# shiinamiyuki/akari_render

Hardware: AMD Instinct MI355X
Metric: Msamples/s (whole node), 1080p path tracer, C2 (higher is better)
Workload: dtype f32

## Files before the change

akari_render_amd/abi.py:

```python
from __future__ import annotations

import ctypes as C
from dataclasses import dataclass, field
from typing import List, Optional

import numpy as np

c_f32p = C.POINTER(C.c_float)
c_u32p = C.POINTER(C.c_uint32)


class _Struct(C.Structure):

    def __setattr__(self, name, value):
        if not any(f[0] == name for f in self._fields_):
            raise AttributeError("%s has no field %r" % (type(self).__name__, name))
        super().__setattr__(name, value)


class MeshDesc(C.Structure):
    _fields_ = [
        ("n_vertices", C.c_uint32),
        ("n_triangles", C.c_uint32),
        ("vertices", c_f32p),
# ... 239 lines not shown
        ("adaptive", C.c_uint32), ("wis", C.c_uint32),
        ("seed", C.c_uint64),
        ("filter_type", C.c_uint32), ("filter_radius", C.c_float), ("sampler_type", C.c_uint32), ("color", C.c_uint32),
        ("sampler_seed", C.c_uint64),
    ]

    @staticmethod
    def default() -> "McmcConfig":
        c = McmcConfig()
        c.spp, c.max_depth, c.rr_depth, c.spp_per_pass, c.use_nee = 256, 7, 5, 64, 1
        c.mcmc_depth, c.n_chains, c.n_bootstrap, c.direct_spp = 0xFFFFFFFF, 512, 100000, 64
        c.exponential_mutation, c.small_sigma, c.large_step_prob, c.image_mutation_prob, c.image_mutation_size = 1, 0.01, 0.1, 0.0, 0.0
        c.filter_type, c.filter_radius = FILTER_GAUSSIAN, 1.5
        c.sampler_type, c.sampler_seed = SAMPLER_INDEPENDENT, 0
        return c


class McmcResult(C.Structure):
    _fields_ = [("normalization", C.c_double), ("acceptance_rate", C.c_double), ("splat_scale", C.c_float), ("contribution", C.c_float),
                ("n_mutations", C.c_uint64), ("sample_dimension", C.c_uint32), ("_pad", C.c_uint32)]


class McmcPartial(C.Structure):

    _fields_ = [("bootstrap_sum", C.c_double), ("b_sum", C.c_double), ("n_bootstrap", C.c_uint64), ("b_cnt", C.c_uint64), ("n_accepted", C.c_uint64),
                ("n_mutations", C.c_uint64), ("n_executed", C.c_uint64), ("spp", C.c_uint32), ("contribution", C.c_float)]


MARKOV_STATE_DTYPE = [("cur_pixel", "<u4", (2,)), ("chain_id", "<u4"), ("cur_f", "<f4"), ("b", "<f4"), ("b_cnt", "<u4"), ("n_accepted", "<u4"),
                      ("n_mutations", "<u4"), ("cur_iter", "<u4"), ("last_large_iter", "<u4")]


class AdaptiveConfig(_Struct):

    _fields_ = [("threshold", C.c_float), ("min_spp", C.c_uint32), ("round_passes", C.c_uint32), ("_pad", C.c_uint32)]

    @staticmethod
    def default() -> "AdaptiveConfig":
        c = AdaptiveConfig()
        c.threshold, c.min_spp, c.round_passes = 0.0625, 16, 1
        return c


DISPLAY_LINEAR, DISPLAY_REINHARD, DISPLAY_ACES, DISPLAY_HABLE = 1, 2, 3, 4
DISPLAY_CURVE_NAMES = {DISPLAY_LINEAR: "linear", DISPLAY_REINHARD: "reinhard", DISPLAY_ACES: "aces", DISPLAY_HABLE: "hable"}


class DisplayConfig(_Struct):

    _fields_ = [
        ("curve", C.c_uint32),
        ("auto_exposure", C.c_uint32),
        ("exposure_ev", C.c_float),
        ("key", C.c_float),
        ("low_permille", C.c_uint32),
        ("high_permille", C.c_uint32),
        ("white", C.c_float),
        ("bloom_strength", C.c_float),
        ("bloom_threshold", C.c_float),
        ("bloom_levels", C.c_uint32),
        ("_pad", C.c_uint32 * 2),
    ]

    @staticmethod
    def default() -> "DisplayConfig":
        c = DisplayConfig()
        c.curve, c.auto_exposure, c.exposure_ev, c.key = DISPLAY_ACES, 0, 0.0, 0.18
        c.low_permille, c.high_permille, c.white = 50, 20, 0.0
        c.bloom_strength, c.bloom_threshold, c.bloom_levels = 0.0, 1.0, 5
        return c


class PtStats(C.Structure):
    _fields_ = [
        ("n_samples", C.c_uint64),
        ("n_closest", C.c_uint64),
        ("n_shadow", C.c_uint64),
        ("n_shaded", C.c_uint64),
        ("n_node_visits", C.c_uint64),
        ("n_tri_tests", C.c_uint64),
        ("kernel_ms", C.c_double),
        ("n_launches", C.c_uint32),
        ("_pad", C.c_uint32),
    ]

    def as_dict(self):
        return {k: getattr(self, k) for k, _ in self._fields_ if not k.startswith("_")}


class AdaptiveStats(C.Structure):

    _fields_ = [("rounds", C.c_uint32), ("tiles_retired", C.c_uint32), ("samples_drawn", C.c_uint64), ("samples_uniform", C.c_uint64), ("pt", PtStats)]

    def as_dict(self):
        return {"rounds": self.rounds, "tiles_retired": self.tiles_retired, "samples_drawn": self.samples_drawn, "samples_uniform": self.samples_uniform,
                "pt": self.pt.as_dict()}


class KernelInfo(C.Structure):

    _fields_ = [
        ("struct_size", C.c_uint32),
        ("specialised", C.c_uint32),
        ("cache_hit", C.c_uint32),
        ("n_shader_kinds", C.c_uint32),
        ("absent_mask", C.c_uint32),
        ("min_waves", C.c_uint32),
        ("vgprs", C.c_uint32),
        ("scratch_bytes", C.c_uint32),
        ("kernel_flags", C.c_uint32),
        ("_pad", C.c_uint32),
        ("compile_ms", C.c_double),
        ("load_ms", C.c_double),
        ("status", C.c_char * 256),
    ]

    def as_dict(self):
        d = {k: getattr(self, k) for k, _ in self._fields_ if k not in ("struct_size", "status", "_pad")}
        d["status"] = self.status.decode(errors="replace")
        return d


class PtLaunchPlan(C.Structure):

    VARIANT = ("bvh", "fd", "tex", "pmj", "stage", "defer", "simple", "inst", "env", "lens")
    _fields_ = [
        ("variant", C.c_uint32 * 10),
        ("simple_scene", C.c_uint32), ("defer_metal", C.c_uint32), ("defer_flags", C.c_uint32),
        ("stage_bytes", C.c_uint32 * 13), ("stage_total", C.c_uint32),
        ("tile_offset", C.c_uint32), ("bvh_tile_nodes", C.c_uint32), ("park_offset", C.c_uint32), ("carry_offset", C.c_uint32),
        ("bn_offset", C.c_uint32), ("val_offset_words", C.c_uint32),
        ("lds_bytes", C.c_uint32), ("blocks", C.c_uint32),
        ("specialised", C.c_uint32),
        ("wrapper", C.c_char * 600),
    ]

    def as_dict(self):
        d = {k: getattr(self, k) for k, _ in self._fields_ if k not in ("variant", "stage_bytes", "wrapper")}
        d["variant"] = {n: int(self.variant[i]) for i, n in enumerate(self.VARIANT)}
        d["stage_bytes"] = [int(b) for b in self.stage_bytes]
        d["wrapper"] = self.wrapper.decode()
        return d


class PtFeaturesPlan(C.Structure):

    _fields_ = [
        ("plan", PtLaunchPlan),
        ("feat", C.c_uint32), ("kernel_compiled", C.c_uint32), ("park_slots", C.c_uint32), ("park_slots_feat", C.c_uint32),
        ("required_bytes", C.c_uint32), ("lds_budget", C.c_uint32),
    ]

    def as_dict(self):
        d = self.plan.as_dict()
        d["variant"]["feat"] = int(self.feat)
        for k in ("kernel_compiled", "park_slots", "park_slots_feat", "required_bytes", "lds_budget"):
            d[k] = int(getattr(self, k))
        return d


class SceneInfo(C.Structure):
    _fields_ = [
        ("width", C.c_uint32),
        ("height", C.c_uint32),
        ("n_instances", C.c_uint32),
        ("n_triangles", C.c_uint32),
        ("n_materials", C.c_uint32),
        ("n_lights", C.c_uint32),
        ("n_bvh_nodes", C.c_uint32),
        ("uses_bvh", C.c_uint32),
# ... 243 lines not shown
```

akari_render_amd/capi.py:

```python
from __future__ import annotations

import ctypes as C
import os
from typing import Optional

import numpy as np

from . import abi
from .build import LIB, build

AKR_OK = 0
FILM_PLANE_RGB, FILM_PLANE_SPLAT, FILM_PLANE_WEIGHT, FILM_PLANES_PT, FILM_PLANES_ALL = 1, 2, 4, 5, 7
ERR_INVALID_ARGUMENT, ERR_HIP, ERR_NO_DEVICE, ERR_IO, ERR_PARSE, ERR_UNSUPPORTED, ERR_OOM, ERR_RENDER = -1, -2, -3, -4, -5, -6, -7, -8

(ARRAY_WOOP, ARRAY_TRI_GID, ARRAY_SHADE, ARRAY_INSTANCES, ARRAY_MATERIALS, ARRAY_BVH_NODES, ARRAY_LIGHT_ENTRIES,
 ARRAY_LIGHT_PDF, ARRAY_AREA_ENTRIES, ARRAY_AREA_PDF, ARRAY_INST_TRI_OFFSET, ARRAY_R2C, ARRAY_C2W,
 ARRAY_TEX_NODES, ARRAY_TEX_IMAGES, ARRAY_TEX_TEXELS, ARRAY_MAT_INPUTS,
 ARRAY_INST_LEAVES, ARRAY_MESH_TRIS, ARRAY_MESH_POS, ARRAY_MESH_META, ARRAY_MESH_NORMALS,
 ARRAY_ENV_MARGINAL_ENTRIES, ARRAY_ENV_MARGINAL_PDF, ARRAY_ENV_CONDITIONAL_ENTRIES, ARRAY_ENV_CONDITIONAL_PDF, ARRAY_ENV_TEXELS) = range(27)
ENV_LIGHT_INSTANCE = 0xFFFFFFFF

EXPORTS = [
    "akr_last_error", "akr_version", "akr_struct_size", "akr_option_set", "akr_option_get", "akr_context_create",
    "akr_context_destroy", "akr_context_synchronize", "akr_context_device_info", "akr_scene_create", "akr_scene_load",
    "akr_scene_destroy", "akr_scene_set_resolution", "akr_scene_get_info", "akr_scene_get_light", "akr_scene_get_ggx_table",
    "akr_scene_get_desc_counts", "akr_scene_get_mesh", "akr_scene_get_instance", "akr_scene_get_material", "akr_scene_get_camera",
    "akr_scene_get_array", "akr_scene_get_image_count", "akr_scene_get_image", "akr_scene_get_material_graph", "akr_film_create",
    "akr_film_wrap", "akr_film_destroy", "akr_film_clear", "akr_film_read", "akr_film_write", "akr_film_resolve",
    "akr_film_device_ptr", "akr_pt_config_default", "akr_pt_config_from_json", "akr_pt_render", "akr_pt_begin", "akr_pt_passes",
    "akr_pt_begin_features", "akr_pt_render_features",
    "akr_pt_end", "akr_pt_get_stats", "akr_render_task", "akr_image_write", "akr_aov_config_default", "akr_aov_render",
    "akr_gpt_config_default", "akr_gpt_render", "akr_gpt_begin", "akr_gpt_sample", "akr_gpt_sums", "akr_gpt_sums_read",
    "akr_gpt_sums_write", "akr_gpt_finish", "akr_gpt_abort", "akr_gpt_reduce", "akr_mcmc_config_default", "akr_mcmc_render",
    "akr_film_set_splat_scale", "akr_film_get_splat_scale", "akr_pt_read_sampler_states", "akr_context_device_ordinal",
    "akr_device_count", "akr_comm_unique_id", "akr_comm_create", "akr_comm_wrap", "akr_comm_destroy", "akr_film_reduce",
    "akr_pt_kernel_info", "akr_scene_spec_source", "akr_host_spec_compile", "akr_host_spec_compile_text",
    "akr_film_reduce_planes", "akr_mcmc_render_shard", "akr_mcmc_combine_host", "akr_mcmc_combine",
    "akr_scene_set_environment", "akr_scene_get_environment", "akr_scene_set_lens", "akr_scene_get_lens",
    "akr_denoise_config_default", "akr_denoise", "akr_denoise_variance",
    "akr_pt_set_active_tiles", "akr_film_tile_error", "akr_adaptive_config_default", "akr_pt_adaptive_render",
    "akr_display_config_default", "akr_film_luminance_histogram", "akr_display_exposure", "akr_display_transform",
]
TEST_EXPORTS = [
    "akr_probe_material_inputs_host", "akr_host_stdrng_u64", "akr_host_chacha_block", "akr_host_pcg32_states",
    "akr_host_pcg_start", "akr_host_alias_table", "akr_probe_math", "akr_probe_bsdf", "akr_probe_intersect",
    "akr_probe_surface_interaction", "akr_probe_material_inputs", "akr_host_decode_png", "akr_host_decode_jpeg",
    "akr_host_decode_exr", "akr_host_decode_tiff", "akr_host_decode_dds", "akr_host_pmj02bn_tables",
    "akr_probe_material_folded_host", "akr_host_sobol_dim1", "akr_host_fastmod", "akr_host_tri_pretest",
    "akr_probe_env_sample", "akr_probe_env_pdf", "akr_host_lens_ray", "akr_probe_camera_rays",
    "akr_probe_div", "akr_probe_intersect_pair", "akr_probe_math2", "akr_host_denoise", "akr_probe_denoise_times",
    "akr_host_pt_launch_plan", "akr_host_denoise_variance", "akr_probe_denoise_variance_times",
    "akr_host_tile_error", "akr_host_half_bracket", "akr_probe_adapt_times",
    "akr_host_display_transform", "akr_host_luminance_histogram", "akr_probe_display_times",
    "akr_host_pt_features_plan", "akr_host_pcg_end_pass", "akr_probe_pcg_end_pass",
]


class RenderSession(C.Structure):

    _fields_ = [("save_intermediate", C.c_int32), ("save_stats", C.c_int32), ("name", C.c_char_p),
                ("override_sampler_independent", C.c_int32), ("verbose", C.c_int32)]


class AkariError(RuntimeError):
    def __init__(self, code: int, msg: str):
        super().__init__(f"akari_hip error {code}: {msg}")
        self.code = code


_lib: Optional[C.CDLL] = None


def lib() -> C.CDLL:
    global _lib
    if _lib is not None:
        return _lib
    if not os.path.exists(LIB):
        build()
    L = C.CDLL(os.environ.get("AKR_HIP_LIB") or LIB)
    vp, u32, u64, i32, f32 = C.c_void_p, C.c_uint32, C.c_uint64, C.c_int32, C.c_float
    fp, up, u64p, vpp = C.POINTER(C.c_float), C.POINTER(C.c_uint32), C.POINTER(C.c_uint64), C.POINTER(C.c_void_p)
    L.akr_last_error.restype = C.c_char_p
    L.akr_version.restype = C.c_char_p
    L.akr_struct_size.restype = C.c_uint32
    L.akr_struct_size.argtypes = [C.c_int32]
    for sid, cls in enumerate((abi.MeshDesc, abi.InstanceDesc, abi.MaterialDesc, abi.CameraDesc, abi.SceneDesc, abi.PtConfig, abi.PtStats, abi.SceneInfo,
                               abi.KernelInfo, abi.AovConfig, abi.GptConfig, abi.McmcConfig, abi.McmcResult, abi.McmcPartial,
                               abi.EnvironmentDesc, abi.LensDesc, abi.DenoiseConfig), start=1):
        if L.akr_struct_size(sid) != C.sizeof(cls):
            raise ImportError("libakari_hip.so and akari_render_amd/abi.py disagree on sizeof(%s): %d vs %d" % (cls.__name__, L.akr_struct_size(sid), C.sizeof(cls)))
    for sid, cls in ((19, abi.AdaptiveConfig), (20, abi.AdaptiveStats), (22, abi.DisplayConfig)):
        if L.akr_struct_size(sid) != C.sizeof(cls):
            raise ImportError("libakari_hip.so and akari_render_amd/abi.py disagree on sizeof(%s): %d vs %d" % (cls.__name__, L.akr_struct_size(sid), C.sizeof(cls)))

    def proto(name, *args):
        if name in TEST_EXPORTS and not hasattr(L, name):
            return
        fn = getattr(L, name)
        fn.restype = i32
        fn.argtypes = list(args)

    proto("akr_context_create", i32, vpp)
    proto("akr_context_destroy", vp)
    proto("akr_context_synchronize", vp)
    proto("akr_context_device_info", vp, C.c_char_p, u32, up, u64p)
    proto("akr_scene_create", vp, C.POINTER(abi.SceneDesc), vpp)
    proto("akr_scene_load", vp, C.c_char_p, u32, u32, vpp)
    proto("akr_scene_destroy", vp)
    proto("akr_scene_set_resolution", vp, u32, u32)
    proto("akr_scene_get_info", vp, C.POINTER(abi.SceneInfo))
    proto("akr_scene_get_light", vp, u32, up, fp, fp)
    proto("akr_scene_set_environment", vp, C.POINTER(abi.EnvironmentDesc))
    proto("akr_scene_get_environment", vp, C.POINTER(abi.EnvironmentDesc))
    proto("akr_scene_set_lens", vp, C.POINTER(abi.LensDesc))
    proto("akr_scene_get_lens", vp, C.POINTER(abi.LensDesc))
    proto("akr_host_lens_ray", vp, u32, f32, u32, up, fp, fp)
    proto("akr_probe_camera_rays", vp, vp, u32, f32, u32, up, fp, fp)
    proto("akr_host_pt_launch_plan", vp, C.POINTER(abi.PtConfig), i32, i32, i32, i32, C.POINTER(abi.PtLaunchPlan))
    proto("akr_host_pt_features_plan", vp, C.POINTER(abi.PtConfig), i32, i32, i32, i32, i32, i32, i32, C.POINTER(abi.PtFeaturesPlan))
    proto("akr_probe_env_sample", vp, vp, u32, fp, fp)
    proto("akr_probe_env_pdf", vp, vp, u32, fp, fp)
    proto("akr_scene_get_ggx_table", vp, fp)
    proto("akr_scene_get_desc_counts", vp, up, up, up)
    proto("akr_scene_get_mesh", vp, u32, C.POINTER(abi.MeshDesc))
    proto("akr_scene_get_instance", vp, u32, C.POINTER(abi.InstanceDesc))
    proto("akr_scene_get_material", vp, u32, C.POINTER(abi.MaterialDesc))
    proto("akr_scene_get_camera", vp, C.POINTER(abi.CameraDesc))
    proto("akr_scene_get_array", vp, i32, vpp, u64p)
    proto("akr_scene_get_image_count", vp, up)
    proto("akr_scene_get_image", vp, u32, C.POINTER(abi.ImageDesc))
    proto("akr_scene_get_material_graph", vp, u32, C.POINTER(abi.MaterialGraph))
    proto("akr_film_create", vp, u32, u32, vpp)
    proto("akr_film_wrap", vp, u32, u32, vp, vpp)
    proto("akr_film_destroy", vp)
    proto("akr_film_clear", vp)
    proto("akr_film_read", vp, fp)
    proto("akr_film_write", vp, fp)
    proto("akr_film_resolve", vp, fp)
    proto("akr_film_device_ptr", vp, vpp, u64p)
    proto("akr_pt_kernel_info", vp, C.POINTER(abi.KernelInfo))
    proto("akr_scene_spec_source", vp, C.c_char_p, u64, u64p)
    proto("akr_host_spec_compile", vp, u32, u32, C.c_char_p, u64p, C.c_char_p, u32)
    proto("akr_probe_material_folded_host", vp, u32, u32, fp, up, fp, fp)
    proto("akr_host_sobol_dim1", u32, up, up, up)
    proto("akr_host_fastmod", u32, up, up, up)
    proto("akr_host_tri_pretest", u32, fp, fp, f32, up, up, fp)
    proto("akr_host_spec_compile_text", C.c_char_p, u32, u32, C.c_char_p, C.c_char_p)
    proto("akr_context_device_ordinal", vp, C.POINTER(C.c_int32))
    proto("akr_device_count", C.POINTER(C.c_int32))
    proto("akr_option_set", C.c_char_p, i32)
    proto("akr_option_get", C.c_char_p, C.POINTER(C.c_int32))
    proto("akr_comm_unique_id", C.POINTER(C.c_uint8))
    proto("akr_comm_create", vp, C.POINTER(C.c_uint8), i32, i32, vpp)
    proto("akr_comm_wrap", vp, vp, i32, i32, vpp)
    proto("akr_comm_destroy", vp)
    proto("akr_film_reduce", vp, vp, i32, i32)
    proto("akr_film_reduce_planes", vp, vp, i32, i32, u32)
    proto("akr_mcmc_render_shard", vp, vp, C.POINTER(abi.McmcConfig), u32, u32, vp, C.POINTER(abi.McmcPartial), up, C.POINTER(abi.PtStats))
    proto("akr_mcmc_combine_host", vp, C.POINTER(abi.McmcPartial), u32, C.POINTER(abi.McmcResult))
    proto("akr_mcmc_combine", vp, vp, i32, C.POINTER(abi.McmcPartial), C.POINTER(abi.McmcResult))
    proto("akr_pt_config_default", C.POINTER(abi.PtConfig))
    proto("akr_aov_config_default", C.POINTER(abi.AovConfig))
    proto("akr_aov_render", vp, vp, C.POINTER(abi.AovConfig), vp, C.POINTER(abi.PtStats))
    proto("akr_gpt_config_default", C.POINTER(abi.GptConfig))
    proto("akr_gpt_render", vp, vp, C.POINTER(abi.GptConfig), vp, fp, C.POINTER(abi.PtStats))
    proto("akr_gpt_begin", vp, vp, C.POINTER(abi.GptConfig), vp, vp, vpp)
    proto("akr_gpt_sample", vp, u32, i32)
    proto("akr_gpt_sums", vp, C.POINTER(fp), u64p)
    proto("akr_gpt_sums_read", vp, fp)
    proto("akr_gpt_sums_write", vp, fp)
    proto("akr_gpt_finish", vp, fp, C.POINTER(abi.PtStats))
    proto("akr_gpt_abort", vp, C.POINTER(abi.PtStats))
    proto("akr_gpt_reduce", vp, vp, i32, i32)
    proto("akr_mcmc_config_default", C.POINTER(abi.McmcConfig))
    proto("akr_mcmc_render", vp, vp, C.POINTER(abi.McmcConfig), vp, C.POINTER(abi.McmcResult), up, C.POINTER(abi.PtStats))
    proto("akr_film_set_splat_scale", vp, C.c_float)
    proto("akr_film_get_splat_scale", vp, fp)
    proto("akr_pt_config_from_json", C.c_char_p, C.POINTER(abi.PtConfig), C.c_char_p, u32)
    proto("akr_pt_render", vp, vp, C.POINTER(abi.PtConfig), vp, C.POINTER(abi.PtStats))
    proto("akr_pt_begin", vp, vp, C.POINTER(abi.PtConfig), vp, vpp)
    proto("akr_pt_passes", vp, u32, i32, up)
    proto("akr_pt_begin_features", vp, vp, C.POINTER(abi.PtConfig), vp, vp, vp, vpp)
    proto("akr_pt_render_features", vp, vp, C.POINTER(abi.PtConfig), vp, vp, vp, C.POINTER(abi.PtStats))
    proto("akr_pt_end", vp, C.POINTER(abi.PtStats))
    proto("akr_pt_get_stats", vp, C.POINTER(abi.PtStats))
    proto("akr_render_task", vp, vp, C.c_char_p, C.POINTER(RenderSession), C.POINTER(abi.PtStats))
    proto("akr_image_write", C.c_char_p, fp, u32, u32)
    proto("akr_pt_read_sampler_states", vp, u64p)
    proto("akr_host_stdrng_u64", u64, u32, u64p)
    proto("akr_host_chacha_block", up, u64, u64, i32, up)
    proto("akr_host_pcg32_states", u64, u64, u64p)
    proto("akr_host_pcg_start", u64p, u64)
    proto("akr_host_pcg_end_pass", u64p, u64, u32)
    proto("akr_probe_pcg_end_pass", vp, u32, u64p, u64p, up, u64p, u64p)
    proto("akr_host_alias_table", fp, u32, up, fp, fp)
    proto("akr_probe_math", vp, u32, fp, fp, fp, fp)
    proto("akr_probe_math2", vp, u32, fp, fp)
    proto("akr_probe_bsdf", vp, C.POINTER(abi.MaterialDesc), fp, i32, fp, u32, fp, fp)
    proto("akr_probe_intersect", vp, vp, u32, fp, up, fp)
    proto("akr_probe_div", vp, u32, fp, fp, fp, fp)
    proto("akr_probe_intersect_pair", vp, vp, u32, fp, up, up, fp)
    proto("akr_probe_surface_interaction", vp, vp, u32, up, fp, fp)
# ... 238 lines not shown
        for i in range(nm.value):
            m = abi.MeshDesc()
            check(lib().akr_scene_get_mesh(self.h, i, C.byref(m)))
            nt = m.n_triangles
            uv = arr(m.uvs, 6 * nt, np.float32)
            nr = arr(m.normals, 9 * nt, np.float32)
            tg = arr(m.tangents, 9 * nt, np.float32)
            meshes.append(abi.MeshData(
                vertices=arr(m.vertices, 3 * m.n_vertices, np.float32).reshape(-1, 3),
                indices=arr(m.indices, 3 * nt, np.uint32).reshape(-1, 3),
                uvs=None if uv is None else uv.reshape(-1, 3, 2),
                normals=None if nr is None else nr.reshape(-1, 3, 3),
                tangents=None if tg is None else tg.reshape(-1, 3, 3),
                material_slots=arr(m.material_slots, nt, np.uint32)))
        for i in range(ni.value):
            d = abi.InstanceDesc()
            check(lib().akr_scene_get_instance(self.h, i, C.byref(d)))
            instances.append(abi.InstanceData(d.mesh, [int(d.materials[k]) for k in range(d.n_materials)],
                                              np.array(list(d.transform), dtype=np.float32)))
        for i in range(nmat.value):
            d = abi.MaterialDesc()
            check(lib().akr_scene_get_material(self.h, i, C.byref(d)))
            md = abi.MaterialData()
            md.kind = d.kind & abi.MAT_KIND_MASK
            md.colorspaces = d.kind & 0xF00
            for name in ("base_color", "specular_tint", "coat_tint", "emission_color", "normal"):
                setattr(md, name, tuple(float(x) for x in getattr(d, name)))
            for name in ("base_alpha", "metallic", "roughness", "ior", "specular_ior_level", "transmission_weight",
                         "coat_weight", "coat_roughness", "coat_ior", "emission_strength"):
                setattr(md, name, float(getattr(d, name)))
            g = abi.MaterialGraph()
            check(lib().akr_scene_get_material_graph(self.h, i, C.byref(g)))
            if g.n_nodes:
                nodes = [abi.NodeData(int(g.nodes[j].op), tuple(int(a) for a in g.nodes[j].arg), tuple(float(x) for x in g.nodes[j].k))
                         for j in range(g.n_nodes)]
                inputs = {abi.INPUT_NAMES[k]: int(g.input[k]) for k in range(abi.IN_COUNT) if g.input[k] != abi.NODE_NONE}
                md.graph = abi.GraphData(nodes, inputs)
            materials.append(md)
        images = []
        nimg = C.c_uint32()
        check(lib().akr_scene_get_image_count(self.h, C.byref(nimg)))
        for i in range(nimg.value):
            d = abi.ImageDesc()
            check(lib().akr_scene_get_image(self.h, i, C.byref(d)))
            n = d.width * d.height * 4
            if d.format == abi.IMAGE_RGBA8:
                t = np.frombuffer((C.c_uint8 * n).from_address(d.texels), dtype=np.uint8).copy()
            else:
                t = np.frombuffer((C.c_float * n).from_address(d.texels), dtype=np.float32).copy()
            images.append(abi.ImageData(t.reshape(d.height, d.width, 4), d.filter, d.address))
        c = abi.CameraDesc()
        check(lib().akr_scene_get_camera(self.h, C.byref(c)))
        cam = abi.CameraData(np.array(list(c.c2w), dtype=np.float32), float(c.fov), c.width, c.height)
        return abi.SceneData(meshes, instances, materials, cam, images=images, environment=self.environment(), lens=self.lens())


def set_option(name: str, value: int) -> None:
    check(lib().akr_option_set(name.encode(), int(value)))


def get_option(name: str) -> int:
    v = C.c_int32()
    check(lib().akr_option_get(name.encode(), C.byref(v)))
    return v.value


class options:

    def __init__(self, **kw):
        self.kw, self.old = kw, {}

    def __enter__(self):
        for k, v in self.kw.items():
            self.old[k] = get_option(k)
            set_option(k, v)
        return self

    def __exit__(self, *exc):
        for k, v in self.old.items():
            set_option(k, v)
        return False


def last_error() -> str:
    return lib().akr_last_error().decode("utf-8", "replace")


def device_count() -> int:
    n = C.c_int32()
    check(lib().akr_device_count(C.byref(n)))
    return n.value


def comm_unique_id() -> bytes:
    buf = (C.c_uint8 * 128)()
    check(lib().akr_comm_unique_id(buf))
    return bytes(buf)


class Comm:

    def __init__(self, ctx: "Context", unique_id: bytes, rank: int, world: int):
        assert len(unique_id) == 128
        self.h = C.c_void_p()
        buf = (C.c_uint8 * 128).from_buffer_copy(unique_id)
        check(lib().akr_comm_create(ctx.h, buf, rank, world, C.byref(self.h)))
        self.rank, self.world = rank, world

    def close(self):
        if getattr(self, "h", None):
            lib().akr_comm_destroy(self.h)
            self.h = None

    def __del__(self):
        try:
            self.close()
        except Exception:
            pass

    def mcmc_combine(self, film: "Film", partial, root: int = 0) -> dict:
        res = abi.McmcResult()
        check(lib().akr_mcmc_combine(film.h, self.h, root, C.byref(partial), C.byref(res)))
        return {k: getattr(res, k) for k, _ in abi.McmcResult._fields_ if k != "_pad"}

    def reduce_film(self, film: "Film", root: int = 0, blocking: bool = True, planes: int = 7):
        check(lib().akr_film_reduce_planes(film.h, self.h, root, 1 if blocking else 0, planes))


class Film:

    def __init__(self, ctx: Context, width: int, height: int, device_ptr: Optional[int] = None):
        self.ctx, self.width, self.height = ctx, width, height
        self.h = C.c_void_p()
        if device_ptr is None:
            check(lib().akr_film_create(ctx.h, width, height, C.byref(self.h)))
        else:
            check(lib().akr_film_wrap(ctx.h, width, height, C.c_void_p(device_ptr), C.byref(self.h)))

    def close(self):
        if self.h:
            lib().akr_film_destroy(self.h)
            self.h = C.c_void_p()

    def __del__(self):
        try:
            self.close()
        except Exception:
            pass

    def clear(self):
        check(lib().akr_film_clear(self.h))

    def read(self) -> np.ndarray:
        out = np.zeros(7 * self.width * self.height, dtype=np.float32)
        check(lib().akr_film_read(self.h, _fp(out)))
        return out

    def write(self, data: np.ndarray):
        data = np.ascontiguousarray(data, dtype=np.float32)
        assert data.size == 7 * self.width * self.height
        check(lib().akr_film_write(self.h, _fp(data)))

    def resolve(self) -> np.ndarray:
        out = np.zeros(3 * self.width * self.height, dtype=np.float32)
        check(lib().akr_film_resolve(self.h, _fp(out)))
        return out.reshape(self.height, self.width, 3)
# ... 522 lines not shown
```

akari_render_amd/csrc/device/pt_pass.h:

```cpp
#pragma once
#include "dpath.h"

namespace akr {

#ifndef AKR_PT_MIN_WAVES
#define AKR_PT_MIN_WAVES 4
#endif
#ifndef AKR_PT_MIN_WAVES_BVH
#define AKR_PT_MIN_WAVES_BVH 4
#endif
#ifndef AKR_PT_MIN_WAVES_FD
#define AKR_PT_MIN_WAVES_FD 4
#endif
#ifndef AKR_PT_MIN_WAVES_TEX
#define AKR_PT_MIN_WAVES_TEX 3
#endif
#ifndef AKR_PT_MIN_WAVES_BVH_TEX
#define AKR_PT_MIN_WAVES_BVH_TEX 3
#endif
template <bool TEX>
using PairWalkOpt = WalkOpt<!TEX>;
template <bool BVH, bool FD, bool TEX, bool PMJ, bool STAGE, bool DEFER, uint32_t ABSENT = 0, bool INST = false, bool ENV = false, bool LENS = false, bool FEAT = false>
AKR_D void pt_pass_body(const PtParams& p) {
    extern __shared__ __attribute__((aligned(16))) uint32_t lds_stack[];
    TraceCtx tc;
    tc.stack = lds_stack + threadIdx.x;
    tc.cnt = TraceCounters{0, 0, 0};
    PtParams staged = p;
    if (STAGE) stage_scene_tables<BVH, TEX, !BVH && !FD && TEX>(p, lds_stack, staged);
    const PtParams& q = STAGE ? staged : p;
    const DScene& sc = q.sc;
    constexpr bool TILE = BVH && !TEX && !INST;
    constexpr uint32_t STRAG = BVH ? (INST ? AKR_PT_STRAGGLERS_INST : (TEX ? AKR_PT_STRAGGLERS_TEX : AKR_PT_STRAGGLERS)) : 0;
    const uint4* tile = (const uint4*)(lds_stack + p.tile_offset);
    if (TILE) {
        uint32_t* l = lds_stack + p.tile_offset;
        const uint32_t* g = (const uint32_t*)p.sc.bvh_nodes;
        for (uint32_t i = threadIdx.x; i < p.sc.bvh_tile_nodes * kBvhNodeWords; i += 256u) l[i] = g[i];
        __syncthreads();
    }
    const float4* lds_recs = nullptr;
    if (!BVH) {
        uint32_t* l = lds_stack + (p.stage_total >> 2);
        const uint32_t* g = (const uint32_t*)p.sc.woop;
        for (uint32_t i = threadIdx.x; i < (p.sc.n_tris + 2u) * 12u; i += 256u) l[i] = g[i];
        __syncthreads();
        lds_recs = (const float4*)l;
    }
    const uint32_t item = blockIdx.x * 256u + threadIdx.x;
    uint32_t px = 0, py = 0;
    const bool in_frame = item < p.n_items && item_to_pixel(p, item, px, py);
    const uint32_t pix = px + py * p.width;
    uint32_t sx, sy;
    shifted_pixel(p, px, py, sx, sy);
    if (PMJ && p.bn_offset != 0) pmj_bluenoise_stage(p, px, py);
    PathRegs r;
    path_regs_init<PMJ, LENS, FEAT>(r, q, in_frame, pix, sx, sy);
    constexpr bool PARK = !FD && TEX;
    uint32_t* park = lds_stack + p.park_offset + threadIdx.x;
    if (PARK) {
        park_put(park, PK_PIX, pix);
        park_put(park, PK_SX, sx);
        park_put(park, PK_SY, sy);
        if (FEAT) {
            park_put(park, PK_FEAT_A + 0, f2u(r.feat_a.x)); park_put(park, PK_FEAT_A + 1, f2u(r.feat_a.y)); park_put(park, PK_FEAT_A + 2, f2u(r.feat_a.z));
            park_put(park, PK_FEAT_N + 0, f2u(r.feat_n.x)); park_put(park, PK_FEAT_N + 1, f2u(r.feat_n.y)); park_put(park, PK_FEAT_N + 2, f2u(r.feat_n.z));
        }
    }

    uint32_t iteration = 0;
    while (__builtin_amdgcn_ballot_w64(r.active) != 0) {
        iteration++;
        if (r.active) {
            Hit hit;
            bool found = false, occluded = false;
            if (!(STRAG > 0 && r.carry)) {
                r.c_closest += r.has_ray ? 1u : 0u;
                r.c_shadow += r.has_shadow ? 1u : 0u;
            }
            if (BVH && INST) {
                trace_pair_inst<TEX, STRAG>(sc, r.has_ray, r.ro, r.rd, r.ray_ex0, r.has_shadow, r.s_o, r.s_d, r.s_tmax, r.s_ex0, r.s_ex1, r.carry, hit, found, occluded, tc.stack,
                                            lds_stack + p.carry_offset + threadIdx.x, tc.cnt);
            } else if (BVH && STRAG > 0) {
                uint32_t* cy = lds_stack + p.carry_offset + threadIdx.x;
                Trav s;
                uint32_t phase;
                hit.t = 1e20f; hit.u = 0.0f; hit.v = 0.0f; hit.gid = kInvalid;
                if (!r.carry) {
                    phase = r.has_ray ? 0u : (r.has_shadow ? 1u : 2u);
                    if (phase == 0) trav_begin(s, r.ro, r.rd, 0.0f, 1e20f, r.ray_ex0, kInvalid);
                    else trav_begin(s, r.s_o, r.s_d, 0.0f, phase == 1 ? r.s_tmax : -1.0f, r.s_ex0, r.s_ex1);
                } else {
                    phase = cy[CY_PHASE * 256];
                    if (phase == 0) trav_begin(s, r.ro, r.rd, 0.0f, 1e20f, r.ray_ex0, kInvalid);
                    else {
                        trav_begin(s, r.s_o, r.s_d, 0.0f, r.s_tmax, r.s_ex0, r.s_ex1);
                        hit.t = u2f(cy[CY_HIT_T * 256]); hit.u = u2f(cy[CY_HIT_U * 256]); hit.v = u2f(cy[CY_HIT_V * 256]); hit.gid = cy[CY_HIT_GID * 256];
                        found = hit.gid != kInvalid;
                    }
                    s.best_t = u2f(cy[CY_BEST_T * 256]); s.best_u = u2f(cy[CY_BEST_U * 256]); s.best_v = u2f(cy[CY_BEST_V * 256]); s.best = cy[CY_BEST * 256];
                    s.G = cy[CY_G * 256]; s.T = cy[CY_T * 256]; s.tbase = cy[CY_TBASE * 256]; s.sp = cy[CY_SP * 256];
                    s.active = true;
                }
                const uint32_t n_in = (uint32_t)__builtin_popcountll(__builtin_amdgcn_ballot_w64(phase != 2u));
                const uint32_t n_leave = n_in / (STRAG > 0 ? STRAG : 1u);
                while (true) {
                    const uint32_t n_now = (uint32_t)__builtin_popcountll(__builtin_amdgcn_ballot_w64(phase != 2u));
                    if (n_now <= n_leave) break;
                    if (phase != 2u) {
                        if (s.active) trav_step<2, TEX, TILE>(sc, s, tc.stack, tc.cnt, phase == 1u, tile);
                        if (!s.active) {
                            if (phase == 0u) {
                                found = s.best != kInvalid;
                                hit.t = s.best_t; hit.u = s.best_u; hit.v = s.best_v; hit.gid = s.best;
                                phase = r.has_shadow ? 1u : 2u;
                                if (r.has_shadow) trav_begin(s, r.s_o, r.s_d, 0.0f, r.s_tmax, r.s_ex0, r.s_ex1);
                            } else {
                                occluded = s.best != kInvalid;
                                phase = 2u;
                            }
                        }
                    }
                }
                r.carry = phase != 2u;
                if (r.carry) {
                    cy[CY_BEST_T * 256] = f2u(s.best_t); cy[CY_BEST_U * 256] = f2u(s.best_u); cy[CY_BEST_V * 256] = f2u(s.best_v); cy[CY_BEST * 256] = s.best;
                    cy[CY_G * 256] = s.G; cy[CY_T * 256] = s.T; cy[CY_TBASE * 256] = s.tbase; cy[CY_SP * 256] = s.sp;
                    cy[CY_PHASE * 256] = phase;
                    if (phase == 1u) { cy[CY_HIT_T * 256] = f2u(hit.t); cy[CY_HIT_U * 256] = f2u(hit.u); cy[CY_HIT_V * 256] = f2u(hit.v); cy[CY_HIT_GID * 256] = hit.gid; }
                }
            } else if (BVH) {
                Trav s;
                uint32_t phase = r.has_ray ? 0u : (r.has_shadow ? 1u : 2u);
                if (phase == 0) trav_begin(s, r.ro, r.rd, 0.0f, 1e20f, r.ray_ex0, kInvalid);
                else trav_begin(s, r.s_o, r.s_d, 0.0f, phase == 1 ? r.s_tmax : -1.0f, r.s_ex0, r.s_ex1);
                hit.t = 1e20f; hit.u = 0.0f; hit.v = 0.0f; hit.gid = kInvalid;
                while (phase != 2u) {
                    if (s.active) trav_step<2, TEX, TILE>(sc, s, tc.stack, tc.cnt, phase == 1u, tile);
                    if (!s.active) {
                        if (phase == 0u) {
                            found = s.best != kInvalid;
                            hit.t = s.best_t; hit.u = s.best_u; hit.v = s.best_v; hit.gid = s.best;
                            phase = r.has_shadow ? 1u : 2u;
                            if (r.has_shadow) trav_begin(s, r.s_o, r.s_d, 0.0f, r.s_tmax, r.s_ex0, r.s_ex1);
                        } else {
                            occluded = s.best != kInvalid;
                            phase = 2u;
                        }
                    }
                }
            } else {
                trace_pair_exhaustive<TEX, PairWalkOpt<TEX>>(sc, r.ro, r.rd, r.has_ray ? 1e20f : -1.0f, r.ray_ex0, r.s_o, r.s_d, r.has_shadow ? r.s_tmax : -1.0f, r.s_ex0, r.s_ex1, hit, found,
                                           occluded, lds_recs);
            }
            if (DEFER) {
                if (r.deferred) {
                    hit.gid = r.d_gid; hit.u = r.d_u; hit.v = r.d_v; hit.t = 0.0f;
                    found = true;
                    r.has_ray = true;
                    r.deferred = false;
                } else if (r.has_ray && found && (iteration & q.defer_metal)) {
                    const uint32_t mat = f2u(sc.shade[(size_t)hit.gid * SHADE_ROWS + 6].y);
                    if (sc.materials[mat].flags & q.defer_flags) {
                        r.d_gid = hit.gid; r.d_u = hit.u; r.d_v = hit.v;
                        r.deferred = true;
                        r.has_ray = false;
                    }
                }
            }
            if (STRAG > 0 && r.carry) {
            } else if (PARK) path_step<FD ? 1 : 0, TEX, PMJ, DEFER ? 1 : 2, ABSENT, INST, ENV, LENS, FEAT>(q, r, hit, found, occluded, 0, 0, 0, park);
            else path_step<FD ? 1 : 0, TEX, PMJ, 0, ABSENT, INST, ENV, LENS, FEAT>(q, r, hit, found, occluded, pix, sx, sy);
        }
    }
    flush_counters(p, r, tc.cnt, BVH);
}

constexpr int pt_pass_min_waves(bool bvh, bool fd, bool tex) {
    return bvh ? (tex ? AKR_PT_MIN_WAVES_BVH_TEX : AKR_PT_MIN_WAVES_BVH) : (fd ? AKR_PT_MIN_WAVES_FD : (tex ? AKR_PT_MIN_WAVES_TEX : AKR_PT_MIN_WAVES));
}

}
```

akari_render_amd/csrc/host/api_internal.h:

```cpp
#pragma once
#include <atomic>
#include <mutex>
#include <hip/hip_runtime.h>

#include <algorithm>
#include <array>
#include <cstdlib>
#include <cstdio>
#include <chrono>
#include <cstring>
#include <functional>
#include <map>
#include <memory>
#include <new>
#include <stdexcept>
#include <string>
#include <vector>

#include "scene_build.h"
#include "specialise.h"
#include "stdrng.h"


namespace akr_api {
// ... 88 lines not shown
    TileGrid g;
    auto or_default = [](uint32_t t) { return t ? t : 32u; };
    g.tile_w = or_default(tile_w);
    g.tile_h = or_default(tile_h);
    g.tiles_x = (width + g.tile_w - 1) / g.tile_w;
    g.tiles_y = (height + g.tile_h - 1) / g.tile_h;
    uint32_t n = g.tiles_x * g.tiles_y;
    if (count > 1) {
        n = 0;
        for (uint32_t ty = 0; ty < g.tiles_y; ty++)
            for (uint32_t tx = 0; tx < g.tiles_x; tx++) n += tile_owner(tx, ty, count) == rank ? 1u : 0u;
    }
    g.n_items = n * g.tile_w * g.tile_h;
    return g;
}

}
using namespace akr_api;


struct akr_context {
    int device = 0;
    hipStream_t stream = nullptr;
    hipDeviceProp_t props;
    void bind() const { HIP_CHECK(hipSetDevice(device)); }
    SpecCache spec_cache;
    std::mutex ggx_mutex;
    std::vector<float> ggx_cache;
    DevBuf pmj_sets, bluenoise;
    void ensure_pmj_tables() {
        if (pmj_sets.p && bluenoise.p) return;
        std::vector<uint32_t> sets;
        std::vector<uint16_t> bn;
        make_pmj02_sets(sets);
        load_bluenoise(bn);
        pmj_sets.upload(sets);
        bluenoise.upload(bn);
    }
};

struct akr_scene {
    akr_context* ctx = nullptr;
    FlatScene flat;
    CompiledScene cs;
    DevBuf light_alias, area_alias, lights;
    DevBuf woop, tri_gid, shade, normals, inst, materials, ggx_table, light_entries, light_pdf, light_inst, light_tri_offset,
        light_n_tris, area_entries, area_pdf, inst_tri_offset, bvh_nodes, tex_nodes, tex_images, tex_texels, tex_mat_inputs;
    DevBuf in2_tlas_leaves, in2_mesh_tris, in2_mesh_pos, in2_mesh_meta, in2_mesh_normals, in2_inst_mats, in2_share_bits;
    DevBuf env_texels, env_marginal, env_conditional, env_rec;
    std::atomic<int> sessions{0};
    std::vector<float> ggx_host;
    struct ColorSet {
        DevBuf materials, tex_nodes, mat_inputs;
    };
    std::map<uint32_t, std::unique_ptr<ColorSet>> color_sets;
    std::mutex color_sets_mutex;
    std::string spec_header;
    bool spec_header_made = false;
    std::mutex spec_mutex;
    DScene dscene;
    float r2c[16], c2w[16];
    uint32_t c2w_identity = 0;
    uint64_t device_bytes = 0;
};

struct akr_film {
    akr_context* ctx = nullptr;
    uint32_t width = 0, height = 0;
    DevBuf own;
    float* data = nullptr;
    float splat_scale = 1.0f;
    size_t n_floats() const { return 7ull * width * height; }
};

struct RenderBase {
    akr_context* ctx = nullptr;
    akr_scene* scene = nullptr;
    akr_film* film = nullptr;
    akr_pt_config cfg;
    DevBuf states, counters;
    TileGrid grid;
    DevBuf owned_tiles;
    uint32_t spp_done = 0, n_launches = 0;
    uint32_t pmj_spp = 1;
    const akr_scene::ColorSet* color_set = nullptr;
    int defer_metal_option = -1;
    int simple_kernels_option = 1;
    int defer_on_option = 0;
    std::vector<std::pair<hipEvent_t, hipEvent_t>> pending;
    double kernel_ms = 0.0;
    PtVariant variant{};
    PtParams params;
    bool holds_scene = false;
    akr_film *feat_albedo = nullptr, *feat_normal = nullptr;
    void fold_events(bool all) {
        size_t keep = 0;
        for (size_t i = 0; i < pending.size(); i++) {
            auto& ev = pending[i];
            if (all || hipEventQuery(ev.second) == hipSuccess) {
                float t = 0.0f;
                if (hipEventElapsedTime(&t, ev.first, ev.second) == hipSuccess) kernel_ms += t;
                (void)hipEventDestroy(ev.first);
                (void)hipEventDestroy(ev.second);
            } else {
                pending[keep++] = ev;
            }
        }
        pending.resize(keep);
    }
    virtual ~RenderBase() {
        if (holds_scene) scene->sessions--;
        for (auto& ev : pending) {
            (void)hipEventDestroy(ev.first);
            (void)hipEventDestroy(ev.second);
        }
    }
};

struct WavefrontState {
    DevBuf state, queues, ctrl, pend, carry;
    bool sort = false;
    DevBuf keys, sorted, sort_tmp;
    uint32_t *sorted_closest = nullptr, *sorted_shadow = nullptr, *sorted_keys = nullptr;
    WfBuffers buf;
    uint32_t slots = 0, trace_blocks = 0;
    std::vector<WfBuffers> group;
    std::vector<hipStream_t> streams;
    std::vector<hipEvent_t> join;
    hipEvent_t fork = nullptr;
    ~WavefrontState() {
        for (hipStream_t st : streams) (void)hipStreamDestroy(st);
        for (hipEvent_t ev : join) (void)hipEventDestroy(ev);
        if (fork) (void)hipEventDestroy(fork);
    }
};

struct akr_pt_session : RenderBase {
    std::unique_ptr<WavefrontState> wf;
    int sched_trial = 0;
    uint64_t passes_launched = 0;
    int max_fused_option = 0;
    bool spec_active = false;
    bool arith_relaxed = false;
    int spec_waves = 3;
    std::shared_ptr<SpecKernel> spec;
    std::string spec_status = "not requested";
    DevBuf active_tiles;
    bool active_set = false;
};

namespace akr_api {
struct LaunchTimer {
    RenderBase* se;
    hipEvent_t e0 = nullptr, e1 = nullptr;
    explicit LaunchTimer(RenderBase* s) : se(s) {
        HIP_CHECK(hipEventCreate(&e0));
        HIP_CHECK(hipEventCreate(&e1));
        HIP_CHECK(hipEventRecord(e0, se->ctx->stream));
    }
    LaunchTimer(const LaunchTimer&) = delete;
    LaunchTimer& operator=(const LaunchTimer&) = delete;
    void stop() {
        HIP_CHECK(hipEventRecord(e1, se->ctx->stream));
        se->pending.emplace_back(e0, e1);
        e0 = e1 = nullptr;
        if (se->pending.size() > 16) se->fold_events(false);
    }
    ~LaunchTimer() {
        if (e0) (void)hipEventDestroy(e0);
        if (e1) (void)hipEventDestroy(e1);
    }
};

void base_begin(RenderBase* se, akr_context* ctx, akr_scene* scene, const akr_pt_config* cfg, akr_film* film);
int32_t render_begin(akr_context* ctx, akr_scene* scene, const akr_pt_config* cfg, akr_film* film, RenderBase** out);
int32_t base_end(RenderBase* se, akr_pt_stats* stats);
void session_params(RenderBase* se, bool spec_active = false, int spec_waves = 3, bool wf_sort = false);
inline void set_launch_passes(RenderBase* se, uint32_t n_passes, uint32_t last_pass_spp) {
    se->params.n_passes = n_passes;
    se->params.last_pass_spp = last_pass_spp;
}
struct PtPlan {
    PtVariant v;
    uint32_t simple_scene, defer_metal, defer_flags;
    uint32_t stage_bytes[13], stage_total, tex_slots;
};
PtPlan pt_plan(const akr_scene* s, const akr_pt_config& c, int defer_metal_option, int simple_kernels_option, int defer_on_option, bool spec_active, int spec_waves, bool feat = false);
std::string pt_features_refusal(const akr_scene* s, const TuningOptions& t);
PtVariant pt_scene_facts(const akr_scene* s, const akr_pt_config& c);
inline uint32_t scene_stack_depth(const CompiledScene& cs) {
    return cs.instanced.on ? cs.bvh_depth : std::max(1u, std::min(cs.bvh_depth, kBvhStackDepth));
}
inline uint32_t scene_n_nodes(const CompiledScene& cs) { return (uint32_t)((cs.instanced.on ? cs.instanced.nodes.size() : cs.bvh_nodes.size()) / kBvhNodeWords); }
void camera_params(PtParams& p, const akr_scene* s, uint32_t filter_type, float filter_radius);
template <typename End>
int32_t end_keeping_first_error(int32_t rc, End&& end) {
    const std::string err = g_last_error;
    const int32_t rc2 = end();
    if (rc == AKR_OK) return rc2;
    g_last_error = err;
    return rc;
}
uint32_t session_samples(const akr_pt_config& c);
std::vector<uint32_t> owned_tiles(uint32_t tiles_x, uint32_t tiles_y, uint32_t rank, uint32_t count);
void scene_finish(akr_scene* s);
void scene_spec_header(akr_scene* scene, std::string& out);
int32_t mcmc_render_impl(akr_context* ctx, akr_scene* scene, const akr_mcmc_config* cfg, akr_film* film, akr_mcmc_result* result, uint32_t* chain_states,
                         akr_pt_stats* stats, const std::function<void(uint32_t, double)>& on_pass, uint32_t shard_rank = 0, uint32_t shard_count = 1,
                         akr_mcmc_partial* partial = nullptr);
}
```

akari_render_amd/csrc/host/api_probe.cpp:

```cpp
#if defined(AKR_TEST_HOOKS) && AKR_TEST_HOOKS
#include "api_internal.h"
#include "../../../include/akari_hip_test.h"
#include "../device/dinst.h"
#include "../device/disect.h"
#include "../device/dpath.h"

extern "C" {

AKR_TEST_API int32_t akr_host_stdrng_u64(uint64_t seed, uint32_t n, uint64_t* out) {
    if (!out) return fail(AKR_ERR_INVALID_ARGUMENT, "out is NULL");
    StdRng rng(seed);
    for (uint32_t i = 0; i < n; i++) out[i] = rng.next_u64();
    return AKR_OK;
}
AKR_TEST_API int32_t akr_host_chacha_block(const uint32_t* key8, uint64_t counter, uint64_t stream, int32_t rounds, uint32_t* out16) {
    if (!key8 || !out16) return fail(AKR_ERR_INVALID_ARGUMENT, "NULL argument");
    StdRng::chacha_block(key8, counter, stream, rounds, out16);
    return AKR_OK;
}
AKR_TEST_API int32_t akr_host_pcg32_states(uint64_t seed, uint64_t n, uint64_t* out2n) {
    if (!out2n) return fail(AKR_ERR_INVALID_ARGUMENT, "out is NULL");
    StdRng rng(seed);
    for (uint64_t i = 0; i < n; i++) {
        Pcg32 p = pcg_new_seq_offset(i, rng.next_u64());
// ... 191 lines not shown
        DevBuf din, dout;
        din.upload(std::vector<float>(in, in + n_in));
        dout.alloc(n_out * 4);
        if (n) HIP_CHECK(launch_probe_env(probe_params(scene), mode, n, din.as<float>(), dout.as<float>(), ctx->stream));
        HIP_CHECK(hipStreamSynchronize(ctx->stream));
        if (n) HIP_CHECK(hipMemcpy(out, dout.p, n_out * 4, hipMemcpyDeviceToHost));
    });
}
AKR_TEST_API int32_t akr_probe_env_sample(akr_context* ctx, akr_scene* scene, uint32_t n, const float* u2, float* out5) {
    return probe_env(ctx, scene, 0, n, u2, out5, "akr_probe_env_sample");
}
AKR_TEST_API int32_t akr_probe_env_pdf(akr_context* ctx, akr_scene* scene, uint32_t n, const float* dirs3, float* out4) {
    return probe_env(ctx, scene, 1, n, dirs3, out4, "akr_probe_env_pdf");
}
static PtParams probe_camera_params(const akr_scene* s, uint32_t filter_type, float filter_radius) {
    PtParams p;
    std::memset(&p, 0, sizeof p);
    camera_params(p, s, filter_type, filter_radius);
    return p;
}
AKR_TEST_API int32_t akr_host_lens_ray(const akr_scene* scene, uint32_t filter_type, float filter_radius, uint32_t n, const uint32_t* pixels2, const float* u4, float* out6) {
    if (!scene || !pixels2 || !u4 || !out6) return fail(AKR_ERR_INVALID_ARGUMENT, "akr_host_lens_ray: NULL argument");
    if (filter_type > AKR_FILTER_GAUSSIAN) return fail(AKR_ERR_INVALID_ARGUMENT, "akr_host_lens_ray: unknown filter_type");
    const PtParams p = probe_camera_params(scene, filter_type, filter_radius);
    for (uint32_t i = 0; i < n; i++) {
        const float* u = u4 + 4ull * i;
        vec3 o, d;
        if (p.lens_radius > 0.0f) generate_ray_lens_from(p, pixels2[2ull * i], pixels2[2ull * i + 1], mk2(u[0], u[1]), mk2(u[2], u[3]), o, d);
        else generate_ray_from(p, pixels2[2ull * i], pixels2[2ull * i + 1], mk2(u[0], u[1]), o, d);
        float* r = out6 + 6ull * i;
        r[0] = o.x; r[1] = o.y; r[2] = o.z; r[3] = d.x; r[4] = d.y; r[5] = d.z;
    }
    return AKR_OK;
}
static std::pair<PtVariant, PtLdsLayout> fill_launch_plan(akr_scene* scene, const akr_pt_config* cfg, int32_t defer_metal, int32_t simple_kernels, int32_t defer_on, int32_t spec_waves, bool feat,
                                                          akr_pt_launch_plan* out) {
        const CompiledScene& cs = scene->cs;
        const bool spec = !feat && spec_waves != 0 && cs.has_textures && !cfg->force_diffuse;
        const PtPlan pl = pt_plan(scene, *cfg, defer_metal, simple_kernels, defer_on, spec, spec ? spec_waves : 3, feat);
        const PtVariant& v = pl.v;
        const PtLdsSizes sizes{scene_stack_depth(cs), cs.n_tris, scene_n_nodes(cs), pl.tex_slots, pl.stage_total, cfg->sampler_type == AKR_SAMPLER_PMJ02BN};
        const PtLdsLayout L = pt_lds_layout(v, sizes);
        const TileGrid grid = tile_grid(cfg->tile_w, cfg->tile_h, scene->flat.camera.width, scene->flat.camera.height, cfg->shard_rank, cfg->shard_count);
        std::memset(out, 0, sizeof *out);
        const bool flags[10] = {v.bvh, v.fd, v.tex, v.pmj, v.stage, v.defer, v.simple, v.inst, v.env, v.lens};
        for (int i = 0; i < 10; i++) out->variant[i] = flags[i] ? 1u : 0u;
        out->simple_scene = pl.simple_scene; out->defer_metal = pl.defer_metal; out->defer_flags = pl.defer_flags;
        std::memcpy(out->stage_bytes, pl.stage_bytes, sizeof out->stage_bytes);
        out->stage_total = pl.stage_total;
        out->tile_offset = L.tile_offset; out->bvh_tile_nodes = L.tile_nodes; out->park_offset = L.park_offset; out->carry_offset = L.carry_offset;
        out->bn_offset = L.bn_offset; out->val_offset_words = L.val_offset_words;
        out->lds_bytes = (uint32_t)L.total_bytes;
        out->blocks = (grid.n_items + 255u) / 256u;
        out->specialised = spec ? 1u : 0u;
        if (spec) std::snprintf(out->wrapper, sizeof out->wrapper, "%s", spec_wrapper_source(v, spec_waves).c_str());
        return {v, L};
}
AKR_TEST_API int32_t akr_host_pt_launch_plan(akr_scene* scene, const akr_pt_config* cfg, int32_t defer_metal, int32_t simple_kernels, int32_t defer_on, int32_t spec_waves,
                                             akr_pt_launch_plan* out) {
    if (!scene || !cfg || !out) return fail(AKR_ERR_INVALID_ARGUMENT, "akr_host_pt_launch_plan: NULL argument");
    return guarded([&] { fill_launch_plan(scene, cfg, defer_metal, simple_kernels, defer_on, spec_waves, false, out); });
}
AKR_TEST_API int32_t akr_host_pt_features_plan(akr_scene* scene, const akr_pt_config* cfg, int32_t defer_metal, int32_t simple_kernels, int32_t defer_on, int32_t spec_waves, int32_t feat,
                                               int32_t wavefront, int32_t arith, akr_pt_features_plan* out) {
    if (!scene || !cfg || !out) return fail(AKR_ERR_INVALID_ARGUMENT, "akr_host_pt_features_plan: NULL argument");
    return guarded([&] {
        if (feat) {
            TuningOptions t;
            t.wavefront = wavefront;
            t.arith = arith;
            const std::string why = pt_features_refusal(scene, t);
            if (!why.empty()) throw Unsupported(why);
        }
        std::memset(out, 0, sizeof *out);
        const auto vl = fill_launch_plan(scene, cfg, defer_metal, simple_kernels, defer_on, spec_waves, feat != 0, &out->plan);
        out->feat = vl.first.feat ? 1u : 0u;
        out->kernel_compiled = pt_variant_compiled(vl.first) ? 1u : 0u;
        out->park_slots = (vl.second.carry_offset - vl.second.park_offset) / 256u;
        out->required_bytes = (uint32_t)vl.second.required_bytes;
        out->lds_budget = (uint32_t)pt_lds_budget(vl.first.tex);
        out->park_slots_feat = kParkSlotsFeat;
    });
}
AKR_TEST_API int32_t akr_probe_camera_rays(akr_context* ctx, akr_scene* scene, uint32_t filter_type, float filter_radius, uint32_t n, const uint32_t* pixels2,
                                      const float* u4, float* out6) {
    if (!ctx || !scene || !pixels2 || !u4 || !out6) return fail(AKR_ERR_INVALID_ARGUMENT, "akr_probe_camera_rays: NULL argument");
    if (filter_type > AKR_FILTER_GAUSSIAN) return fail(AKR_ERR_INVALID_ARGUMENT, "akr_probe_camera_rays: unknown filter_type");
    return guarded([&] {
        ctx->bind();
        DevBuf dpx, du, dout;
        dpx.upload(std::vector<uint32_t>(pixels2, pixels2 + 2ull * n));
        du.upload(std::vector<float>(u4, u4 + 4ull * n));
        dout.alloc(6ull * n * 4);
        if (n) HIP_CHECK(launch_probe_camera_rays(probe_camera_params(scene, filter_type, filter_radius), n, dpx.as<uint32_t>(), du.as<float>(), dout.as<float>(), ctx->stream));
        HIP_CHECK(hipStreamSynchronize(ctx->stream));
        if (n) HIP_CHECK(hipMemcpy(out6, dout.p, 6ull * n * 4, hipMemcpyDeviceToHost));
    });
}
AKR_TEST_API int32_t akr_probe_surface_interaction(akr_context* ctx, akr_scene* scene, uint32_t n, const uint32_t* inst_prim, const float* bary,
                                              float* out) {
    if (!ctx || !scene || !inst_prim || !bary || !out) return fail(AKR_ERR_INVALID_ARGUMENT, "akr_probe_surface_interaction: NULL argument");
    return guarded([&] {
        ctx->bind();
        for (uint32_t i = 0; i < n; i++) {
            uint32_t inst = inst_prim[2 * i], prim = inst_prim[2 * i + 1];
            if (inst >= scene->flat.instances.size() || prim >= scene->flat.meshes[scene->flat.instances[inst].mesh].n_triangles())
                throw std::invalid_argument("akr_probe_surface_interaction: (inst, prim) out of range");
        }
        DevBuf dip, db, dout;
        std::vector<uint32_t> ipv(inst_prim, inst_prim + 2ull * n);
        std::vector<float> bv(bary, bary + 2ull * n);
        dip.upload(ipv);
        db.upload(bv);
        dout.alloc(19ull * n * 4);
        if (n) HIP_CHECK(launch_probe_si(probe_params(scene), n, dip.as<uint32_t>(), db.as<float>(), dout.as<float>(), ctx->stream));
        HIP_CHECK(hipStreamSynchronize(ctx->stream));
        if (n) HIP_CHECK(hipMemcpy(out, dout.p, 19ull * n * 4, hipMemcpyDeviceToHost));
    });
}

AKR_TEST_API int32_t akr_host_pmj02bn_tables(uint32_t* sets, uint16_t* bluenoise) {
    return guarded([&] {
        if (sets) {
            std::vector<uint32_t> v;
            make_pmj02_sets(v);
            std::memcpy(sets, v.data(), v.size() * 4);
        }
        if (bluenoise) {
            std::vector<uint16_t> v;
            load_bluenoise(v);
            std::memcpy(bluenoise, v.data(), v.size() * 2);
        }
    });
}
AKR_TEST_API int32_t akr_host_decode_png(const uint8_t* data, uint64_t len, uint32_t* width, uint32_t* height, uint8_t* rgba, uint64_t capacity) {
    if (!data || !width || !height) return fail(AKR_ERR_INVALID_ARGUMENT, "akr_host_decode_png: NULL argument");
    return guarded([&] {
        std::vector<uint8_t> px;
        decode_png(data, (size_t)len, *width, *height, px);
        if (rgba) {
            if (capacity < px.size()) throw std::invalid_argument("akr_host_decode_png: output buffer too small");
            std::memcpy(rgba, px.data(), px.size());
        }
    });
}
AKR_TEST_API int32_t akr_host_decode_jpeg(const uint8_t* data, uint64_t len, uint32_t* width, uint32_t* height, uint8_t* rgba, uint64_t capacity) {
    if (!data || !width || !height) return fail(AKR_ERR_INVALID_ARGUMENT, "akr_host_decode_jpeg: NULL argument");
    return guarded([&] {
        std::vector<uint8_t> px;
        decode_jpeg(data, (size_t)len, *width, *height, px);
        if (rgba) {
            if (capacity < px.size()) throw std::invalid_argument("akr_host_decode_jpeg: output buffer too small");
            std::memcpy(rgba, px.data(), px.size());
        }
    });
}
AKR_TEST_API int32_t akr_host_decode_tiff(const uint8_t* data, uint64_t len, uint32_t* width, uint32_t* height, uint8_t* rgba, uint64_t capacity) {
    if (!data || !width || !height) return fail(AKR_ERR_INVALID_ARGUMENT, "akr_host_decode_tiff: NULL argument");
    return guarded([&] {
        std::vector<uint8_t> px;
        decode_tiff(data, (size_t)len, *width, *height, px);
        if (rgba) {
            if (capacity < px.size()) throw std::invalid_argument("akr_host_decode_tiff: output buffer too small");
            std::memcpy(rgba, px.data(), px.size());
        }
    });
// ... 101 lines not shown
```

akari_render_amd/csrc/host/api_pt.cpp:

```cpp
#include "api_internal.h"

void akr_api::camera_params(PtParams& p, const akr_scene* s, uint32_t filter_type, float filter_radius) {
    std::memcpy(p.r2c, s->r2c, 64);
    std::memcpy(p.c2w, s->c2w, 64);
    p.c2w_identity = s->c2w_identity;
    p.width = s->flat.camera.width;
    p.height = s->flat.camera.height;
    p.filter_type = filter_type;
    p.filter_radius = filter_radius;
    p.lens_radius = s->flat.lens.radius;
    p.lens_focal = s->flat.lens.focal_distance;
}
PtVariant akr_api::pt_scene_facts(const akr_scene* s, const akr_pt_config& c) {
    const CompiledScene& cs = s->cs;
    return PtVariant{cs.has_tree(), c.force_diffuse != 0, cs.has_textures, c.sampler_type != AKR_SAMPLER_INDEPENDENT, false, false, false,
                     cs.instanced.on, cs.env.on, s->flat.lens.radius > 0.0f};
}
std::string akr_api::pt_features_refusal(const akr_scene* s, const TuningOptions& t) {
    if (s->cs.instanced.on)
        return "unsupported: akr_pt_begin_features: the scene is kept as meshes + instances (option instancing); its kernels collect no guides -- render them with akr_aov_render";
    if (t.wavefront == 1) return "unsupported: akr_pt_begin_features: the wavefront schedule is forced (option wavefront = 1); only the megakernel collects guides";
    if (t.arith == 1) return "unsupported: akr_pt_begin_features: the relaxed arithmetic tier (option arith = 1) has no kernels that collect guides";
    return "";
}
// ... 374 lines not shown
    });
}

}
void akr_api::base_begin(RenderBase* se, akr_context* ctx, akr_scene* scene, const akr_pt_config* cfg, akr_film* film) {
    if (!ctx || !scene || !cfg || !film) throw std::invalid_argument("akr_pt_begin: NULL argument");
    if (scene->ctx != ctx) throw std::invalid_argument("akr_pt_begin: the scene was not created on this context (host-only scenes cannot render)");
    se->grid = tile_grid(cfg->tile_w, cfg->tile_h, scene->flat.camera.width, scene->flat.camera.height, cfg->shard_rank, cfg->shard_count);
    validate_config(*cfg, se->grid);
    if (film->width != scene->flat.camera.width || film->height != scene->flat.camera.height)
        throw std::invalid_argument("film resolution does not match the scene camera (pt.rs:1072-1073)");
    ctx->bind();
    se->ctx = ctx;
    se->scene = scene;
    se->film = film;
    se->cfg = *cfg;
    std::unique_lock<std::mutex> color_lock(scene->color_sets_mutex);
    if (cfg->color != 0 && !scene->color_sets.count(cfg->color)) {
        CompiledScene tmp;
        tmp.images = scene->cs.images;
        std::vector<akr_material_desc> descs;
        compile_materials(scene->flat, cfg->color, tmp, descs);
        auto set = std::make_unique<akr_scene::ColorSet>();
        set->materials.upload(tmp.materials);
        if (tmp.has_textures) {
            set->tex_nodes.upload(tmp.tex_nodes);
            set->mat_inputs.upload(tmp.mat_inputs);
        }
        scene->color_sets[cfg->color] = std::move(set);
    }
    if (cfg->color != 0) se->color_set = scene->color_sets.at(cfg->color).get();
    color_lock.unlock();
    const uint64_t n = (uint64_t)film->width * film->height;
    if (cfg->sampler_type == AKR_SAMPLER_PMJ02BN || cfg->sampler_type == AKR_SAMPLER_SOBOL) {
        if (cfg->sampler_type == AKR_SAMPLER_PMJ02BN) ctx->ensure_pmj_tables();
        se->pmj_spp = cfg->spp ? cfg->spp : 1;
        std::vector<Pcg32> init(n);
        const uint64_t first = cfg->sample_begin ? (uint64_t)(cfg->sample_begin - 1u) : 0xffffffffull;
        for (uint64_t i = 0; i < n; i++) init[i] = Pcg32{first, (i % film->width) | ((i / film->width) << 32)};
        se->states.upload(init);
    } else {
        std::vector<uint64_t> seeds(n);
        StdRng rng(cfg->sampler_seed);
        for (auto& v : seeds) v = rng.next_u64();
        DevBuf dseeds;
        dseeds.upload(seeds);
        se->states.alloc(n * sizeof(Pcg32));
        HIP_CHECK(launch_init_pcg32(dseeds.as<uint64_t>(), se->states.p, n, ctx->stream));
        HIP_CHECK(hipStreamSynchronize(ctx->stream));
    }
    se->counters.alloc(8 * kStatStripes * sizeof(uint64_t));
    HIP_CHECK(hipMemsetAsync(se->counters.p, 0, se->counters.bytes, ctx->stream));
    if (cfg->shard_count > 1) se->owned_tiles.upload(owned_tiles(se->grid.tiles_x, se->grid.tiles_y, cfg->shard_rank, cfg->shard_count));
    const TuningOptions t = tuning();
    se->defer_metal_option = t.defer_metal;
    se->simple_kernels_option = t.simple_kernels;
    se->defer_on_option = t.defer_on;
    scene->sessions++;
    se->holds_scene = true;
}
int32_t akr_api::render_begin(akr_context* ctx, akr_scene* scene, const akr_pt_config* cfg, akr_film* film, RenderBase** out) {
    *out = nullptr;
    return guarded([&] {
        auto se = std::make_unique<RenderBase>();
        base_begin(se.get(), ctx, scene, cfg, film);
        session_params(se.get());
        HIP_CHECK(hipStreamSynchronize(ctx->stream));
        *out = se.release();
    });
}
static int32_t pt_begin(akr_context* ctx, akr_scene* scene, const akr_pt_config* cfg, akr_film* film, akr_film* albedo, akr_film* normal, akr_pt_session** out) {
    *out = nullptr;
    return guarded([&] {
        auto se = std::make_unique<akr_pt_session>();
        base_begin(se.get(), ctx, scene, cfg, film);
        se->feat_albedo = albedo;
        se->feat_normal = normal;
        const bool features = albedo != nullptr;
        const bool wavefront = !features && choose_wavefront(se.get());
        const bool wf_sort = wavefront && tuning().wf_sort != 0;
        {
            const TuningOptions t = tuning();
            se->max_fused_option = t.max_fused_passes;
            const uint64_t samples = (uint64_t)film->width * film->height * (uint64_t)session_samples(*cfg);
            const bool may_compile = t.specialise == 1 || samples >= kSpecAutoSamples;
            const PtVariant facts = pt_scene_facts(scene, *cfg);
            se->arith_relaxed = t.arith == 1 && !facts.inst && !wavefront && !features;
            if (se->arith_relaxed && facts.env)
                throw Unsupported("unsupported: the relaxed arithmetic tier (option arith = 1) does not render scenes with an environment light");
            if (se->arith_relaxed && facts.lens)
                throw Unsupported("unsupported: the relaxed arithmetic tier (option arith = 1) does not render through a lens (akr_scene_set_lens)");
            if (se->arith_relaxed) se->spec_status = "relaxed arithmetic tier: precompiled kernels";
            else if (wavefront) se->spec_status = "wavefront schedule";
            else if (features) se->spec_status = scene->cs.has_textures && t.specialise == 1 ? "guides are collected by the interpreter kernels: no per-scene kernel (option specialise ignored)"
                                                                                            : "guides are collected by the precompiled kernels";
            else if (!scene->cs.has_textures) se->spec_status = "the scene has no texture-fed material";
            else if (t.specialise == 0) se->spec_status = "option specialise = 0";
            else if (cfg->force_diffuse) se->spec_status = "force_diffuse kernels evaluate no surface graphs";
            else {
                {
                    std::lock_guard<std::mutex> lock(scene->spec_mutex);
                    if (!scene->spec_header_made) {
                        scene->spec_header = generate_scene_spec(scene->cs);
                        scene->spec_header_made = true;
                    }
                }
                se->spec_waves = t.specialise_waves ? t.specialise_waves : 3;
                se->spec_active = true;
            }
            session_params(se.get(), se->spec_active, se->spec_waves, wf_sort);
            if (se->spec_active) {
                se->spec = ctx->spec_cache.get(scene->spec_header, se->variant, se->spec_waves, ctx->props.gcnArchName, may_compile);
                se->spec_status = se->spec->status;
                if (!se->spec->fn) {
                    se->spec_active = false;
                    session_params(se.get(), false, se->spec_waves, wf_sort);
                }
            }
        }
        if (wavefront) se->wf = wf_allocate(se.get(), wf_sort);
        se->sched_trial = schedule_trial_eligible(se.get()) ? 1 : 0;
        HIP_CHECK(hipStreamSynchronize(ctx->stream));
        *out = se.release();
    });
}
extern "C" {
AKR_API int32_t akr_pt_begin(akr_context* ctx, akr_scene* scene, const akr_pt_config* cfg, akr_film* film, akr_pt_session** out) {
    if (!out) return fail(AKR_ERR_INVALID_ARGUMENT, "akr_pt_begin: NULL argument");
    return pt_begin(ctx, scene, cfg, film, nullptr, nullptr, out);
}
AKR_API int32_t akr_pt_begin_features(akr_context* ctx, akr_scene* scene, const akr_pt_config* cfg, akr_film* film, akr_film* albedo, akr_film* normal, akr_pt_session** out) {
    if (!out) return fail(AKR_ERR_INVALID_ARGUMENT, "akr_pt_begin_features: NULL argument");
    *out = nullptr;
    if (!ctx || (scene && !scene->ctx))
        return fail(AKR_ERR_UNSUPPORTED, "unsupported: akr_pt_begin_features: guides are collected by GPU kernels; a host-only scene (no device context) cannot render them");
    if (!scene || !cfg || !film) return fail(AKR_ERR_INVALID_ARGUMENT, "akr_pt_begin_features: NULL argument");
    if (!albedo || !normal) return fail(AKR_ERR_INVALID_ARGUMENT, "akr_pt_begin_features: both guide films are required (albedo and normal)");
    if (albedo == normal || albedo == film || normal == film) return fail(AKR_ERR_INVALID_ARGUMENT, "akr_pt_begin_features: film, albedo and normal must be three different films");
    for (const akr_film* g : {albedo, normal}) {
        if (g->ctx != ctx) return fail(AKR_ERR_INVALID_ARGUMENT, "akr_pt_begin_features: a guide film belongs to another context");
        if (g->width != scene->flat.camera.width || g->height != scene->flat.camera.height)
            return fail(AKR_ERR_INVALID_ARGUMENT, "akr_pt_begin_features: a guide film's resolution does not match the scene camera");
    }
    const std::string why = pt_features_refusal(scene, tuning());
    if (!why.empty()) return fail(AKR_ERR_UNSUPPORTED, why);
    return pt_begin(ctx, scene, cfg, film, albedo, normal, out);
}
AKR_API int32_t akr_pt_passes(akr_pt_session* se, uint32_t n_passes, int32_t blocking, uint32_t* spp_done) {
    if (!se) return fail(AKR_ERR_INVALID_ARGUMENT, "session is NULL");
    return guarded([&] {
        se->ctx->bind();
        uint32_t kMaxFusedPasses = 16;
        se->fold_events(false);
        if (se->max_fused_option > 0) {
            kMaxFusedPasses = (uint32_t)se->max_fused_option;
        } else if (blocking && se->pending.empty() && se->passes_launched > 0 && se->kernel_ms > 0.0) {
            const double per_pass_ms = se->kernel_ms / (double)se->passes_launched;
            const double fit = 3000.0 / per_pass_ms;
            kMaxFusedPasses = fit >= 64.0 ? 64u : (fit <= 16.0 ? 16u : (uint32_t)fit);
        }
        uint32_t left = n_passes;
        const uint32_t total = session_samples(se->cfg);
        auto launch = [&](uint32_t max_fused) {
            uint32_t fused = 0, last = 0, done = se->spp_done;
            while (fused < max_fused && fused < left && done < total) {
                last = std::min(total - done, se->cfg.spp_per_pass);
                done += last;
                fused++;
            }
            set_launch_passes(se, fused, last);
            LaunchTimer timer(se);
            if (se->active_set && se->params.n_items == 0) {}
            else if (se->wf) wf_run(se);
            else HIP_CHECK(launch_pt_pass(se->params, se->variant, se->ctx->stream, se->spec_active ? se->spec->fn : nullptr, se->arith_relaxed));
            timer.stop();
            se->spp_done = done;
            se->n_launches++;
            se->passes_launched += fused;
            left -= fused;
        };
        if (se->sched_trial == 1 && blocking && left >= 4 && total - se->spp_done >= 4 * se->cfg.spp_per_pass) {
            se->sched_trial = 2;
            auto timed = [&](double& ms_per_sample, double& shaded_per_closest) {
                HIP_CHECK(hipStreamSynchronize(se->ctx->stream));
                akr_pt_stats a, b;
                read_stats(se, &a);
                launch(2);
                read_stats(se, &b);
                ms_per_sample = (b.kernel_ms - a.kernel_ms) / (double)std::max<uint64_t>(1, b.n_samples - a.n_samples);
                shaded_per_closest = (double)(b.n_shaded - a.n_shaded) / (double)std::max<uint64_t>(1, b.n_closest - a.n_closest);
            };
            double mk = 0.0, wf = 0.0, ratio = 0.0, unused = 0.0;
            timed(mk, ratio);
            char msg[200];
            if (ratio >= 0.97 && tuning().sched_trial != 1) {
                std::snprintf(msg, sizeof msg, "megakernel (no trial of the other schedule: %.3f shaded vertices per closest-hit ray, a closed scene)", ratio);
            } else {
                se->wf = wf_allocate(se, false);
                timed(wf, unused);
                const bool keep = wf < 0.95 * mk;
                std::snprintf(msg, sizeof msg, keep ? "wavefront schedule (timed trial, 2 passes each: %.3g ns per sample against the megakernel's %.3g)"
                                                    : "megakernel (timed trial, 2 passes each: %.3g ns per sample against the other schedule's %.3g)",
                              (keep ? wf : mk) * 1e6, (keep ? mk : wf) * 1e6);
                if (!keep) se->wf.reset();
            }
            se->spec_status = msg;
        }
        while (left > 0 && se->spp_done < total) launch(kMaxFusedPasses);
        if (blocking) HIP_CHECK(hipStreamSynchronize(se->ctx->stream));
        if (spp_done) *spp_done = se->spp_done;
    });
}
AKR_API int32_t akr_pt_set_active_tiles(akr_pt_session* se, const uint32_t* tiles, uint32_t n) {
    if (!se) return fail(AKR_ERR_INVALID_ARGUMENT, "akr_pt_set_active_tiles: session is NULL");
    return guarded([&] {
        se->ctx->bind();
        PtParams& p = se->params;
        const akr_pt_config& c = se->cfg;
        const uint32_t n_tiles = se->grid.tiles_x * se->grid.tiles_y, tile_px = se->grid.tile_w * se->grid.tile_h;
        const uint32_t count = c.shard_count > 1 ? c.shard_count : 1, rank = c.shard_count > 1 ? c.shard_rank : 0;
        if (tiles) {
            std::vector<uint8_t> seen(n_tiles, 0);
            for (uint32_t j = 0; j < n; j++) {
                const uint32_t t = tiles[j];
                if (t >= n_tiles) throw std::invalid_argument("akr_pt_set_active_tiles: tile " + std::to_string(t) + " is out of range (the grid has " + std::to_string(n_tiles) + " tiles)");
                if (tile_owner(t % se->grid.tiles_x, t / se->grid.tiles_x, count) != rank)
                    throw std::invalid_argument("akr_pt_set_active_tiles: tile " + std::to_string(t) + " is not owned by this session (shard " + std::to_string(rank) + " of " + std::to_string(count) + ")");
                if (seen[t]) throw std::invalid_argument("akr_pt_set_active_tiles: duplicate tile " + std::to_string(t));
                seen[t] = 1;
            }
        }
        HIP_CHECK(hipStreamSynchronize(se->ctx->stream));
        se->sched_trial = se->sched_trial == 1 ? 0 : se->sched_trial;
        if (!tiles) {
            se->active_set = false;
            p.shard_count = count;
            p.owned_tiles = se->owned_tiles.as<uint32_t>();
            p.n_items = se->grid.n_items;
        } else {
            if (!se->active_tiles.p) se->active_tiles.alloc((size_t)std::max(1u, n_tiles) * sizeof(uint32_t));
            if (n) HIP_CHECK(hipMemcpy(se->active_tiles.p, tiles, (size_t)n * sizeof(uint32_t), hipMemcpyHostToDevice));
            se->active_set = true;
            p.shard_count = std::max(2u, count);
            p.owned_tiles = se->active_tiles.as<uint32_t>();
            p.n_items = n * tile_px;
        }
        if (se->wf) wf_set_range(*se->wf, p.n_items);
    });
}
AKR_API int32_t akr_pt_read_sampler_states(akr_pt_session* se, uint64_t* dst) {
    if (!se || !dst) return fail(AKR_ERR_INVALID_ARGUMENT, "akr_pt_read_sampler_states: NULL argument");
    return guarded([&] {
        se->ctx->bind();
        HIP_CHECK(hipStreamSynchronize(se->ctx->stream));
        HIP_CHECK(hipMemcpy(dst, se->states.p, se->states.bytes, hipMemcpyDeviceToHost));
    });
}
static std::array<uint64_t, 8> read_counters(RenderBase* se) {
    se->ctx->bind();
    HIP_CHECK(hipStreamSynchronize(se->ctx->stream));
    std::vector<uint64_t> stripes(8 * kStatStripes);
    HIP_CHECK(hipMemcpy(stripes.data(), se->counters.p, stripes.size() * sizeof(uint64_t), hipMemcpyDeviceToHost));
    std::array<uint64_t, 8> c{};
    for (uint32_t k = 0; k < kStatStripes; k++)
        for (int i = 0; i < 8; i++) c[i] += stripes[8 * k + i];
    return c;
}
static void read_stats(RenderBase* se, akr_pt_stats* stats) {
    const std::array<uint64_t, 8> c = read_counters(se);
    se->fold_events(true);
    const double ms = se->kernel_ms;
    if (stats) {
        stats->n_samples = c[0];
        stats->n_closest = c[1];
        stats->n_shadow = c[2];
        stats->n_shaded = c[3];
        stats->n_node_visits = c[4];
        stats->n_tri_tests = c[5];
        stats->kernel_ms = ms;
        stats->n_launches = se->n_launches;
        stats->_pad = (uint32_t)c[6];
    }
    if (c[6] != 0) throw RenderError("BVH traversal stack overflow: the render is incomplete");
}
AKR_API int32_t akr_pt_get_stats(akr_pt_session* se, akr_pt_stats* stats) {
    if (!se || !stats) return fail(AKR_ERR_INVALID_ARGUMENT, "akr_pt_get_stats: NULL argument");
    return guarded([&] { read_stats(se, stats); });
}
AKR_API int32_t akr_pt_kernel_info(akr_pt_session* se, akr_kernel_info* info) {
    if (!se || !info) return fail(AKR_ERR_INVALID_ARGUMENT, "akr_pt_kernel_info: NULL argument");
    if (info->struct_size < sizeof(akr_kernel_info)) return fail(AKR_ERR_INVALID_ARGUMENT, "akr_pt_kernel_info: struct_size is smaller than this library's akr_kernel_info (set it to sizeof)");
    return guarded([&] {
        const uint32_t size = info->struct_size;
        std::memset(info, 0, sizeof *info);
        info->struct_size = size;
        info->specialised = se->spec_active ? 1u : 0u;
        info->n_shader_kinds = (uint32_t)se->scene->cs.shader_kinds.size();
        const PtVariant& v = se->variant;
        info->kernel_flags = (v.bvh && !v.inst ? 1u : 0u) | (v.pmj ? 2u : 0u) | (v.stage ? 4u : 0u) | (v.defer ? 8u : 0u) | (se->arith_relaxed ? 16u : 0u) | (v.lens ? 32u : 0u) | (v.feat ? 64u : 0u);
        info->absent_mask = se->scene->cs.absent;
        if (se->spec) {
            info->cache_hit = se->spec->cache_hit ? 1u : 0u;
            info->min_waves = (uint32_t)se->spec_waves;
            info->vgprs = (uint32_t)se->spec->vgprs;
            info->scratch_bytes = (uint32_t)se->spec->scratch_bytes;
            info->compile_ms = se->spec->compile_ms;
            info->load_ms = se->spec->load_ms;
        }
        std::snprintf(info->status, sizeof info->status, "%s", se->spec_status.c_str());
        if (se->wf && se->wf->buf.carry != nullptr && se->counters.p) {
            const uint64_t carried = read_counters(se)[7];
            std::snprintf(info->status, sizeof info->status, "%s; %llu rays carried into a later trace launch", se->spec_status.c_str(), (unsigned long long)carried);
        }
    });
}
AKR_API int32_t akr_pt_end(akr_pt_session* se, akr_pt_stats* stats) { return base_end(se, stats); }
AKR_API int32_t akr_pt_render(akr_context* ctx, akr_scene* scene, const akr_pt_config* cfg, akr_film* film, akr_pt_stats* stats) {
    akr_pt_session* se = nullptr;
    int32_t rc = akr_pt_begin(ctx, scene, cfg, film, &se);
    if (rc != AKR_OK) return rc;
    uint32_t n_passes = (session_samples(*cfg) + cfg->spp_per_pass - 1) / cfg->spp_per_pass;
    rc = akr_pt_passes(se, n_passes, 1, nullptr);
    return end_keeping_first_error(rc, [&] { return akr_pt_end(se, stats); });
}
AKR_API int32_t akr_pt_render_features(akr_context* ctx, akr_scene* scene, const akr_pt_config* cfg, akr_film* film, akr_film* albedo, akr_film* normal, akr_pt_stats* stats) {
    akr_pt_session* se = nullptr;
    int32_t rc = akr_pt_begin_features(ctx, scene, cfg, film, albedo, normal, &se);
    if (rc != AKR_OK) return rc;
    uint32_t n_passes = (session_samples(*cfg) + cfg->spp_per_pass - 1) / cfg->spp_per_pass;
    rc = akr_pt_passes(se, n_passes, 1, nullptr);
    return end_keeping_first_error(rc, [&] { return akr_pt_end(se, stats); });
}

}
int32_t akr_api::base_end(RenderBase* se, akr_pt_stats* stats) {
    if (!se) return AKR_OK;
    int32_t rc = guarded([&] { read_stats(se, stats); });
    (void)hipSetDevice(se->ctx->device);
    delete se;
    return rc;
}
```

akari_render_amd/csrc/host/scene_build.cpp:

```cpp
#include "scene_build.h"
#include "../device/dinst.h"
#include "host_parallel.h"

#include <chrono>
#include <cstdio>
#include <mutex>
#include <cmath>
#include <cstdlib>
#include <cstring>
#include <deque>
#include <stdexcept>

#include "../device/dgeom.h"

namespace akr {

FlatScene FlatScene::from_desc(const akr_scene_desc& d) {
    FlatScene s;
    if ((d.n_meshes && !d.meshes) || (d.n_instances && !d.instances) || (d.n_materials && !d.materials))
        throw std::invalid_argument("akr_scene_desc: null array with non-zero count");
    s.meshes.resize(d.n_meshes);
    for (uint32_t i = 0; i < d.n_meshes; i++) {
        const akr_mesh_desc& m = d.meshes[i];
        if (!m.vertices || !m.indices || m.n_triangles == 0) throw std::invalid_argument("akr_mesh_desc: empty mesh");
// ... 678 lines not shown
                    for (int a = 0; a < 3; a++) {
                        const float extra = pad_scale * tri_cond_extra(k[a], mag, pad / pad_scale);
                        if (extra > 0.0f) {
                            bb[a] -= extra;
                            bb[3 + a] += extra;
                        }
                    }
                }
            });
        }
        std::vector<float>().swap(tri_cond);
        std::vector<uint32_t> order;
        const bool force_balanced = tune.bvh_balanced != 0;
        build_bvh8(bounds, n_tris, pad, kBvhNodeWords, force_balanced, order, out.bvh_nodes, out.bvh_depth);
        if (out.bvh_depth > kBvhStackDepth) build_bvh8(bounds, n_tris, pad, kBvhNodeWords, true, order, out.bvh_nodes, out.bvh_depth);
        if (out.bvh_depth > kBvhStackDepth)
            throw std::runtime_error("unsupported: BVH depth " + std::to_string(out.bvh_depth) + " exceeds the traversal stack (" +
                                     std::to_string(kBvhStackDepth) + " levels)");
        phase.lap("BVH build");
        std::vector<float> rec((size_t)kBvhTriWords * n_tris, 0.0f);
        {
            const unsigned nc = n_tris > (1u << 17) ? host_threads() * 4 : 1;
            parallel_chunks(nc, host_threads(), [&](unsigned c) {
                const uint32_t lo = (uint32_t)((uint64_t)n_tris * c / nc), hi = (uint32_t)((uint64_t)n_tris * (c + 1) / nc);
                for (uint32_t k = lo; k < hi; k++) {
                    std::memcpy(&rec[(size_t)kBvhTriWords * k], &out.woop[12ull * order[k]], 48);
                    rec[(size_t)kBvhTriWords * k + 12] = u2f(order[k]);
                }
            });
        }
        out.woop.swap(rec);
        out.tri_gid = order;
        phase.lap("records in traversal order");
    }
    out.woop.resize(out.woop.size() + 32, 0.0f);
}

namespace {
std::mutex g_tuning_mutex;
bool g_tuning_init = false;
TuningOptions g_tuning;
void tuning_init_locked() {
    if (g_tuning_init) return;
    g_tuning_init = true;
    auto flag = [](const char* name) { const char* e = std::getenv(name); return e && e[0] == '1' ? 1 : 0; };
    g_tuning.force_bvh = flag("AKR_FORCE_BVH");
    g_tuning.bvh_balanced = flag("AKR_BVH_BALANCED");
    if (const char* e = std::getenv("AKR_PT_DEFER_METAL")) g_tuning.defer_metal = std::atoi(e);
    if (const char* e = std::getenv("AKR_PT_MODE")) g_tuning.wavefront = std::string(e) == "wavefront" ? 1 : (std::string(e) == "auto" ? -1 : 0);
    if (const char* e = std::getenv("AKR_PT_SIMPLE")) g_tuning.simple_kernels = std::atoi(e) != 0 ? 1 : 0;
    if (const char* e = std::getenv("AKR_SPECIALISE")) g_tuning.specialise = std::atoi(e);
    if (const char* e = std::getenv("AKR_SPECIALISE_WAVES")) g_tuning.specialise_waves = std::atoi(e);
    if (const char* e = std::getenv("AKR_WF_SORT")) g_tuning.wf_sort = std::atoi(e) != 0 ? 1 : 0;
    if (const char* e = std::getenv("AKR_LENS")) g_tuning.lens = std::atoi(e) != 0 ? 1 : 0;
    if (const char* e = std::getenv("AKR_INSTANCING")) g_tuning.instancing = std::atoi(e);
    if (const char* e = std::getenv("AKR_WF_GROUPS")) g_tuning.wf_groups = std::max(0, std::min(32, std::atoi(e)));
    if (const char* e = std::getenv("AKR_WF_CARRY")) g_tuning.wf_carry = std::max(0, std::min(1 << 30, std::atoi(e)));
    if (const char* e = std::getenv("AKR_SCHED_TRIAL")) g_tuning.sched_trial = std::max(-1, std::min(1, std::atoi(e)));
    if (const char* e = std::getenv("AKR_REBRAID")) g_tuning.rebraid = std::max(1, std::min(64, std::atoi(e)));
    if (const char* e = std::getenv("AKR_ARITH")) g_tuning.arith = std::atoi(e) != 0 ? 1 : 0;
    if (const char* e = std::getenv("AKR_DENOISE")) g_tuning.denoise = std::max(0, std::min(65536, std::atoi(e)));
    if (const char* e = std::getenv("AKR_DENOISE_VARIANCE")) g_tuning.denoise_variance = std::atoi(e) != 0 ? 1 : 0;
    if (const char* e = std::getenv("AKR_DENOISE_FEATURES")) g_tuning.denoise_features = std::atoi(e) != 0 ? 1 : 0;
    if (const char* e = std::getenv("AKR_DENOISE_KERNEL")) g_tuning.denoise_kernel = std::max(-1, std::min(1, std::atoi(e)));
    if (const char* e = std::getenv("AKR_ADAPTIVE")) g_tuning.adaptive = std::max(0, std::min(1 << 20, std::atoi(e)));
    if (const char* e = std::getenv("AKR_DISPLAY")) g_tuning.display = std::max(0, std::min(4, std::atoi(e)));
    if (const char* e = std::getenv("AKR_DISPLAY_AUTO_EXPOSURE")) g_tuning.display_auto_exposure = std::atoi(e) != 0 ? 1 : 0;
    if (const char* e = std::getenv("AKR_DISPLAY_EXPOSURE")) g_tuning.display_exposure = std::max(-65536, std::min(65536, std::atoi(e)));
    if (const char* e = std::getenv("AKR_DISPLAY_BLOOM")) g_tuning.display_bloom = std::max(0, std::min(65536, std::atoi(e)));
    if (const char* e = std::getenv("AKR_DISPLAY_KERNEL")) g_tuning.display_kernel = std::max(-1, std::min(1, std::atoi(e)));
    if (const char* e = std::getenv("AKR_ADAPTIVE_MIN_SPP")) g_tuning.adaptive_min_spp = std::max(0, std::min(65536, std::atoi(e)));
}
int* tuning_field(const char* name) {
    const std::string n = name ? name : "";
    if (n == "force_bvh") return &g_tuning.force_bvh;
    if (n == "bvh_balanced") return &g_tuning.bvh_balanced;
    if (n == "defer_metal") return &g_tuning.defer_metal;
    if (n == "wavefront") return &g_tuning.wavefront;
    if (n == "simple_kernels") return &g_tuning.simple_kernels;
    if (n == "defer_on") return &g_tuning.defer_on;
    if (n == "specialise") return &g_tuning.specialise;
    if (n == "specialise_waves") return &g_tuning.specialise_waves;
    if (n == "max_fused_passes") return &g_tuning.max_fused_passes;
    if (n == "wf_sort") return &g_tuning.wf_sort;
    if (n == "lens") return &g_tuning.lens;
    if (n == "instancing") return &g_tuning.instancing;
    if (n == "arith") return &g_tuning.arith;
    if (n == "rebraid") return &g_tuning.rebraid;
    if (n == "wf_groups") return &g_tuning.wf_groups;
    if (n == "wf_carry") return &g_tuning.wf_carry;
    if (n == "sched_trial") return &g_tuning.sched_trial;
    if (n == "pad_percent") return &g_tuning.pad_percent;
    if (n == "denoise") return &g_tuning.denoise;
    if (n == "denoise_variance") return &g_tuning.denoise_variance;
    if (n == "denoise_features") return &g_tuning.denoise_features;
    if (n == "denoise_kernel") return &g_tuning.denoise_kernel;
    if (n == "adaptive") return &g_tuning.adaptive;
    if (n == "adaptive_min_spp") return &g_tuning.adaptive_min_spp;
    if (n == "display") return &g_tuning.display;
    if (n == "display_auto_exposure") return &g_tuning.display_auto_exposure;
    if (n == "display_exposure") return &g_tuning.display_exposure;
    if (n == "display_bloom") return &g_tuning.display_bloom;
    if (n == "display_kernel") return &g_tuning.display_kernel;
    return nullptr;
}
}
TuningOptions tuning() {
    std::lock_guard<std::mutex> lock(g_tuning_mutex);
    tuning_init_locked();
    return g_tuning;
}
bool tuning_set(const char* name, int value) {
    std::lock_guard<std::mutex> lock(g_tuning_mutex);
    tuning_init_locked();
    int* f = tuning_field(name);
    if (!f) return false;
    if (f == &g_tuning.defer_on && (value < 0 || value > 3)) return false;
    if (f == &g_tuning.specialise && (value < -1 || value > 1)) return false;
    if (f == &g_tuning.specialise_waves && value != 0 && (value < 2 || value > 4)) return false;
    if (f == &g_tuning.max_fused_passes && (value < 0 || value > 64)) return false;
    if (f == &g_tuning.wf_sort && (value < 0 || value > 1)) return false;
    if (f == &g_tuning.lens && (value < 0 || value > 1)) return false;
    if (f == &g_tuning.instancing && (value < -1 || value > 1)) return false;
    if (f == &g_tuning.arith && (value < 0 || value > 1)) return false;
    if (f == &g_tuning.rebraid && (value < 1 || value > 64)) return false;
    if (f == &g_tuning.wf_groups && (value < 0 || value > 32)) return false;
    if (f == &g_tuning.wf_carry && (value < 0 || value > (1 << 30))) return false;
    if (f == &g_tuning.sched_trial && (value < -1 || value > 1)) return false;
    if (f == &g_tuning.wavefront && (value < -1 || value > 1)) return false;
    if (f == &g_tuning.pad_percent && (value < 1 || value > 10000)) return false;
    if (f == &g_tuning.denoise && (value < 0 || value > 65536)) return false;
    if (f == &g_tuning.denoise_variance && (value < 0 || value > 1)) return false;
    if (f == &g_tuning.denoise_features && (value < 0 || value > 1)) return false;
    if (f == &g_tuning.denoise_kernel && (value < -1 || value > 1)) return false;
    if (f == &g_tuning.adaptive && (value < 0 || value > (1 << 20))) return false;
    if (f == &g_tuning.adaptive_min_spp && (value < 0 || value > 65536)) return false;
    if (f == &g_tuning.display && (value < 0 || value > 4)) return false;
    if (f == &g_tuning.display_auto_exposure && (value < 0 || value > 1)) return false;
    if (f == &g_tuning.display_exposure && (value < -65536 || value > 65536)) return false;
    if (f == &g_tuning.display_bloom && (value < 0 || value > 65536)) return false;
    if (f == &g_tuning.display_kernel && (value < -1 || value > 1)) return false;
    *f = value;
    return true;
}
bool tuning_get(const char* name, int* value) {
    std::lock_guard<std::mutex> lock(g_tuning_mutex);
    tuning_init_locked();
    int* f = tuning_field(name);
    if (!f) return false;
    *value = *f;
    return true;
}

}
```

akari_render_amd/csrc/host/scene_build.h:

```cpp
#pragma once
#include <cmath>
#include <stdint.h>

#include <string>
#include <vector>

#include "../../../include/akari_hip.h"
#include "../kernels.h"

namespace akr {

struct HostMesh {
    std::vector<float> vertices;
    std::vector<uint32_t> indices;
    std::vector<float> uvs;
    std::vector<float> normals;
    std::vector<float> tangents;
    std::vector<uint32_t> slots;
    uint32_t n_triangles() const { return (uint32_t)(indices.size() / 3); }
};
struct HostInstance {
    uint32_t mesh = 0;
    std::vector<uint32_t> materials;
    float transform[16];
// ... 63 lines not shown
    uint32_t tex_slots = 0;
    std::vector<akr_shader_node> tex_nodes_ssa;
    struct ShaderKind {
        std::string signature;
        uint32_t mat_kind = 0, n_nodes = 0;
        std::vector<uint32_t> materials;
    };
    std::vector<ShaderKind> shader_kinds;
    uint32_t absent = 0;
    struct Instanced {
        bool on = false;
        std::vector<uint32_t> nodes;
        std::vector<float> tlas_leaves;
        std::vector<float> mesh_tris;
        std::vector<uint32_t> mesh_pos;
        std::vector<uint32_t> mesh_meta;
        std::vector<float> mesh_normals;
        std::vector<uint32_t> inst_mats;
        std::vector<uint32_t> inst_light;
        uint32_t tlas_nodes = 0, tlas_depth = 0, blas_depth = 0, n_mesh_tris = 0;
        uint32_t n_padding_classes = 0;
    } instanced;
    struct Environment {
        bool on = false;
        uint32_t w = 0, h = 0, filter = 0;
        std::vector<float> texels;
        std::vector<AliasEntry> marginal_entries, conditional_entries;
        std::vector<float> marginal_pdf, conditional_pdf;
        float rot_t[9] = {1, 0, 0, 0, 1, 0, 0, 0, 1};
        float power = 0.0f;
    } env;
    bool has_textures = false;
    bool has_alpha = false;
    bool needs_ggx_table = false;
    float scene_lo[3], scene_hi[3];
    bool has_tree() const { return !bvh_nodes.empty() || instanced.on; }
};

inline float bvh_box_padding(const float lo[3], const float hi[3], const float* c2w ) {
    float diag2 = 0.0f, reach = 0.0f;
    for (int a = 0; a < 3; a++) {
        diag2 += (hi[a] - lo[a]) * (hi[a] - lo[a]);
        const float m = std::fabs(lo[a]) > std::fabs(hi[a]) ? std::fabs(lo[a]) : std::fabs(hi[a]);
        const float c = std::fabs(c2w[12 + a]);
        reach += m > c ? m : c;
    }
    const float diag = __builtin_sqrtf(diag2);
    return 4e-6f * (diag > reach ? diag : reach);
}
inline void lens_origin_bound(const float* c2w , float radius, float out[3]) {
    const double w = std::fabs((double)c2w[15]) > 0.0 ? std::fabs((double)c2w[15]) : 1.0;
    for (int a = 0; a < 3; a++)
        out[a] = (float)(((double)std::fabs(c2w[12 + a]) + (double)radius * std::sqrt((double)c2w[a] * c2w[a] + (double)c2w[4 + a] * c2w[4 + a])) / w * 1.000001);
}

constexpr float kTriCondEps = 10.0f * 5.9604645e-8f;
constexpr float kTriCondFree = 0.64f;
inline void tri_conditioning(const double A[3], const double B[3], const double C[3], float k[3]) {
    const double e1[3] = {B[0] - A[0], B[1] - A[1], B[2] - A[2]}, e2[3] = {C[0] - A[0], C[1] - A[1], C[2] - A[2]};
    const double n[3] = {e1[1] * e2[2] - e1[2] * e2[1], e1[2] * e2[0] - e1[0] * e2[2], e1[0] * e2[1] - e1[1] * e2[0]};
    const double nl = std::sqrt(n[0] * n[0] + n[1] * n[1] + n[2] * n[2]);
    const double l1 = std::sqrt(e1[0] * e1[0] + e1[1] * e1[1] + e1[2] * e1[2]), l2 = std::sqrt(e2[0] * e2[0] + e2[1] * e2[1] + e2[2] * e2[2]);
    for (int a = 0; a < 3; a++) {
        const double v = nl > 0.0 ? (l2 * std::fabs(e1[a]) + l1 * std::fabs(e2[a])) / nl : 0.0;
        k[a] = v < 1e30 ? (float)(v * 1.0001) : 1e30f;
    }
}
inline float tri_cond_extra(float k, float magnitude, float pad) {
    const float need = kTriCondEps * magnitude * k, have = kTriCondFree * pad;
    return need > have ? need - have : 0.0f;
}
inline float box_magnitude(const float lo[3], const float hi[3]) {
    float m2 = 0.0f;
    for (int a = 0; a < 3; a++) {
        const float m = std::fabs(lo[a]) > std::fabs(hi[a]) ? std::fabs(lo[a]) : std::fabs(hi[a]);
        m2 += m * m;
    }
    return __builtin_sqrtf(m2) * 1.0001f;
}
DMaterial fold_material(const akr_material_desc& m, uint32_t color = 0);
void compile_materials(const FlatScene& flat, uint32_t color, CompiledScene& out, std::vector<akr_material_desc>& descs);
void build_alias_table(const std::vector<float>& weights, std::vector<AliasEntry>& entries, std::vector<float>& pdf);
struct TuningOptions {
    int force_bvh = 0, bvh_balanced = 0, defer_metal = -1, wavefront = -1, simple_kernels = 1;
    int defer_on = 0;
    int specialise = -1, specialise_waves = 0;
    int max_fused_passes = 0;
    int instancing = -1;
    int rebraid = 1;
    int arith = 0;
    int pad_percent = 100;
    int wf_groups = 0;
    int wf_carry = 1;
    int sched_trial = -1;
    int lens = 0;
    int denoise = 0;
    int denoise_variance = 0;
    int denoise_features = 0;
    int denoise_kernel = -1;
    int adaptive = 0;
    int adaptive_min_spp = 0;
    int display = 0;
    int display_auto_exposure = 0, display_exposure = 0, display_bloom = 0;
    int display_kernel = -1;
    int wf_sort = 0;
};
constexpr uint64_t kSpecAutoSamples = 1ull << 31;
TuningOptions tuning();
bool tuning_set(const char* name, int value);
bool tuning_get(const char* name, int* value);

void compile_scene(const FlatScene& flat, CompiledScene& out);
constexpr uint32_t kEnvConstW = 32, kEnvConstH = 16;
void compile_environment(const FlatScene& flat, CompiledScene& out);
HostEnvironment environment_from_desc(const akr_environment_desc& d);
float triangle_emission_power(const CompiledScene& out, const TexScene& host_tex, uint32_t material, uint32_t prim, vec2 uv0, vec2 uv1, vec2 uv2, float area);
bool instance_may_emit(const CompiledScene& out, const std::vector<akr_material_desc>& descs, const HostInstance& in);
bool want_instancing(const FlatScene& flat);
struct InstXf;
void compile_instanced_geometry(const FlatScene& flat, const std::vector<InstXf>& xf, const std::vector<akr_material_desc>& descs, CompiledScene& out);
void camera_matrices(const akr_camera_desc& cam, float r2c[16], float c2w[16], uint32_t* c2w_identity);
PcgStartConsts pcg_start_constants();

FlatScene load_scene_json(const std::string& path);
void parse_method_json(const std::string& text, akr_pt_config* cfg, std::string* film_out);
constexpr size_t kStageMaxBytes = 32 * 1024;
constexpr size_t kStageMaxBytesBvh = 12 * 1024;

struct ParsedTask {
    bool is_aov = false;
    akr_pt_config cfg;
    akr_aov_config aov;
    bool is_gpt = false;
    akr_gpt_config gpt;
    bool is_mcmc = false;
    akr_mcmc_config mcmc;
    std::string film_out;
};
std::vector<ParsedTask> parse_render_tasks(const std::string& text, bool allow_sampler_override);
void make_pmj02_sets(std::vector<uint32_t>& out);
void load_bluenoise(std::vector<uint16_t>& out);
void write_image(const std::string& path, const float* rgb, uint32_t w, uint32_t h);
void decode_png(const uint8_t* data, size_t n, uint32_t& w, uint32_t& h, std::vector<uint8_t>& rgba);
void decode_jpeg(const uint8_t* data, size_t n, uint32_t& w, uint32_t& h, std::vector<uint8_t>& rgba);
void decode_exr(const uint8_t* data, size_t n, uint32_t& w, uint32_t& h, std::vector<float>& rgba);
void decode_tiff(const uint8_t* data, size_t n, uint32_t& w, uint32_t& h, std::vector<uint8_t>& rgba);
void decode_dds(const uint8_t* data, size_t n, uint32_t& w, uint32_t& h, std::vector<uint8_t>& rgba);
std::vector<uint8_t> inflate_zlib_stream(const uint8_t* data, size_t n);

}
```

akari_render_amd/csrc/kernels.h:

```cpp
#pragma once
#if !defined(__HIPCC_RTC__)
#include <hip/hip_runtime.h>
#endif

#include "device/drng.h"
#include "device/dscene.h"

#if !defined(__HIPCC_RTC__)
#include <algorithm>
struct PtVariant {
    bool bvh, fd, tex, pmj, stage, defer, simple, inst, env, lens;
    bool feat;
};
constexpr bool pt_variant_compiled(const PtVariant& v) {
    return (v.bvh || v.stage) && !(v.defer && (v.fd || (v.bvh && !v.tex))) && !(v.simple && (v.fd || v.tex)) && !((v.env || v.lens || v.feat) && (v.defer || v.simple)) &&
           !(v.inst && !(v.bvh && !v.stage && !v.defer && !v.simple && !v.feat));
}
constexpr uint32_t pt_variant_bits(const PtVariant& v) {
    return (v.bvh ? 1u : 0u) | (v.pmj ? 2u : 0u) | (v.stage ? 4u : 0u) | (v.defer ? 8u : 0u) | (v.inst ? 16u : 0u) | (v.env ? 32u : 0u) | (v.lens ? 64u : 0u) |
           (v.feat ? 128u : 0u);
}
constexpr PtVariant pt_variant_from_bits(uint32_t f) {
    return PtVariant{(f & 1u) != 0, false, true, (f & 2u) != 0, (f & 4u) != 0, (f & 8u) != 0, false, (f & 16u) != 0, (f & 32u) != 0, (f & 64u) != 0, (f & 128u) != 0};
}
// ... 24 lines not shown
constexpr uint32_t kParkSlotsFeat = 19;
enum : uint32_t { CY_BEST_T = 0, CY_BEST_U, CY_BEST_V, CY_BEST, CY_G, CY_T, CY_TBASE, CY_SP, CY_PHASE, CY_HIT_T, CY_HIT_U, CY_HIT_V, CY_HIT_GID, CY_END,
                  CY_LEAF = CY_END, CY_PEND_REC, CY_PEND_INST, CY_END_INST };
constexpr uint32_t kCarrySlots = CY_END, kCarrySlotsInstanced = CY_END_INST;
constexpr size_t kBlueNoiseColumnBytes = 48 * 256 * 2;
#if !defined(__HIPCC_RTC__)
inline size_t pt_lds_budget(bool tex) { return (tex ? 53 : 40) * 1024; }
inline PtLdsLayout pt_lds_layout(const PtVariant& v, const PtLdsSizes& s, bool plan_larger_park = false) {
    PtLdsLayout L{};
    const size_t slots = v.tex ? (size_t)s.tex_slots * kTexValStride * sizeof(TexVal) : 0;
    const int stragglers = v.inst ? AKR_PT_STRAGGLERS_INST : (v.tex ? AKR_PT_STRAGGLERS_TEX : AKR_PT_STRAGGLERS);
    const size_t park = (!v.fd && v.tex) ? (size_t)(v.feat ? kParkSlotsFeat : (v.defer || plan_larger_park ? kParkSlots : kParkSlotsNoDefer)) * 256 * 4 : 0;
    const size_t carry = (v.bvh && stragglers > 0) ? (size_t)(v.inst ? kCarrySlotsInstanced : kCarrySlots) * 256 * 4 : 0;
    auto align = [](size_t b) { return (b + 15) & ~(size_t)15; };
    size_t base = v.bvh ? (size_t)s.stack_depth * 256 * 4 : 0;
    L.stage_offset = (uint32_t)(base / 4);
    base += s.stage_bytes;
    L.recs_offset = (uint32_t)(base / 4);
    base = align(base + (!v.bvh ? (size_t)(s.n_tris + 2) * 48 : 0));
    L.required_bytes = align(base + park + carry) + slots;
    L.tile_offset = (uint32_t)(base / 4);
    if (v.bvh && !v.tex && !v.inst) {
        const size_t other = base + park + carry + slots, budget = pt_lds_budget(v.tex) - 256;
        if (other < budget) L.tile_nodes = (uint32_t)std::min<size_t>({(budget - other) / (kBvhNodeWords * 4), (size_t)s.n_nodes, (size_t)1024});
        base = align(base + (size_t)L.tile_nodes * kBvhNodeWords * 4);
    }
    L.park_offset = (uint32_t)(base / 4);
    base += park;
    L.carry_offset = (uint32_t)(base / 4);
    base += carry;
    if (s.bluenoise && !v.bvh && base + slots + kBlueNoiseColumnBytes <= pt_lds_budget(v.tex)) {
        L.bn_offset = (uint32_t)(align(base) / 4);
        base = align(base) + kBlueNoiseColumnBytes;
    }
    L.val_offset_words = (uint32_t)((base = align(base)) / 4);
    L.total_bytes = base + slots;
    return L;
}
#endif

constexpr uint32_t kStatStripes = 256;
struct PtParams {
    DScene sc;
    float r2c[16];
    float c2w[16];
    uint32_t c2w_identity;
    uint32_t width, height;
    uint32_t max_depth, rr_depth, use_nee, indirect_only, force_diffuse;
    int32_t debug_depth;
    int32_t pixel_offset[2];
    uint32_t filter_type;
    float filter_radius;
    uint32_t color;
    uint32_t pass_spp;
    uint32_t n_passes;
    uint32_t last_pass_spp;
    PcgStartConsts start;
    Pcg32* states;
    float* film;
    uint64_t* counters;
    uint32_t sampler;
    uint32_t smp_seed, smp_spp, smp_w;
    uint64_t smp_mod_magic;
    const uint32_t* pmj_sets;
    const uint16_t* bluenoise;
    uint32_t stage_bytes[13];
    uint32_t stage_total;
    uint32_t simple_scene;
    uint32_t defer_metal;
    uint32_t defer_flags;
    uint32_t tex_slots;
    uint32_t tile_offset;
    uint32_t park_offset;
    uint32_t carry_offset;
    uint32_t bn_offset;
    uint32_t wf_sort;
    float sort_lo[3], sort_scale[3];
    uint32_t n_items;
    uint32_t shard_rank, shard_count;
    uint32_t tile_w, tile_h, tiles_x, tiles_y;
    const uint32_t* owned_tiles;
    float lens_radius, lens_focal;
    float *feat_albedo, *feat_normal;
};

AKR_HD uint32_t morton_spread16(uint32_t x) {
    x &= 0xffffu;
    x = (x | (x << 8)) & 0x00ff00ffu;
    x = (x | (x << 4)) & 0x0f0f0f0fu;
    x = (x | (x << 2)) & 0x33333333u;
    x = (x | (x << 1)) & 0x55555555u;
    return x;
}
AKR_HD uint32_t tile_morton(uint32_t tx, uint32_t ty) { return morton_spread16(tx) | (morton_spread16(ty) << 1); }
AKR_HD uint32_t tile_owner(uint32_t tx, uint32_t ty, uint32_t count) { return tile_morton(tx, ty) % count; }

struct WfBuffers {
    float4 *ray_o, *ray_d;
    float4 *sh_o, *sh_d, *sh_c;
    float4* hit;
    float4 *beta, *rad, *base;
    float4* film;
    uint4 *rng, *misc;
    uint32_t* queue_closest[2];
    uint32_t* queue_shadow[2];
    uint32_t* key_closest[2];
    uint32_t* key_shadow[2];
    uint32_t* qcount;
    uint32_t* qhead;
    uint32_t* n_active;
    uint32_t* pend;
    uint32_t* carry;
    uint32_t carry_words, n_slots;
    uint32_t carry_queue;
    uint32_t carry_lanes, carry_steps;
    uint32_t slot_base, slot_end;
};

struct GptParams {
    float* own;
    float* shifted[4];
    float *acc_p, *acc_gx, *acc_gy, *sqr_p, *sqr_gx, *sqr_gy;
    uint32_t reconnect, stride, separate_weights, reconstruction;
    const uint32_t* item_pixels;
    uint32_t shard_rank, shard_count, tile_w, tile_h, tiles_x;
};

struct PssSample {
    float cur, backup;
    uint32_t last_modified, modified_backup;
};
struct MarkovState {
    uint32_t cur_pixel[2], chain_id;
    float cur_f, b;
    uint32_t b_cnt, n_accepted, n_mutations, cur_iter, last_large_iter;
};
struct McmcParams {
    PssSample* pss;
    MarkovState* states;
    float4* cur_colors;
    Pcg32* rngs;
    const Pcg32* seeds;
    float* fs;
    const uint32_t* resampled;
    float* film;
    uint32_t n_chains, n_bootstrap, dim, width, height;
    uint32_t chain_begin, chain_count;
    uint32_t exponential_mutation;
    float small_sigma, large_step_prob, image_mutation_prob, image_mutation_size;
};
#if !defined(__HIPCC_RTC__)
hipError_t launch_mcmc_bootstrap(const PtParams& p, const McmcParams& m, hipStream_t stream);
hipError_t launch_mcmc_init(const PtParams& p, const McmcParams& m, hipStream_t stream);
hipError_t launch_mcmc_advance(const PtParams& p, const McmcParams& m, uint32_t mutations_per_chain, float contribution, hipStream_t stream);
#endif

#if !defined(__HIPCC_RTC__)
inline PtLdsSizes pt_lds_sizes(const PtParams& p) {
    return PtLdsSizes{p.sc.bvh_stack_depth, p.sc.n_tris, p.sc.n_nodes, p.tex_slots, p.stage_total, p.sampler == 1u && p.bluenoise != nullptr};
}
inline PtParams pt_params_with_layout(const PtParams& p, const PtLdsLayout& L) {
    PtParams q = p;
    q.tile_offset = L.tile_offset; q.sc.bvh_tile_nodes = L.tile_nodes; q.park_offset = L.park_offset; q.carry_offset = L.carry_offset;
    q.bn_offset = L.bn_offset; q.sc.tex.val_offset_words = L.val_offset_words;
    return q;
}
#endif
inline PtParams with_tex_slots(const PtParams& p, size_t base_bytes, size_t& lds_bytes) {
    PtParams q = p;
    base_bytes = (base_bytes + 15) & ~(size_t)15;
    q.sc.tex.val_offset_words = (uint32_t)(base_bytes / 4);
    lds_bytes = base_bytes + (p.sc.tex.nodes != nullptr ? (size_t)p.tex_slots * kTexValStride * sizeof(TexVal) : 0);
    return q;
}
#if !defined(__HIPCC_RTC__)
hipError_t launch_inst_share_bits(const DScene& sc, uint32_t* bits, uint32_t* mesh_tri_words, hipStream_t stream);
hipError_t launch_probe_env(const PtParams& p, uint32_t mode, uint32_t n, const float* in, float* out, hipStream_t stream);
hipError_t launch_probe_camera_rays(const PtParams& p, uint32_t n, const uint32_t* pixels2, const float* u4, float* out6, hipStream_t stream);
hipError_t launch_pt_pass(const PtParams& p, const PtVariant& v, hipStream_t stream, hipFunction_t spec_fn = nullptr, bool relaxed = false);
hipError_t launch_gpt_sample(const PtParams& p, const GptParams& g, hipStream_t stream);
hipError_t launch_gpt_update(const GptParams& g, uint32_t W, uint32_t H, float* film, hipStream_t stream);
hipError_t launch_gpt_recon_init(const GptParams& g, uint32_t W, uint32_t H, float* old, float spp, hipStream_t stream);
hipError_t launch_gpt_recon(const GptParams& g, uint32_t W, uint32_t H, const float* old, float* cur, float scaling, float spp, hipStream_t stream);
hipError_t launch_aov(const PtParams& p, uint32_t spp, uint32_t aov, uint32_t remap, hipStream_t stream);
hipError_t launch_wf_init(const PtParams& p, const WfBuffers& wf, hipStream_t stream);
hipError_t launch_wf_shade(const PtParams& p, const WfBuffers& wf, uint32_t q_out, hipStream_t stream);
uint32_t wf_trace_blocks_per_cu(const PtParams& p);
hipError_t launch_wf_trace(const PtParams& p, const WfBuffers& wf, uint32_t q_in, uint32_t n_blocks, hipStream_t stream);
size_t wf_sort_temp_bytes(uint32_t n);
hipError_t wf_sort_pairs(void* temp, size_t temp_bytes, const uint32_t* keys_in, uint32_t* keys_out, const uint32_t* vals_in, uint32_t* vals_out, uint32_t n, hipStream_t stream);
hipError_t launch_probe_material(const PtParams& p, uint32_t material, uint32_t n, const float* uv, uint32_t* out, hipStream_t stream);
hipError_t launch_init_pcg32(const uint64_t* seeds, void* states, uint64_t n, hipStream_t stream);
hipError_t launch_film_resolve(const float* film, uint64_t n, float splat_scale, float* rgb, hipStream_t stream);
hipError_t launch_ggx_table(const uint64_t* seeds, float* table, uint32_t samples, hipStream_t stream);
hipError_t launch_probe_math(uint32_t n, const float* x, float* s, float* c, float* l, hipStream_t stream);
hipError_t launch_probe_math2(uint32_t n, const float* xy, float* out, hipStream_t stream);
hipError_t launch_probe_bsdf(const DMaterial* m, const float* table, int mode, const float* wo, uint32_t n, const float* in, float* out,
                             hipStream_t stream);
hipError_t launch_probe_div(uint32_t n, const float* a, const float* b, float* out_fast, float* out_ieee, hipStream_t stream);
hipError_t launch_probe_pcg_end_pass(uint32_t n, const uint64_t* state, const uint64_t* inc, const uint32_t* dim, uint64_t* out_closed, uint64_t* out_loop, hipStream_t stream);
hipError_t launch_probe_intersect_pair(const PtParams& p, uint32_t n, const float* rays, const uint32_t* excl, uint32_t* out, float* out_tuv, hipStream_t stream);
hipError_t launch_probe_intersect(const PtParams& p, uint32_t n, const float* rays, uint32_t* out, float* bary, hipStream_t stream);
hipError_t launch_probe_si(const PtParams& p, uint32_t n, const uint32_t* inst_prim, const float* bary, float* out, hipStream_t stream);
#endif

}
```

akari_render_amd/csrc/launch.h:

```cpp
#pragma once
#include <hip/hip_runtime.h>
#include <type_traits>

namespace akr {

template <class F>
void dispatch_bools(F&& f) { f(); }
template <class F, class... Bs>
void dispatch_bools(F&& f, bool b0, Bs... rest) {
    if (b0) dispatch_bools([&](auto... c) { f(std::true_type{}, c...); }, rest...);
    else dispatch_bools([&](auto... c) { f(std::false_type{}, c...); }, rest...);
}

template <bool BIG_LDS = false, class... P, class... A>
void launch_kernel(void (*kernel)(P...), uint32_t blocks, size_t lds, hipStream_t stream, const A&... args) {
    if (BIG_LDS && lds > 64 * 1024) (void)hipFuncSetAttribute((const void*)kernel, hipFuncAttributeMaxDynamicSharedMemorySize, (int)lds);
    hipLaunchKernelGGL(kernel, dim3(blocks), dim3(256), lds, stream, args...);
}

}
```

akari_render_amd/csrc/pt_env_kernels.hip:

```cpp
#include "pt_launch.h"

namespace akr {

hipError_t pt_pass_entry_env(const PtParams& q, const PtVariant& v, uint32_t blocks, size_t lds, hipStream_t stream) { return pt_pass_entry_t<true, false>(q, v, blocks, lds, stream); }

__global__ void k_probe_env(const DEnv* __restrict__ env_p, uint32_t color, uint32_t mode, uint32_t n, const float* __restrict__ in, float* __restrict__ out) {
    const uint32_t i = blockIdx.x * blockDim.x + threadIdx.x;
    if (i >= n) return;
    const DEnv& env = *env_p;
    if (mode == 0) {
        vec3 wi;
        float pdf;
        const bool ok = env_sample(env, mk2(in[2 * (size_t)i], in[2 * (size_t)i + 1]), wi, pdf);
        float* o = out + 5 * (size_t)i;
        o[0] = wi.x; o[1] = wi.y; o[2] = wi.z; o[3] = pdf; o[4] = ok ? 1.0f : 0.0f;
    } else {
        const vec3 d = mk3(in[3 * (size_t)i], in[3 * (size_t)i + 1], in[3 * (size_t)i + 2]);
        const vec3 le = env_eval(env, color, d);
        float* o = out + 4 * (size_t)i;
        o[0] = env_pdf(env, d); o[1] = le.x; o[2] = le.y; o[3] = le.z;
    }
}
hipError_t launch_probe_env(const PtParams& p, uint32_t mode, uint32_t n, const float* in, float* out, hipStream_t stream) {
    if (!p.sc.env || mode > 1) return hipErrorInvalidValue;
    if (n == 0) return hipSuccess;
    hipLaunchKernelGGL(k_probe_env, dim3((n + 255) / 256), dim3(256), 0, stream, p.sc.env, p.color, mode, n, in, out);
    return hipGetLastError();
}

}
```

akari_render_amd/csrc/pt_feat_env_kernels.hip:

```cpp
#include "pt_launch.h"

namespace akr {

hipError_t pt_pass_entry_feat_env(const PtParams& q, const PtVariant& v, uint32_t blocks, size_t lds, hipStream_t stream) { return pt_pass_entry_t<true, false, true>(q, v, blocks, lds, stream); }

}
```

akari_render_amd/csrc/pt_feat_kernels.hip:

```cpp
#include "pt_launch.h"

namespace akr {

hipError_t pt_pass_entry_feat(const PtParams& q, const PtVariant& v, uint32_t blocks, size_t lds, hipStream_t stream) { return pt_pass_entry_t<false, false, true>(q, v, blocks, lds, stream); }

}
```

akari_render_amd/csrc/pt_feat_lens_env_kernels.hip:

```cpp
#include "pt_launch.h"

namespace akr {

hipError_t pt_pass_entry_feat_lens_env(const PtParams& q, const PtVariant& v, uint32_t blocks, size_t lds, hipStream_t stream) { return pt_pass_entry_t<true, true, true>(q, v, blocks, lds, stream); }

}
```

akari_render_amd/csrc/pt_feat_lens_kernels.hip:

```cpp
#include "pt_launch.h"

namespace akr {

hipError_t pt_pass_entry_feat_lens(const PtParams& q, const PtVariant& v, uint32_t blocks, size_t lds, hipStream_t stream) { return pt_pass_entry_t<false, true, true>(q, v, blocks, lds, stream); }

}
```

akari_render_amd/csrc/pt_inst_env_kernels.hip:

```cpp
#include "pt_inst_kernel.h"

namespace akr {

hipError_t pt_pass_entry_inst_env(const PtParams& q, const PtVariant& v, uint32_t blocks, size_t lds, hipStream_t stream) { return pt_pass_entry_inst_t<true, false>(q, v, blocks, lds, stream); }

}
```

akari_render_amd/csrc/pt_inst_kernel.h:

```cpp
#pragma once
#include "pt_launch.h"

#ifndef AKR_PT_MIN_WAVES_INST
#define AKR_PT_MIN_WAVES_INST AKR_PT_MIN_WAVES_BVH
#endif
#ifndef AKR_PT_MIN_WAVES_INST_TEX
#define AKR_PT_MIN_WAVES_INST_TEX AKR_PT_MIN_WAVES_BVH_TEX
#endif

namespace akr {

template <bool FD, bool TEX, bool PMJ, bool ENV = false, bool LENS = false>
__global__ __launch_bounds__(256, TEX ? AKR_PT_MIN_WAVES_INST_TEX : AKR_PT_MIN_WAVES_INST) void k_pt_pass_inst(const PtParams p) {
    pt_pass_body<true, FD, TEX, PMJ, false, false, 0u, true, ENV, LENS>(p);
}

template <bool ENV, bool LENS>
hipError_t pt_pass_entry_inst_t(const PtParams& q, const PtVariant& v, uint32_t blocks, size_t lds, hipStream_t stream) {
    if (!v.inst || v.env != ENV || v.lens != LENS || !pt_variant_compiled(v)) return hipErrorInvalidValue;
    dispatch_bools([&](auto F, auto T, auto P) { launch_kernel<true>(k_pt_pass_inst<F(), T(), P(), ENV, LENS>, blocks, lds, stream, q); }, v.fd, v.tex, v.pmj);
    return hipGetLastError();
}

}
```

akari_render_amd/csrc/pt_inst_kernels.hip:

```cpp
#include "pt_inst_kernel.h"

namespace akr {

__global__ __launch_bounds__(256) void k_inst_share_bits(const DScene sc, uint32_t* __restrict__ bits, uint32_t* __restrict__ mesh_tri_words) {
    const uint32_t n_inst = sc.in2.n_instances;
    for (uint64_t gid = (uint64_t)blockIdx.x * 256u + threadIdx.x; gid < sc.n_tris; gid += (uint64_t)gridDim.x * 256u) {
        uint32_t lo = 0, hi = n_inst;
        while (hi - lo > 1u) {
            const uint32_t mid = lo + (hi - lo) / 2u;
            if (sc.inst_tri_offset[mid] <= gid) lo = mid; else hi = mid;
        }
        const uint32_t prim = (uint32_t)gid - sc.inst_tri_offset[lo];
        uint32_t pos;
        if ((prim & 1u) && inst_pair_shares(sc, lo, prim, pos)) {
            atomicOr(&bits[gid >> 5], 1u << ((uint32_t)gid & 31u));
            atomicOr(&mesh_tri_words[16ull * pos + 15u], kMeshTriShares);
        }
    }
}
hipError_t launch_inst_share_bits(const DScene& sc, uint32_t* bits, uint32_t* mesh_tri_words, hipStream_t stream) {
    if (sc.n_tris == 0 || sc.in2.n_instances == 0) return hipSuccess;
    const uint64_t blocks = ((uint64_t)sc.n_tris + 255u) / 256u;
    hipLaunchKernelGGL(k_inst_share_bits, dim3((uint32_t)(blocks < (1u << 20) ? blocks : (1u << 20))), dim3(256), 0, stream, sc, bits, mesh_tri_words);
    return hipGetLastError();
}

hipError_t pt_pass_entry_inst(const PtParams& q, const PtVariant& v, uint32_t blocks, size_t lds, hipStream_t stream) { return pt_pass_entry_inst_t<false, false>(q, v, blocks, lds, stream); }

}
```

akari_render_amd/csrc/pt_inst_lens_kernels.hip:

```cpp
#include "pt_inst_kernel.h"

namespace akr {

hipError_t pt_pass_entry_inst_lens_env(const PtParams& q, const PtVariant& v, uint32_t blocks, size_t lds, hipStream_t stream) { return pt_pass_entry_inst_t<true, true>(q, v, blocks, lds, stream); }
hipError_t pt_pass_entry_inst_lens(const PtParams& q, const PtVariant& v, uint32_t blocks, size_t lds, hipStream_t stream) { return pt_pass_entry_inst_t<false, true>(q, v, blocks, lds, stream); }

}
```

akari_render_amd/csrc/pt_kernels.hip:

```cpp
#include <algorithm>
#include "device/pt_pass.h"
#include "pt_launch.h"

namespace akr {

__global__ void k_init_pcg32(const uint64_t* __restrict__ seeds, Pcg32* __restrict__ states, uint64_t n) {
    uint64_t i = (uint64_t)blockIdx.x * blockDim.x + threadIdx.x;
    if (i < n) states[i] = pcg_new_seq_offset(i, seeds[i]);
}

__global__ void k_film_resolve(const float* __restrict__ film, uint64_t n, float splat_scale, float* __restrict__ rgb) {
    uint64_t i = (uint64_t)blockIdx.x * blockDim.x + threadIdx.x;
    if (i >= n) return;
    float w = film[6 * n + i];
    float inv = w == 0.0f ? 1.0f : w;
#pragma unroll
    for (int c = 0; c < 3; c++) rgb[3 * i + c] = film[3 * i + c] / inv + film[3 * n + 3 * i + c] * splat_scale;
}

__global__ void k_ggx_dielectric_table(const uint64_t* __restrict__ seeds, float* __restrict__ table, uint32_t samples) {
    const uint32_t dim = 16;
    uint32_t gid = blockIdx.x * blockDim.x + threadIdx.x;
    if (gid >= dim * dim * dim) return;
    uint32_t tx = gid % dim, ty = (gid / dim) % dim, tz = gid / (dim * dim);
// ... 83 lines not shown
        o[6] = s.pdf;
        o[7] = s.valid ? 1.0f : 0.0f;
    }
}
template <bool BVH, bool INST = false>
__global__ __launch_bounds__(256) void k_probe_intersect(PtParams p, uint32_t n, const float* __restrict__ rays, uint32_t* __restrict__ out, float* __restrict__ bary) {
    extern __shared__ __attribute__((aligned(16))) uint32_t lds_stack[];
    TraceCtx tc;
    tc.stack = lds_stack + threadIdx.x;
    tc.cnt = TraceCounters{0, 0, 0};
    uint32_t i = blockIdx.x * blockDim.x + threadIdx.x;
    bool act = i < n;
    const float* r = rays + 8 * (size_t)(act ? i : 0);
    Hit h;
    bool found = INST ? trace_inst<false, false>(p.sc, mk3(r[0], r[1], r[2]), mk3(r[3], r[4], r[5]), r[6], r[7], kInvalid, kInvalid, h, tc.stack, tc.cnt)
                      : trace<BVH, false>(p, tc, mk3(r[0], r[1], r[2]), mk3(r[3], r[4], r[5]), r[6], r[7], kInvalid, kInvalid, h);
    if (!act) return;
    uint32_t inst = 0, prim = 0;
    if (found) {
        inst = INST ? inst_of_gid(p.sc, h.gid) : f2u(p.sc.shade[(size_t)h.gid * SHADE_ROWS + 6].z);
        prim = h.gid - p.sc.inst_tri_offset[inst];
    }
    out[3 * i + 0] = found ? 1u : 0u;
    out[3 * i + 1] = inst;
    out[3 * i + 2] = prim;
    bary[2 * i + 0] = found ? h.u : 0.0f;
    bary[2 * i + 1] = found ? h.v : 0.0f;
}
__global__ __launch_bounds__(256) void k_probe_intersect_pair(PtParams p, uint32_t n, const float* __restrict__ rays, const uint32_t* __restrict__ excl, uint32_t* __restrict__ out,
                                                              float* __restrict__ out_tuv) {
    extern __shared__ __attribute__((aligned(16))) uint32_t lds_stack[];
    const uint32_t* g = (const uint32_t*)p.sc.woop;
    for (uint32_t i = threadIdx.x; i < (p.sc.n_tris + 2u) * 12u; i += 256u) lds_stack[i] = g[i];
    __syncthreads();
    const uint32_t i = blockIdx.x * blockDim.x + threadIdx.x;
    const bool act = i < n;
    const float* r = rays + 16 * (size_t)(act ? i : 0);
    const uint32_t* e = excl + 3 * (size_t)(act ? i : 0);
    Hit h;
    bool found = false, occluded = false;
    uint32_t redo = 0;
    trace_pair_exhaustive<false>(p.sc, mk3(r[0], r[1], r[2]), mk3(r[3], r[4], r[5]), act ? r[6] : -1.0f, e[0], mk3(r[8], r[9], r[10]), mk3(r[11], r[12], r[13]),
                                 act ? r[14] : -1.0f, e[1], e[2], h, found, occluded, (const float4*)lds_stack, &redo);
    if (!act) return;
    out[4 * i + 0] = found ? 1u : 0u;
    out[4 * i + 1] = h.gid;
    out[4 * i + 2] = occluded ? 1u : 0u;
    out[4 * i + 3] = redo;
    out_tuv[3 * i + 0] = h.t;
    out_tuv[3 * i + 1] = h.u;
    out_tuv[3 * i + 2] = h.v;
}
template <bool INST>
__global__ void k_probe_si(PtParams p, uint32_t n, const uint32_t* __restrict__ inst_prim, const float* __restrict__ bary, float* __restrict__ out) {
    uint32_t i = blockIdx.x * blockDim.x + threadIdx.x;
    if (i >= n) return;
    uint32_t gid = p.sc.inst_tri_offset[inst_prim[2 * i]] + inst_prim[2 * i + 1];
    SurfacePoint s = surface_interaction_any<INST>(p.sc, gid, mk2(bary[2 * i], bary[2 * i + 1]));
    float* o = out + 19 * (size_t)i;
    o[0] = s.p.x; o[1] = s.p.y; o[2] = s.p.z;
    o[3] = s.ng.x; o[4] = s.ng.y; o[5] = s.ng.z;
    o[6] = s.frame.n.x; o[7] = s.frame.n.y; o[8] = s.frame.n.z;
    o[9] = s.frame.t.x; o[10] = s.frame.t.y; o[11] = s.frame.t.z;
    o[12] = s.frame.s.x; o[13] = s.frame.s.y; o[14] = s.frame.s.z;
    o[15] = s.uv.x;
    o[16] = s.uv.y;
    o[17] = s.prim_area;
    o[18] = (float)s.material;
}

__global__ void k_probe_material(PtParams p, uint32_t material, uint32_t n, const float* __restrict__ uv, uint32_t* __restrict__ out) {
    uint32_t i = blockIdx.x * blockDim.x + threadIdx.x;
    if (i >= n) return;
    const DMaterial& m = p.sc.materials[material];
    MatInputs in = p.sc.tex.mat_inputs[material];
    if (m.flags & MF_TEXTURED) {
        eval_material_graph(p.sc.tex, m.tex_first_node, m.tex_n_nodes & kTexCountMask, mk2(uv[2 * i], uv[2 * i + 1]), in);
    }
    const uint32_t* w = reinterpret_cast<const uint32_t*>(&in);
    for (uint32_t k = 0; k < 26; k++) out[26 * (size_t)i + k] = w[k];
}

}
extern "C" hipError_t akr_launch_pt_pass_relaxed(const void* params, const PtVariant* v, uint32_t blocks, size_t lds, hipStream_t stream);
namespace akr {
static hipError_t pt_pass_entry_plain(const PtParams& q, const PtVariant& v, uint32_t blocks, size_t lds, hipStream_t stream) { return pt_pass_entry_t<false, false>(q, v, blocks, lds, stream); }
static constexpr PtPassEntry kPtPassEntry[2][2][2] = {{{pt_pass_entry_plain, pt_pass_entry_lens}, {pt_pass_entry_env, pt_pass_entry_lens_env}},
                                                      {{pt_pass_entry_inst, pt_pass_entry_inst_lens}, {pt_pass_entry_inst_env, pt_pass_entry_inst_lens_env}}};
static constexpr PtPassEntry kPtPassEntryFeat[2][2] = {{pt_pass_entry_feat, pt_pass_entry_feat_lens}, {pt_pass_entry_feat_env, pt_pass_entry_feat_lens_env}};
hipError_t launch_pt_pass(const PtParams& p, const PtVariant& v, hipStream_t stream, hipFunction_t spec_fn, bool relaxed) {
    const uint32_t blocks = (p.n_items + 255u) / 256u;
    if (blocks == 0) return hipSuccess;
    const PtLdsLayout L = pt_lds_layout(v, pt_lds_sizes(p));
    const PtParams q = pt_params_with_layout(p, L);
    if (v.feat) {
        if (spec_fn || relaxed || v.inst) return hipErrorInvalidValue;
        return kPtPassEntryFeat[v.env][v.lens](q, v, blocks, L.total_bytes, stream);
    }
    if (spec_fn) {
        if (L.total_bytes > 64 * 1024) (void)hipFuncSetAttribute((const void*)spec_fn, hipFuncAttributeMaxDynamicSharedMemorySize, (int)L.total_bytes);
        void* args[] = {(void*)&q};
        return hipModuleLaunchKernel(spec_fn, blocks, 1, 1, 256, 1, 1, (unsigned)L.total_bytes, stream, args, nullptr);
    }
    if (relaxed) return akr_launch_pt_pass_relaxed(&q, &v, blocks, L.total_bytes, stream);
    return kPtPassEntry[v.inst][v.env][v.lens](q, v, blocks, L.total_bytes, stream);
}
hipError_t launch_probe_material(const PtParams& p, uint32_t material, uint32_t n, const float* uv, uint32_t* out, hipStream_t stream) {
    size_t lds;
    const PtParams q = with_tex_slots(p, 0, lds);
    hipLaunchKernelGGL(k_probe_material, dim3((n + 127) / 128), dim3(128), lds, stream, q, material, n, uv, out);
    return hipGetLastError();
}
hipError_t launch_init_pcg32(const uint64_t* seeds, void* states, uint64_t n, hipStream_t stream) {
    uint32_t blocks = (uint32_t)((n + 255) / 256);
    if (blocks == 0) return hipSuccess;
    hipLaunchKernelGGL(k_init_pcg32, dim3(blocks), dim3(256), 0, stream, seeds, (Pcg32*)states, n);
    return hipGetLastError();
}
hipError_t launch_film_resolve(const float* film, uint64_t n, float splat_scale, float* rgb, hipStream_t stream) {
    uint32_t blocks = (uint32_t)((n + 255) / 256);
    if (blocks == 0) return hipSuccess;
    hipLaunchKernelGGL(k_film_resolve, dim3(blocks), dim3(256), 0, stream, film, n, splat_scale, rgb);
    return hipGetLastError();
}
hipError_t launch_ggx_table(const uint64_t* seeds, float* table, uint32_t samples, hipStream_t stream) {
    hipLaunchKernelGGL(k_ggx_dielectric_table, dim3(64), dim3(64), 0, stream, seeds, table, samples);
    return hipGetLastError();
}
hipError_t launch_probe_math(uint32_t n, const float* x, float* s, float* c, float* l, hipStream_t stream) {
    hipLaunchKernelGGL(k_probe_math, dim3((n + 255) / 256), dim3(256), 0, stream, n, x, s, c, l);
    return hipGetLastError();
}
hipError_t launch_probe_math2(uint32_t n, const float* xy, float* out, hipStream_t stream) {
    hipLaunchKernelGGL(k_probe_math2, dim3((n + 255) / 256), dim3(256), 0, stream, n, xy, out);
    return hipGetLastError();
}
hipError_t launch_probe_div(uint32_t n, const float* a, const float* b, float* out_fast, float* out_ieee, hipStream_t stream) {
    hipLaunchKernelGGL(k_probe_div, dim3((n + 255) / 256), dim3(256), 0, stream, n, a, b, out_fast, out_ieee);
    return hipGetLastError();
}
hipError_t launch_probe_pcg_end_pass(uint32_t n, const uint64_t* state, const uint64_t* inc, const uint32_t* dim, uint64_t* out_closed, uint64_t* out_loop, hipStream_t stream) {
    hipLaunchKernelGGL(k_probe_pcg_end_pass, dim3((n + 255) / 256), dim3(256), 0, stream, n, state, inc, dim, out_closed, out_loop);
    return hipGetLastError();
}
hipError_t launch_probe_intersect_pair(const PtParams& p, uint32_t n, const float* rays, const uint32_t* excl, uint32_t* out, float* out_tuv, hipStream_t stream) {
    launch_kernel(k_probe_intersect_pair, (n + 255) / 256, (p.sc.n_tris + 2u) * 48u, stream, p, n, rays, excl, out, out_tuv);
    return hipGetLastError();
}
hipError_t launch_probe_bsdf(const DMaterial* m, const float* table, int mode, const float* wo, uint32_t n, const float* in, float* out,
                             hipStream_t stream) {
    hipLaunchKernelGGL(k_probe_bsdf, dim3((n + 255) / 256), dim3(256), 0, stream, m, table, mode, mk3(wo[0], wo[1], wo[2]), n, in, out);
    return hipGetLastError();
}
hipError_t launch_probe_intersect(const PtParams& p, uint32_t n, const float* rays, uint32_t* out, float* bary, hipStream_t stream) {
    const bool bvh = p.sc.bvh_nodes != nullptr, inst = p.sc.in2.on != 0;
    dispatch_bools([&](auto B, auto I) {
        launch_kernel(k_probe_intersect<B() || I(), I()>, (n + 255) / 256, B() || I() ? p.sc.bvh_stack_depth * 256 * 4 : 0, stream, p, n, rays, out, bary);
    }, bvh, inst);
    return hipGetLastError();
}
hipError_t launch_probe_si(const PtParams& p, uint32_t n, const uint32_t* inst_prim, const float* bary, float* out, hipStream_t stream) {
    dispatch_bools([&](auto I) { launch_kernel(k_probe_si<I()>, (n + 255) / 256, 0, stream, p, n, inst_prim, bary, out); }, p.sc.in2.on != 0);
    return hipGetLastError();
}

}
```

akari_render_amd/csrc/pt_kernels_relaxed.hip:

```cpp
#include <hip/hip_runtime.h>
#include <stdint.h>
#include <algorithm>

#define AKR_ARITH_RELAXED 1
#define akr akr_rx
#include "pt_launch.h"
#undef akr

extern "C" hipError_t akr_launch_pt_pass_relaxed(const void* params, const PtVariant* v, uint32_t blocks, size_t lds, hipStream_t stream) {
    return akr_rx::pt_pass_entry_t<false, false>(*static_cast<const akr_rx::PtParams*>(params), *v, blocks, lds, stream);
}
```

akari_render_amd/csrc/pt_launch.h:

```cpp
#pragma once
#include "device/pt_pass.h"
#include "launch.h"

namespace akr {

template <bool BVH, bool FD, bool TEX, bool PMJ, bool STAGE, bool DEFER, bool SIMPLE = false, bool ENV = false, bool LENS = false, bool FEAT = false>
__global__ __launch_bounds__(256, pt_pass_min_waves(BVH, FD, TEX)) void k_pt_pass(const PtParams p) {
    pt_pass_body<BVH, FD, TEX, PMJ, STAGE, DEFER, SIMPLE ? AB_SIMPLE : 0u, false, ENV, LENS, FEAT>(p);
}

using PtPassEntry = hipError_t (*)(const PtParams& q, const PtVariant& v, uint32_t blocks, size_t lds, hipStream_t stream);
hipError_t pt_pass_entry_env(const PtParams& q, const PtVariant& v, uint32_t blocks, size_t lds, hipStream_t stream);
hipError_t pt_pass_entry_lens(const PtParams& q, const PtVariant& v, uint32_t blocks, size_t lds, hipStream_t stream);
hipError_t pt_pass_entry_lens_env(const PtParams& q, const PtVariant& v, uint32_t blocks, size_t lds, hipStream_t stream);
hipError_t pt_pass_entry_feat(const PtParams& q, const PtVariant& v, uint32_t blocks, size_t lds, hipStream_t stream);
hipError_t pt_pass_entry_feat_env(const PtParams& q, const PtVariant& v, uint32_t blocks, size_t lds, hipStream_t stream);
hipError_t pt_pass_entry_feat_lens(const PtParams& q, const PtVariant& v, uint32_t blocks, size_t lds, hipStream_t stream);
hipError_t pt_pass_entry_feat_lens_env(const PtParams& q, const PtVariant& v, uint32_t blocks, size_t lds, hipStream_t stream);
hipError_t pt_pass_entry_inst(const PtParams& q, const PtVariant& v, uint32_t blocks, size_t lds, hipStream_t stream);
hipError_t pt_pass_entry_inst_env(const PtParams& q, const PtVariant& v, uint32_t blocks, size_t lds, hipStream_t stream);
hipError_t pt_pass_entry_inst_lens(const PtParams& q, const PtVariant& v, uint32_t blocks, size_t lds, hipStream_t stream);
hipError_t pt_pass_entry_inst_lens_env(const PtParams& q, const PtVariant& v, uint32_t blocks, size_t lds, hipStream_t stream);

template <bool ENV, bool LENS, bool FEAT = false>
hipError_t pt_pass_entry_t(const PtParams& q, const PtVariant& v, uint32_t blocks, size_t lds, hipStream_t stream) {
    if (v.inst || v.env != ENV || v.lens != LENS || v.feat != FEAT || !pt_variant_compiled(v)) return hipErrorInvalidValue;
    if (FEAT && (q.feat_albedo == nullptr || q.feat_normal == nullptr)) return hipErrorInvalidValue;
    dispatch_bools([&](auto B, auto F, auto T, auto P, auto S, auto D, auto X) {
        if constexpr (pt_variant_compiled(PtVariant{B(), F(), T(), P(), S(), D(), X(), false, ENV, LENS, FEAT}))
            launch_kernel<true>(k_pt_pass<B(), F(), T(), P(), S(), D(), X(), ENV, LENS, FEAT>, blocks, lds, stream, q);
    }, v.bvh, v.fd, v.tex, v.pmj, v.stage, v.defer, v.simple);
    return hipGetLastError();
}
}
```

akari_render_amd/csrc/pt_lens_env_kernels.hip:

```cpp
#include "pt_launch.h"

namespace akr {

hipError_t pt_pass_entry_lens_env(const PtParams& q, const PtVariant& v, uint32_t blocks, size_t lds, hipStream_t stream) { return pt_pass_entry_t<true, true>(q, v, blocks, lds, stream); }

}
```

akari_render_amd/csrc/pt_lens_kernels.hip:

```cpp
#include "pt_launch.h"

namespace akr {

hipError_t pt_pass_entry_lens(const PtParams& q, const PtVariant& v, uint32_t blocks, size_t lds, hipStream_t stream) { return pt_pass_entry_t<false, true>(q, v, blocks, lds, stream); }

__global__ void k_probe_camera_rays(const PtParams p, uint32_t n, const uint32_t* __restrict__ pixels, const float* __restrict__ u, float* __restrict__ out) {
    const uint32_t i = blockIdx.x * blockDim.x + threadIdx.x;
    if (i >= n) return;
    const float* ui = u + 4 * (size_t)i;
    vec3 o, d;
    if (p.lens_radius > 0.0f) generate_ray_lens_from(p, pixels[2 * (size_t)i], pixels[2 * (size_t)i + 1], mk2(ui[0], ui[1]), mk2(ui[2], ui[3]), o, d);
    else generate_ray_from(p, pixels[2 * (size_t)i], pixels[2 * (size_t)i + 1], mk2(ui[0], ui[1]), o, d);
    float* r = out + 6 * (size_t)i;
    r[0] = o.x; r[1] = o.y; r[2] = o.z; r[3] = d.x; r[4] = d.y; r[5] = d.z;
}
hipError_t launch_probe_camera_rays(const PtParams& p, uint32_t n, const uint32_t* pixels2, const float* u4, float* out6, hipStream_t stream) {
    if (n == 0) return hipSuccess;
    hipLaunchKernelGGL(k_probe_camera_rays, dim3((n + 255) / 256), dim3(256), 0, stream, p, n, pixels2, u4, out6);
    return hipGetLastError();
}

}
```

include/akari_hip.h:

```cpp
#ifndef AKARI_HIP_H
#define AKARI_HIP_H
#include <stdint.h>

#ifdef __cplusplus
extern "C" {
#endif

#if defined(_WIN32)
#define AKR_API
#else
#define AKR_API __attribute__((visibility("default")))
#endif

typedef enum {
    AKR_OK = 0,
    AKR_ERR_INVALID_ARGUMENT = -1,
    AKR_ERR_HIP = -2,
    AKR_ERR_NO_DEVICE = -3,
    AKR_ERR_IO = -4,
    AKR_ERR_PARSE = -5,
    AKR_ERR_UNSUPPORTED = -6,
    AKR_ERR_OUT_OF_MEMORY = -7,
    AKR_ERR_RENDER = -8
} akr_status;
// ... 52 lines not shown
    AKR_NODE_IMAGE = 3,
    AKR_NODE_MAPPING = 4,
    AKR_NODE_CHECKERBOARD = 5,
    AKR_NODE_SPECTRAL_UPLIFT = 6,
    AKR_NODE_SEPARATE_COLOR = 7,
    AKR_NODE_EXTRACT = 8,
    AKR_NODE_NORMAL_MAP = 9
} akr_node_op;
typedef enum { AKR_MAPPING_POINT = 0, AKR_MAPPING_TEXTURE = 1 } akr_mapping_type;
typedef enum { AKR_FIELD_RED = 0, AKR_FIELD_GREEN = 1, AKR_FIELD_BLUE = 2, AKR_FIELD_UV = 3 } akr_extract_field;
typedef struct {
    uint32_t op;
    uint32_t arg[4];
    float k[3];
} akr_shader_node;

typedef enum {
    AKR_IN_BASE_COLOR = 0, AKR_IN_METALLIC, AKR_IN_ROUGHNESS, AKR_IN_IOR, AKR_IN_SPECULAR_IOR_LEVEL, AKR_IN_SPECULAR_TINT,
    AKR_IN_TRANSMISSION_WEIGHT, AKR_IN_COAT_WEIGHT, AKR_IN_COAT_ROUGHNESS, AKR_IN_COAT_IOR, AKR_IN_COAT_TINT,
    AKR_IN_EMISSION_COLOR, AKR_IN_EMISSION_STRENGTH, AKR_IN_NORMAL, AKR_IN_COUNT
} akr_material_input;
typedef struct {
    uint32_t n_nodes;
    uint32_t _pad;
    const akr_shader_node *nodes;
    uint32_t input[AKR_IN_COUNT];
} akr_material_graph;

typedef enum { AKR_IMAGE_RGBA8 = 0 , AKR_IMAGE_RGBA32F = 1  } akr_image_format;
typedef enum { AKR_TEX_FILTER_NEAREST = 0, AKR_TEX_FILTER_LINEAR = 1 } akr_tex_filter;
typedef enum { AKR_TEX_REPEAT = 0, AKR_TEX_CLIP = 1 , AKR_TEX_MIRROR = 2, AKR_TEX_EXTEND = 3  } akr_tex_address;
typedef struct {
    uint32_t width, height;
    uint32_t format, filter, address, _pad;
    const void *texels;
} akr_image_desc;

typedef struct {
    float c2w[16];
    float fov;
    uint32_t width, height;
} akr_camera_desc;

typedef struct {
    uint32_t n_meshes, n_instances, n_materials, _pad;
    const akr_mesh_desc *meshes;
    const akr_instance_desc *instances;
    const akr_material_desc *materials;
    akr_camera_desc camera;
    const float *ggx_dielectric_table;
    uint32_t n_images, _pad2;
    const akr_image_desc *images;
    const akr_material_graph *material_graphs;
} akr_scene_desc;

typedef enum { AKR_FILTER_BOX = 0, AKR_FILTER_GAUSSIAN = 1 } akr_filter_type;
typedef enum { AKR_SAMPLER_INDEPENDENT = 0, AKR_SAMPLER_PMJ02BN = 1, AKR_SAMPLER_SOBOL = 2 } akr_sampler_type;
typedef enum { AKR_COLOR_REPR_ACESCG = 1, AKR_COLOR_RGB_ACESCG = 2 } akr_color_pipeline_bits;

typedef struct {
    uint32_t spp, max_depth, spp_per_pass, rr_depth;
    uint32_t use_nee, indirect_only, force_diffuse;
    int32_t pixel_offset[2];
    int32_t debug_depth;
    uint32_t filter_type;
    float filter_radius;
    uint32_t sampler_type;
    uint32_t color;
    uint64_t sampler_seed;
    uint32_t shard_rank, shard_count, tile_w, tile_h;
    uint32_t sample_begin, sample_count;
} akr_pt_config;

typedef struct {
    uint64_t n_samples;
    uint64_t n_closest;
    uint64_t n_shadow;
    uint64_t n_shaded;
    uint64_t n_node_visits;
    uint64_t n_tri_tests;
    double kernel_ms;
    uint32_t n_launches;
    uint32_t _pad;
} akr_pt_stats;


AKR_API const char *akr_last_error(void);

AKR_API int32_t akr_context_create(int32_t device, akr_context **out);
AKR_API int32_t akr_context_destroy(akr_context *ctx);
AKR_API int32_t akr_context_synchronize(akr_context *ctx);
AKR_API int32_t akr_device_count(int32_t *count);
AKR_API int32_t akr_context_device_ordinal(akr_context *ctx, int32_t *device);
AKR_API int32_t akr_context_device_info(akr_context *ctx, char *name, uint32_t name_len, uint32_t *compute_units,
                                        uint64_t *hbm_bytes);

AKR_API int32_t akr_scene_create(akr_context *ctx, const akr_scene_desc *desc, akr_scene **out);
AKR_API int32_t akr_scene_load(akr_context *ctx, const char *scene_json_path, uint32_t width, uint32_t height,
                               akr_scene **out);
AKR_API int32_t akr_scene_destroy(akr_scene *scene);
AKR_API int32_t akr_scene_set_resolution(akr_scene *scene, uint32_t width, uint32_t height);

typedef struct {
    uint32_t width, height;
    uint32_t n_instances, n_triangles, n_materials, n_lights;
    uint32_t n_bvh_nodes;
    uint32_t uses_bvh;
    uint64_t device_bytes;
    uint32_t node_bytes;
    uint32_t node_stride_bytes;
    uint32_t tri_bytes;
    uint32_t bvh_depth;
} akr_scene_info;
AKR_API int32_t akr_scene_get_info(const akr_scene *scene, akr_scene_info *info);
AKR_API int32_t akr_scene_get_light(const akr_scene *scene, uint32_t light, uint32_t *instance, float *power, float *pdf);
typedef struct {
    uint32_t width, height;
    uint32_t filter;
    uint32_t _pad;
    const float *texels;
    float color[3];
    float strength;
    float rotation[9];
    uint32_t _pad2;
} akr_environment_desc;
AKR_API int32_t akr_scene_set_environment(akr_scene *scene, const akr_environment_desc *desc);
AKR_API int32_t akr_scene_get_environment(const akr_scene *scene, akr_environment_desc *out);
typedef struct {
    float radius;
    float focal_distance;
} akr_lens_desc;
AKR_API int32_t akr_scene_set_lens(akr_scene *scene, const akr_lens_desc *desc);
AKR_API int32_t akr_scene_get_lens(const akr_scene *scene, akr_lens_desc *out);
AKR_API int32_t akr_scene_get_ggx_table(const akr_scene *scene, float *dst4096);
AKR_API int32_t akr_scene_get_desc_counts(const akr_scene *scene, uint32_t *n_meshes, uint32_t *n_instances, uint32_t *n_materials);
AKR_API int32_t akr_scene_get_mesh(const akr_scene *scene, uint32_t mesh, akr_mesh_desc *out );
AKR_API int32_t akr_scene_get_instance(const akr_scene *scene, uint32_t instance, akr_instance_desc *out);
AKR_API int32_t akr_scene_get_material(const akr_scene *scene, uint32_t material, akr_material_desc *out);
AKR_API int32_t akr_scene_get_camera(const akr_scene *scene, akr_camera_desc *out);
AKR_API int32_t akr_scene_get_image_count(const akr_scene *scene, uint32_t *n_images);
AKR_API int32_t akr_scene_get_image(const akr_scene *scene, uint32_t image, akr_image_desc *out );
AKR_API int32_t akr_scene_get_material_graph(const akr_scene *scene, uint32_t material, akr_material_graph *out );
typedef enum {
    AKR_ARRAY_WOOP = 0,
    AKR_ARRAY_TRI_GID = 1,
    AKR_ARRAY_SHADE = 2,
    AKR_ARRAY_INSTANCES = 3,
    AKR_ARRAY_MATERIALS = 4,
    AKR_ARRAY_BVH_NODES = 5,
    AKR_ARRAY_LIGHT_ENTRIES = 6,
    AKR_ARRAY_LIGHT_PDF = 7,
    AKR_ARRAY_AREA_ENTRIES = 8,
    AKR_ARRAY_AREA_PDF = 9,
    AKR_ARRAY_INST_TRI_OFFSET = 10,
    AKR_ARRAY_R2C = 11,
    AKR_ARRAY_C2W = 12,
    AKR_ARRAY_TEX_NODES = 13,
    AKR_ARRAY_TEX_IMAGES = 14,
    AKR_ARRAY_TEX_TEXELS = 15,
    AKR_ARRAY_MAT_INPUTS = 16,
    AKR_ARRAY_INST_LEAVES = 17,
    AKR_ARRAY_MESH_TRIS = 18,
    AKR_ARRAY_MESH_POS = 19,
    AKR_ARRAY_MESH_META = 20,
    AKR_ARRAY_MESH_NORMALS = 21,
    AKR_ARRAY_ENV_MARGINAL_ENTRIES = 22,
// ... 235 lines not shown
```

Measured before the change: 3469.

## Chain multiple fused-pass chunks into one grid launch with per-group progress words

Replaces a sequence of separate fused-pass kernel launches with a single large grid. Each block decodes a chunk index and a pixel group, and waits on an atomic per-group progress word, so chunks for the same pixels run in order. Blocks that find their predecessor unfinished count themselves as deferred and exit. The host then replays the deferred groups with follow-up launches driven by a sorted group list. This targets launch gaps and tail idle time between passes, at the cost of atomics, fences, an occupancy query, and a host sync plus readback after each chained grid.

```diff
diff --git a/akari_render_amd/abi.py b/akari_render_amd/abi.py
--- a/akari_render_amd/abi.py
+++ b/akari_render_amd/abi.py
@@ -345,10 +345,17 @@
         ("kernel_ms", C.c_double),
         ("n_launches", C.c_uint32),
         ("_pad", C.c_uint32),
+        ("n_chain_deferred", C.c_uint32),
+        ("_pad2", C.c_uint32),
     ]
 
     def as_dict(self):
         return {k: getattr(self, k) for k, _ in self._fields_ if not k.startswith("_")}
+
+
+class PtChainPlan(C.Structure):
+
+    _fields_ = [("chunks", C.c_uint32), ("grid_chunks", C.c_uint32), ("groups", C.c_uint32), ("groups_padded", C.c_uint32), ("last_chunk_passes", C.c_uint32), ("eligible", C.c_uint32)]
 
 
 class AdaptiveStats(C.Structure):
diff --git a/akari_render_amd/capi.py b/akari_render_amd/capi.py
--- a/akari_render_amd/capi.py
+++ b/akari_render_amd/capi.py
@@ -53,6 +53,7 @@
     "akr_host_tile_error", "akr_host_half_bracket", "akr_probe_adapt_times",
     "akr_host_display_transform", "akr_host_luminance_histogram", "akr_probe_display_times",
     "akr_host_pt_features_plan", "akr_host_pcg_end_pass", "akr_probe_pcg_end_pass",
+    "akr_host_pt_chain_plan",
 ]
 
 
@@ -118,6 +119,7 @@
     proto("akr_probe_camera_rays", vp, vp, u32, f32, u32, up, fp, fp)
     proto("akr_host_pt_launch_plan", vp, C.POINTER(abi.PtConfig), i32, i32, i32, i32, C.POINTER(abi.PtLaunchPlan))
     proto("akr_host_pt_features_plan", vp, C.POINTER(abi.PtConfig), i32, i32, i32, i32, i32, i32, i32, C.POINTER(abi.PtFeaturesPlan))
+    proto("akr_host_pt_chain_plan", u32, u32, u32, u32, C.c_double, C.POINTER(abi.PtChainPlan))
     proto("akr_probe_env_sample", vp, vp, u32, fp, fp)
     proto("akr_probe_env_pdf", vp, vp, u32, fp, fp)
     proto("akr_scene_get_ggx_table", vp, fp)
@@ -522,6 +524,12 @@
         return False
 
 
+def host_pt_chain_plan(n_items: int, n_passes: int, max_fused: int, resident: int, per_pass_ms: float = 0.0) -> dict:
+    out = abi.PtChainPlan()
+    check(lib().akr_host_pt_chain_plan(n_items, n_passes, max_fused, resident, float(per_pass_ms), C.byref(out)))
+    return {k: getattr(out, k) for k, _ in abi.PtChainPlan._fields_}
+
+
 def last_error() -> str:
     return lib().akr_last_error().decode("utf-8", "replace")
 
diff --git a/akari_render_amd/csrc/device/pt_pass.h b/akari_render_amd/csrc/device/pt_pass.h
--- a/akari_render_amd/csrc/device/pt_pass.h
+++ b/akari_render_amd/csrc/device/pt_pass.h
@@ -26,6 +26,27 @@
     TraceCtx tc;
     tc.stack = lds_stack + threadIdx.x;
     tc.cnt = TraceCounters{0, 0, 0};
+    uint32_t group = blockIdx.x;
+    if (p.chain_chunks != 0) {
+        const uint32_t chunk = blockIdx.x / p.chain_groups_padded;
+        group = blockIdx.x - chunk * p.chain_groups_padded;
+        if (group >= p.chain_groups) return;
+        if (threadIdx.x == 0) {
+            uint32_t seen = __hip_atomic_load(p.chain_progress + group, __ATOMIC_ACQUIRE, __HIP_MEMORY_SCOPE_AGENT);
+            if (p.chain_test_m != 0 && chunk == p.chain_test_c0 && group % p.chain_test_m == p.chain_test_r) seen = 0xffffffffu;
+            lds_stack[0] = seen;
+        }
+        __syncthreads();
+        const uint32_t seen = (uint32_t)__builtin_amdgcn_readfirstlane((int)lds_stack[0]);
+        __syncthreads();
+        if (seen != chunk) {
+            if (threadIdx.x == 0) atomicAdd(p.chain_deferred, 1u);
+            return;
+        }
+        __builtin_amdgcn_fence(__ATOMIC_ACQUIRE, "agent");
+    } else if (p.chain_group_list != nullptr) {
+        group = p.chain_group_list[blockIdx.x];
+    }
     PtParams staged = p;
     if (STAGE) stage_scene_tables<BVH, TEX, !BVH && !FD && TEX>(p, lds_stack, staged);
     const PtParams& q = STAGE ? staged : p;
@@ -47,7 +68,7 @@
         __syncthreads();
         lds_recs = (const float4*)l;
     }
-    const uint32_t item = blockIdx.x * 256u + threadIdx.x;
+    const uint32_t item = group * 256u + threadIdx.x;
     uint32_t px = 0, py = 0;
     const bool in_frame = item < p.n_items && item_to_pixel(p, item, px, py);
     const uint32_t pix = px + py * p.width;
@@ -173,6 +194,14 @@
             else path_step<FD ? 1 : 0, TEX, PMJ, 0, ABSENT, INST, ENV, LENS, FEAT>(q, r, hit, found, occluded, pix, sx, sy);
         }
     }
+    if (p.chain_chunks != 0) {
+        __builtin_amdgcn_fence(__ATOMIC_RELEASE, "agent");
+        __syncthreads();
+        uint32_t b = blockIdx.x;
+        asm volatile("" : "+s"(b));
+        const uint32_t c = b / p.chain_groups_padded;
+        if (threadIdx.x == 0) __hip_atomic_store(p.chain_progress + (b - c * p.chain_groups_padded), c + 1u, __ATOMIC_RELEASE, __HIP_MEMORY_SCOPE_AGENT);
+    }
     flush_counters(p, r, tc.cnt, BVH);
 }
 
diff --git a/akari_render_amd/csrc/host/api_internal.h b/akari_render_amd/csrc/host/api_internal.h
--- a/akari_render_amd/csrc/host/api_internal.h
+++ b/akari_render_amd/csrc/host/api_internal.h
@@ -194,6 +194,7 @@
     TileGrid grid;
     DevBuf owned_tiles;
     uint32_t spp_done = 0, n_launches = 0;
+    uint32_t n_chain_deferred = 0;
     uint32_t pmj_spp = 1;
     const akr_scene::ColorSet* color_set = nullptr;
     int defer_metal_option = -1;
@@ -252,6 +253,9 @@
     int sched_trial = 0;
     uint64_t passes_launched = 0;
     int max_fused_option = 0;
+    int chain_option = 1, chain_rounds_option = 2, max_chain_ms_option = 20000, chain_test_defer_option = 0;
+    int resident_groups = -1;
+    DevBuf chain_words;
     bool spec_active = false;
     bool arith_relaxed = false;
     int spec_waves = 3;
@@ -291,6 +295,25 @@
 inline void set_launch_passes(RenderBase* se, uint32_t n_passes, uint32_t last_pass_spp) {
     se->params.n_passes = n_passes;
     se->params.last_pass_spp = last_pass_spp;
+}
+struct PtChainPlan {
+    uint32_t chunks, grid_chunks, groups, groups_padded, last_chunk_passes;
+    bool eligible;
+};
+inline PtChainPlan pt_chain_plan(uint32_t n_items, uint32_t n_passes, uint32_t max_fused, uint32_t resident, double per_pass_ms, int chain_passes, int rounds, int max_chain_ms,
+                                 bool last_pass_short = false) {
+    PtChainPlan c{};
+    c.groups = (n_items + 255u) / 256u;
+    c.groups_padded = (c.groups + 7u) & ~7u;
+    if (max_fused == 0 || n_passes == 0 || c.groups == 0) return c;
+    c.chunks = (n_passes + max_fused - 1u) / max_fused;
+    c.last_chunk_passes = n_passes - (c.chunks - 1u) * max_fused;
+    uint64_t cap = per_pass_ms > 0.0 ? (uint64_t)std::min(1e9, (double)max_chain_ms / ((double)max_fused * per_pass_ms)) : std::max(1u, 64u / max_fused);
+    cap = std::min<uint64_t>(cap, 0x7fffffffull / c.groups_padded);
+    const uint32_t equal = (c.last_chunk_passes == max_fused && !last_pass_short) ? c.chunks : c.chunks - 1u;
+    c.grid_chunks = (uint32_t)std::min<uint64_t>(equal, cap);
+    c.eligible = chain_passes != 0 && c.grid_chunks >= 2u && (chain_passes == 2 || (resident > 0 && (uint64_t)c.groups >= (uint64_t)rounds * resident));
+    return c;
 }
 struct PtPlan {
     PtVariant v;
diff --git a/akari_render_amd/csrc/host/api_probe.cpp b/akari_render_amd/csrc/host/api_probe.cpp
--- a/akari_render_amd/csrc/host/api_probe.cpp
+++ b/akari_render_amd/csrc/host/api_probe.cpp
@@ -297,6 +297,16 @@
         out->park_slots_feat = kParkSlotsFeat;
     });
 }
+AKR_TEST_API int32_t akr_host_pt_chain_plan(uint32_t n_items, uint32_t n_passes, uint32_t max_fused, uint32_t resident, double per_pass_ms, akr_pt_chain_plan* out) {
+    if (!out) return fail(AKR_ERR_INVALID_ARGUMENT, "akr_host_pt_chain_plan: NULL argument");
+    if (max_fused == 0 || max_fused > 64) return fail(AKR_ERR_INVALID_ARGUMENT, "akr_host_pt_chain_plan: max_fused must be 1..64");
+    return guarded([&] {
+        const TuningOptions t = tuning();
+        const PtChainPlan c = pt_chain_plan(n_items, n_passes, max_fused, resident, per_pass_ms, t.chain_passes, t.chain_rounds, t.max_chain_ms);
+        out->chunks = c.chunks; out->grid_chunks = c.grid_chunks; out->groups = c.groups; out->groups_padded = c.groups_padded; out->last_chunk_passes = c.last_chunk_passes;
+        out->eligible = c.eligible ? 1u : 0u;
+    });
+}
 AKR_TEST_API int32_t akr_probe_camera_rays(akr_context* ctx, akr_scene* scene, uint32_t filter_type, float filter_radius, uint32_t n, const uint32_t* pixels2,
                                       const float* u4, float* out6) {
     if (!ctx || !scene || !pixels2 || !u4 || !out6) return fail(AKR_ERR_INVALID_ARGUMENT, "akr_probe_camera_rays: NULL argument");
diff --git a/akari_render_amd/csrc/host/api_pt.cpp b/akari_render_amd/csrc/host/api_pt.cpp
--- a/akari_render_amd/csrc/host/api_pt.cpp
+++ b/akari_render_amd/csrc/host/api_pt.cpp
@@ -480,6 +480,10 @@
         {
             const TuningOptions t = tuning();
             se->max_fused_option = t.max_fused_passes;
+            se->chain_option = t.chain_passes;
+            se->chain_rounds_option = t.chain_rounds;
+            se->max_chain_ms_option = t.max_chain_ms;
+            se->chain_test_defer_option = t.chain_test_defer;
             const uint64_t samples = (uint64_t)film->width * film->height * (uint64_t)session_samples(*cfg);
             const bool may_compile = t.specialise == 1 || samples >= kSpecAutoSamples;
             const PtVariant facts = pt_scene_facts(scene, *cfg);
@@ -604,7 +608,89 @@
             }
             se->spec_status = msg;
         }
-        while (left > 0 && se->spp_done < total) launch(kMaxFusedPasses);
+        auto chain = [&]() -> bool {
+            if (!blocking || se->wf || se->chain_option == 0 || se->params.n_items == 0) return false;
+            const uint32_t spp_pass = se->cfg.spp_per_pass;
+            const uint32_t passes = (uint32_t)std::min<uint64_t>(left, ((uint64_t)(total - se->spp_done) + spp_pass - 1) / spp_pass);
+            if (passes <= kMaxFusedPasses) return false;
+            hipFunction_t spec_fn = se->spec_active ? se->spec->fn : nullptr;
+            if (se->resident_groups < 0 && se->chain_option == 1) {
+                int per_cu = 0;
+                HIP_CHECK(launch_pt_pass(se->params, se->variant, se->ctx->stream, spec_fn, se->arith_relaxed, &per_cu));
+                se->resident_groups = std::max(0, per_cu) * se->ctx->props.multiProcessorCount;
+            }
+            const double per_pass_ms = se->pending.empty() && se->passes_launched > 0 && se->kernel_ms > 0.0 ? se->kernel_ms / (double)se->passes_launched : 0.0;
+            const bool last_pass_short = (uint64_t)se->spp_done + (uint64_t)passes * spp_pass > total;
+            const PtChainPlan plan = pt_chain_plan(se->params.n_items, passes, kMaxFusedPasses, (uint32_t)std::max(0, se->resident_groups), per_pass_ms, se->chain_option,
+                                                   se->chain_rounds_option, se->max_chain_ms_option, last_pass_short);
+            if (!plan.eligible) return false;
+            const uint32_t n = plan.grid_chunks, groups = plan.groups;
+            const uint32_t n_fused = n * kMaxFusedPasses;
+            const uint32_t done = se->spp_done + n_fused * spp_pass;
+            auto chunk_passes = [&](uint32_t) { return kMaxFusedPasses; };
+            auto chunk_last_spp = [&](uint32_t) { return spp_pass; };
+            const size_t max_groups = ((size_t)se->grid.n_items + 255u) / 256u;
+            if (!se->chain_words.p) se->chain_words.alloc((1 + 2 * max_groups) * sizeof(uint32_t));
+            uint32_t* const words = se->chain_words.as<uint32_t>();
+            PtParams& p = se->params;
+            struct Restore {
+                PtParams& p;
+                ~Restore() { p.chain_chunks = 0; p.chain_group_list = nullptr; p.chain_list_len = 0; }
+            } restore{p};
+            HIP_CHECK(hipMemsetAsync(words, 0, (1 + (size_t)groups) * sizeof(uint32_t), se->ctx->stream));
+            p.chain_chunks = n; p.chain_groups = groups; p.chain_groups_padded = plan.groups_padded;
+            p.chain_deferred = words; p.chain_progress = words + 1;
+            p.chain_test_m = (uint32_t)se->chain_test_defer_option & 1023u;
+            p.chain_test_r = ((uint32_t)se->chain_test_defer_option >> 10) & 1023u;
+            p.chain_test_c0 = ((uint32_t)se->chain_test_defer_option >> 20) & 1023u;
+            set_launch_passes(se, kMaxFusedPasses, spp_pass);
+            {
+                LaunchTimer timer(se);
+                HIP_CHECK(launch_pt_pass(p, se->variant, se->ctx->stream, spec_fn, se->arith_relaxed));
+                timer.stop();
+            }
+            p.chain_chunks = 0;
+            se->n_launches++;
+            HIP_CHECK(hipStreamSynchronize(se->ctx->stream));
+            uint32_t deferred = 0;
+            HIP_CHECK(hipMemcpy(&deferred, words, sizeof deferred, hipMemcpyDeviceToHost));
+            if (deferred != 0) {
+                std::vector<uint32_t> progress(groups);
+                HIP_CHECK(hipMemcpy(progress.data(), words + 1, (size_t)groups * sizeof(uint32_t), hipMemcpyDeviceToHost));
+                std::vector<uint32_t> list(groups);
+                for (uint32_t g = 0; g < groups; g++) list[g] = g;
+                std::stable_sort(list.begin(), list.end(), [&](uint32_t a, uint32_t b) { return progress[a] < progress[b]; });
+                uint64_t owed = 0;
+                for (uint32_t g = 0; g < groups; g++) {
+                    if (progress[g] > n) throw RenderError("chained grid: a group's progress word is out of range");
+                    owed += n - progress[g];
+                }
+                if (owed != deferred) throw RenderError("chained grid: the deferred count does not match the groups' progress");
+                uint32_t* const dlist = words + 1 + max_groups;
+                HIP_CHECK(hipMemcpy(dlist, list.data(), (size_t)groups * sizeof(uint32_t), hipMemcpyHostToDevice));
+                p.chain_group_list = dlist;
+                uint32_t len = 0;
+                for (uint32_t c = 0; c < n; c++) {
+                    while (len < groups && progress[list[len]] <= c) len++;
+                    if (len == 0) continue;
+                    p.chain_list_len = len;
+                    set_launch_passes(se, chunk_passes(c), chunk_last_spp(c));
+                    LaunchTimer timer(se);
+                    HIP_CHECK(launch_pt_pass(p, se->variant, se->ctx->stream, spec_fn, se->arith_relaxed));
+                    timer.stop();
+                    se->n_launches++;
+                }
+                HIP_CHECK(hipStreamSynchronize(se->ctx->stream));
+                se->n_chain_deferred += deferred;
+            }
+            se->fold_events(true);
+            se->spp_done = done;
+            se->passes_launched += n_fused;
+            left -= n_fused;
+            return true;
+        };
+        while (left > 0 && se->spp_done < total)
+            if (!chain()) launch(kMaxFusedPasses);
         if (blocking) HIP_CHECK(hipStreamSynchronize(se->ctx->stream));
         if (spp_done) *spp_done = se->spp_done;
     });
@@ -677,6 +763,8 @@
         stats->n_tri_tests = c[5];
         stats->kernel_ms = ms;
         stats->n_launches = se->n_launches;
+        stats->n_chain_deferred = se->n_chain_deferred;
+        stats->_pad2 = 0;
         stats->_pad = (uint32_t)c[6];
     }
     if (c[6] != 0) throw RenderError("BVH traversal stack overflow: the render is incomplete");
diff --git a/akari_render_amd/csrc/host/scene_build.cpp b/akari_render_amd/csrc/host/scene_build.cpp
--- a/akari_render_amd/csrc/host/scene_build.cpp
+++ b/akari_render_amd/csrc/host/scene_build.cpp
@@ -784,6 +784,12 @@
     if (n == "specialise") return &g_tuning.specialise;
     if (n == "specialise_waves") return &g_tuning.specialise_waves;
     if (n == "max_fused_passes") return &g_tuning.max_fused_passes;
+    if (n == "chain_passes") return &g_tuning.chain_passes;
+    if (n == "chain_rounds") return &g_tuning.chain_rounds;
+    if (n == "max_chain_ms") return &g_tuning.max_chain_ms;
+#if defined(AKR_TEST_HOOKS) && AKR_TEST_HOOKS
+    if (n == "chain_test_defer") return &g_tuning.chain_test_defer;
+#endif
     if (n == "wf_sort") return &g_tuning.wf_sort;
     if (n == "lens") return &g_tuning.lens;
     if (n == "instancing") return &g_tuning.instancing;
@@ -821,6 +827,10 @@
     if (f == &g_tuning.specialise && (value < -1 || value > 1)) return false;
     if (f == &g_tuning.specialise_waves && value != 0 && (value < 2 || value > 4)) return false;
     if (f == &g_tuning.max_fused_passes && (value < 0 || value > 64)) return false;
+    if (f == &g_tuning.chain_passes && (value < 0 || value > 2)) return false;
+    if (f == &g_tuning.chain_rounds && (value < 1 || value > 64)) return false;
+    if (f == &g_tuning.max_chain_ms && value < 1) return false;
+    if (f == &g_tuning.chain_test_defer && value != 0 && (value < 0 || (value & 1023) == 0 || ((value >> 10) & 1023) >= (value & 1023))) return false;
     if (f == &g_tuning.wf_sort && (value < 0 || value > 1)) return false;
     if (f == &g_tuning.lens && (value < 0 || value > 1)) return false;
     if (f == &g_tuning.instancing && (value < -1 || value > 1)) return false;
diff --git a/akari_render_amd/csrc/host/scene_build.h b/akari_render_amd/csrc/host/scene_build.h
--- a/akari_render_amd/csrc/host/scene_build.h
+++ b/akari_render_amd/csrc/host/scene_build.h
@@ -169,6 +169,7 @@
 void compile_materials(const FlatScene& flat, uint32_t color, CompiledScene& out, std::vector<akr_material_desc>& descs);
 void build_alias_table(const std::vector<float>& weights, std::vector<AliasEntry>& entries, std::vector<float>& pdf);
 struct TuningOptions {
+    int chain_passes = 1, chain_rounds = 2, max_chain_ms = 20000, chain_test_defer = 0;
     int force_bvh = 0, bvh_balanced = 0, defer_metal = -1, wavefront = -1, simple_kernels = 1;
     int defer_on = 0;
     int specialise = -1, specialise_waves = 0;
diff --git a/akari_render_amd/csrc/kernels.h b/akari_render_amd/csrc/kernels.h
--- a/akari_render_amd/csrc/kernels.h
+++ b/akari_render_amd/csrc/kernels.h
@@ -130,6 +130,14 @@
     const uint32_t* owned_tiles;
     float lens_radius, lens_focal;
     float *feat_albedo, *feat_normal;
+    uint32_t chain_chunks, chain_groups, chain_groups_padded;
+    uint32_t chain_pad0_, chain_pad1_;
+    uint32_t chain_list_len;
+    uint32_t chain_test_m, chain_test_r, chain_test_c0;
+    uint32_t chain_pad_;
+    uint32_t* chain_progress;
+    uint32_t* chain_deferred;
+    const uint32_t* chain_group_list;
 };
 
 AKR_HD uint32_t morton_spread16(uint32_t x) {
@@ -225,7 +233,7 @@
 hipError_t launch_inst_share_bits(const DScene& sc, uint32_t* bits, uint32_t* mesh_tri_words, hipStream_t stream);
 hipError_t launch_probe_env(const PtParams& p, uint32_t mode, uint32_t n, const float* in, float* out, hipStream_t stream);
 hipError_t launch_probe_camera_rays(const PtParams& p, uint32_t n, const uint32_t* pixels2, const float* u4, float* out6, hipStream_t stream);
-hipError_t launch_pt_pass(const PtParams& p, const PtVariant& v, hipStream_t stream, hipFunction_t spec_fn = nullptr, bool relaxed = false);
+hipError_t launch_pt_pass(const PtParams& p, const PtVariant& v, hipStream_t stream, hipFunction_t spec_fn = nullptr, bool relaxed = false, int* occupancy = nullptr);
 hipError_t launch_gpt_sample(const PtParams& p, const GptParams& g, hipStream_t stream);
 hipError_t launch_gpt_update(const GptParams& g, uint32_t W, uint32_t H, float* film, hipStream_t stream);
 hipError_t launch_gpt_recon_init(const GptParams& g, uint32_t W, uint32_t H, float* old, float spp, hipStream_t stream);
diff --git a/akari_render_amd/csrc/launch.h b/akari_render_amd/csrc/launch.h
--- a/akari_render_amd/csrc/launch.h
+++ b/akari_render_amd/csrc/launch.h
@@ -17,5 +17,11 @@
     if (BIG_LDS && lds > 64 * 1024) (void)hipFuncSetAttribute((const void*)kernel, hipFuncAttributeMaxDynamicSharedMemorySize, (int)lds);
     hipLaunchKernelGGL(kernel, dim3(blocks), dim3(256), lds, stream, args...);
 }
+template <bool BIG_LDS = false, class... P, class... A>
+void launch_kernel_or_occupancy(int* occupancy, void (*kernel)(P...), uint32_t blocks, size_t lds, hipStream_t stream, const A&... args) {
+    if (occupancy == nullptr) return launch_kernel<BIG_LDS>(kernel, blocks, lds, stream, args...);
+    if (BIG_LDS && lds > 64 * 1024) (void)hipFuncSetAttribute((const void*)kernel, hipFuncAttributeMaxDynamicSharedMemorySize, (int)lds);
+    if (hipOccupancyMaxActiveBlocksPerMultiprocessor(occupancy, (const void*)kernel, 256, lds) != hipSuccess) *occupancy = 0;
+}
 
 }
diff --git a/akari_render_amd/csrc/pt_env_kernels.hip b/akari_render_amd/csrc/pt_env_kernels.hip
--- a/akari_render_amd/csrc/pt_env_kernels.hip
+++ b/akari_render_amd/csrc/pt_env_kernels.hip
@@ -2,7 +2,7 @@
 
 namespace akr {
 
-hipError_t pt_pass_entry_env(const PtParams& q, const PtVariant& v, uint32_t blocks, size_t lds, hipStream_t stream) { return pt_pass_entry_t<true, false>(q, v, blocks, lds, stream); }
+hipError_t pt_pass_entry_env(const PtParams& q, const PtVariant& v, uint32_t blocks, size_t lds, hipStream_t stream, int* occupancy) { return pt_pass_entry_t<true, false>(q, v, blocks, lds, stream, occupancy); }
 
 __global__ void k_probe_env(const DEnv* __restrict__ env_p, uint32_t color, uint32_t mode, uint32_t n, const float* __restrict__ in, float* __restrict__ out) {
     const uint32_t i = blockIdx.x * blockDim.x + threadIdx.x;
diff --git a/akari_render_amd/csrc/pt_feat_env_kernels.hip b/akari_render_amd/csrc/pt_feat_env_kernels.hip
--- a/akari_render_amd/csrc/pt_feat_env_kernels.hip
+++ b/akari_render_amd/csrc/pt_feat_env_kernels.hip
@@ -2,6 +2,6 @@
 
 namespace akr {
 
-hipError_t pt_pass_entry_feat_env(const PtParams& q, const PtVariant& v, uint32_t blocks, size_t lds, hipStream_t stream) { return pt_pass_entry_t<true, false, true>(q, v, blocks, lds, stream); }
+hipError_t pt_pass_entry_feat_env(const PtParams& q, const PtVariant& v, uint32_t blocks, size_t lds, hipStream_t stream, int* occupancy) { return pt_pass_entry_t<true, false, true>(q, v, blocks, lds, stream, occupancy); }
 
 }
diff --git a/akari_render_amd/csrc/pt_feat_kernels.hip b/akari_render_amd/csrc/pt_feat_kernels.hip
--- a/akari_render_amd/csrc/pt_feat_kernels.hip
+++ b/akari_render_amd/csrc/pt_feat_kernels.hip
@@ -2,6 +2,6 @@
 
 namespace akr {
 
-hipError_t pt_pass_entry_feat(const PtParams& q, const PtVariant& v, uint32_t blocks, size_t lds, hipStream_t stream) { return pt_pass_entry_t<false, false, true>(q, v, blocks, lds, stream); }
+hipError_t pt_pass_entry_feat(const PtParams& q, const PtVariant& v, uint32_t blocks, size_t lds, hipStream_t stream, int* occupancy) { return pt_pass_entry_t<false, false, true>(q, v, blocks, lds, stream, occupancy); }
 
 }
diff --git a/akari_render_amd/csrc/pt_feat_lens_env_kernels.hip b/akari_render_amd/csrc/pt_feat_lens_env_kernels.hip
--- a/akari_render_amd/csrc/pt_feat_lens_env_kernels.hip
+++ b/akari_render_amd/csrc/pt_feat_lens_env_kernels.hip
@@ -2,6 +2,6 @@
 
 namespace akr {
 
-hipError_t pt_pass_entry_feat_lens_env(const PtParams& q, const PtVariant& v, uint32_t blocks, size_t lds, hipStream_t stream) { return pt_pass_entry_t<true, true, true>(q, v, blocks, lds, stream); }
+hipError_t pt_pass_entry_feat_lens_env(const PtParams& q, const PtVariant& v, uint32_t blocks, size_t lds, hipStream_t stream, int* occupancy) { return pt_pass_entry_t<true, true, true>(q, v, blocks, lds, stream, occupancy); }
 
 }
diff --git a/akari_render_amd/csrc/pt_feat_lens_kernels.hip b/akari_render_amd/csrc/pt_feat_lens_kernels.hip
--- a/akari_render_amd/csrc/pt_feat_lens_kernels.hip
+++ b/akari_render_amd/csrc/pt_feat_lens_kernels.hip
@@ -2,6 +2,6 @@
 
 namespace akr {
 
-hipError_t pt_pass_entry_feat_lens(const PtParams& q, const PtVariant& v, uint32_t blocks, size_t lds, hipStream_t stream) { return pt_pass_entry_t<false, true, true>(q, v, blocks, lds, stream); }
+hipError_t pt_pass_entry_feat_lens(const PtParams& q, const PtVariant& v, uint32_t blocks, size_t lds, hipStream_t stream, int* occupancy) { return pt_pass_entry_t<false, true, true>(q, v, blocks, lds, stream, occupancy); }
 
 }
diff --git a/akari_render_amd/csrc/pt_inst_env_kernels.hip b/akari_render_amd/csrc/pt_inst_env_kernels.hip
--- a/akari_render_amd/csrc/pt_inst_env_kernels.hip
+++ b/akari_render_amd/csrc/pt_inst_env_kernels.hip
@@ -2,6 +2,6 @@
 
 namespace akr {
 
-hipError_t pt_pass_entry_inst_env(const PtParams& q, const PtVariant& v, uint32_t blocks, size_t lds, hipStream_t stream) { return pt_pass_entry_inst_t<true, false>(q, v, blocks, lds, stream); }
+hipError_t pt_pass_entry_inst_env(const PtParams& q, const PtVariant& v, uint32_t blocks, size_t lds, hipStream_t stream, int* occupancy) { return pt_pass_entry_inst_t<true, false>(q, v, blocks, lds, stream, occupancy); }
 
 }
diff --git a/akari_render_amd/csrc/pt_inst_kernel.h b/akari_render_amd/csrc/pt_inst_kernel.h
--- a/akari_render_amd/csrc/pt_inst_kernel.h
+++ b/akari_render_amd/csrc/pt_inst_kernel.h
@@ -16,9 +16,9 @@
 }
 
 template <bool ENV, bool LENS>
-hipError_t pt_pass_entry_inst_t(const PtParams& q, const PtVariant& v, uint32_t blocks, size_t lds, hipStream_t stream) {
+hipError_t pt_pass_entry_inst_t(const PtParams& q, const PtVariant& v, uint32_t blocks, size_t lds, hipStream_t stream, int* occupancy) {
     if (!v.inst || v.env != ENV || v.lens != LENS || !pt_variant_compiled(v)) return hipErrorInvalidValue;
-    dispatch_bools([&](auto F, auto T, auto P) { launch_kernel<true>(k_pt_pass_inst<F(), T(), P(), ENV, LENS>, blocks, lds, stream, q); }, v.fd, v.tex, v.pmj);
+    dispatch_bools([&](auto F, auto T, auto P) { launch_kernel_or_occupancy<true>(occupancy, k_pt_pass_inst<F(), T(), P(), ENV, LENS>, blocks, lds, stream, q); }, v.fd, v.tex, v.pmj);
     return hipGetLastError();
 }
 
diff --git a/akari_render_amd/csrc/pt_inst_kernels.hip b/akari_render_amd/csrc/pt_inst_kernels.hip
--- a/akari_render_amd/csrc/pt_inst_kernels.hip
+++ b/akari_render_amd/csrc/pt_inst_kernels.hip
@@ -25,6 +25,6 @@
     return hipGetLastError();
 }
 
-hipError_t pt_pass_entry_inst(const PtParams& q, const PtVariant& v, uint32_t blocks, size_t lds, hipStream_t stream) { return pt_pass_entry_inst_t<false, false>(q, v, blocks, lds, stream); }
+hipError_t pt_pass_entry_inst(const PtParams& q, const PtVariant& v, uint32_t blocks, size_t lds, hipStream_t stream, int* occupancy) { return pt_pass_entry_inst_t<false, false>(q, v, blocks, lds, stream, occupancy); }
 
 }
diff --git a/akari_render_amd/csrc/pt_inst_lens_kernels.hip b/akari_render_amd/csrc/pt_inst_lens_kernels.hip
--- a/akari_render_amd/csrc/pt_inst_lens_kernels.hip
+++ b/akari_render_amd/csrc/pt_inst_lens_kernels.hip
@@ -2,7 +2,7 @@
 
 namespace akr {
 
-hipError_t pt_pass_entry_inst_lens_env(const PtParams& q, const PtVariant& v, uint32_t blocks, size_t lds, hipStream_t stream) { return pt_pass_entry_inst_t<true, true>(q, v, blocks, lds, stream); }
-hipError_t pt_pass_entry_inst_lens(const PtParams& q, const PtVariant& v, uint32_t blocks, size_t lds, hipStream_t stream) { return pt_pass_entry_inst_t<false, true>(q, v, blocks, lds, stream); }
+hipError_t pt_pass_entry_inst_lens_env(const PtParams& q, const PtVariant& v, uint32_t blocks, size_t lds, hipStream_t stream, int* occupancy) { return pt_pass_entry_inst_t<true, true>(q, v, blocks, lds, stream, occupancy); }
+hipError_t pt_pass_entry_inst_lens(const PtParams& q, const PtVariant& v, uint32_t blocks, size_t lds, hipStream_t stream, int* occupancy) { return pt_pass_entry_inst_t<false, true>(q, v, blocks, lds, stream, occupancy); }
 
 }
diff --git a/akari_render_amd/csrc/pt_kernels.hip b/akari_render_amd/csrc/pt_kernels.hip
--- a/akari_render_amd/csrc/pt_kernels.hip
+++ b/akari_render_amd/csrc/pt_kernels.hip
@@ -189,28 +189,32 @@
 }
 
 }
-extern "C" hipError_t akr_launch_pt_pass_relaxed(const void* params, const PtVariant* v, uint32_t blocks, size_t lds, hipStream_t stream);
+extern "C" hipError_t akr_launch_pt_pass_relaxed(const void* params, const PtVariant* v, uint32_t blocks, size_t lds, hipStream_t stream, int* occupancy);
 namespace akr {
-static hipError_t pt_pass_entry_plain(const PtParams& q, const PtVariant& v, uint32_t blocks, size_t lds, hipStream_t stream) { return pt_pass_entry_t<false, false>(q, v, blocks, lds, stream); }
+static hipError_t pt_pass_entry_plain(const PtParams& q, const PtVariant& v, uint32_t blocks, size_t lds, hipStream_t stream, int* occupancy) { return pt_pass_entry_t<false, false>(q, v, blocks, lds, stream, occupancy); }
 static constexpr PtPassEntry kPtPassEntry[2][2][2] = {{{pt_pass_entry_plain, pt_pass_entry_lens}, {pt_pass_entry_env, pt_pass_entry_lens_env}},
                                                       {{pt_pass_entry_inst, pt_pass_entry_inst_lens}, {pt_pass_entry_inst_env, pt_pass_entry_inst_lens_env}}};
 static constexpr PtPassEntry kPtPassEntryFeat[2][2] = {{pt_pass_entry_feat, pt_pass_entry_feat_lens}, {pt_pass_entry_feat_env, pt_pass_entry_feat_lens_env}};
-hipError_t launch_pt_pass(const PtParams& p, const PtVariant& v, hipStream_t stream, hipFunction_t spec_fn, bool relaxed) {
-    const uint32_t blocks = (p.n_items + 255u) / 256u;
+hipError_t launch_pt_pass(const PtParams& p, const PtVariant& v, hipStream_t stream, hipFunction_t spec_fn, bool relaxed, int* occupancy) {
+    const uint32_t groups = (p.n_items + 255u) / 256u;
+    const uint32_t blocks = p.chain_chunks != 0 ? p.chain_chunks * p.chain_groups_padded : (p.chain_group_list != nullptr ? p.chain_list_len : groups);
+    if (p.chain_chunks != 0 && (p.chain_groups != groups || p.chain_groups_padded < groups || p.chain_progress == nullptr || p.chain_deferred == nullptr)) return hipErrorInvalidValue;
+    if (occupancy) *occupancy = 0;
     if (blocks == 0) return hipSuccess;
     const PtLdsLayout L = pt_lds_layout(v, pt_lds_sizes(p));
     const PtParams q = pt_params_with_layout(p, L);
     if (v.feat) {
         if (spec_fn || relaxed || v.inst) return hipErrorInvalidValue;
-        return kPtPassEntryFeat[v.env][v.lens](q, v, blocks, L.total_bytes, stream);
+        return kPtPassEntryFeat[v.env][v.lens](q, v, blocks, L.total_bytes, stream, occupancy);
     }
     if (spec_fn) {
         if (L.total_bytes > 64 * 1024) (void)hipFuncSetAttribute((const void*)spec_fn, hipFuncAttributeMaxDynamicSharedMemorySize, (int)L.total_bytes);
+        if (occupancy) return hipModuleOccupancyMaxActiveBlocksPerMultiprocessor(occupancy, spec_fn, 256, L.total_bytes);
         void* args[] = {(void*)&q};
         return hipModuleLaunchKernel(spec_fn, blocks, 1, 1, 256, 1, 1, (unsigned)L.total_bytes, stream, args, nullptr);
     }
-    if (relaxed) return akr_launch_pt_pass_relaxed(&q, &v, blocks, L.total_bytes, stream);
-    return kPtPassEntry[v.inst][v.env][v.lens](q, v, blocks, L.total_bytes, stream);
+    if (relaxed) return akr_launch_pt_pass_relaxed(&q, &v, blocks, L.total_bytes, stream, occupancy);
+    return kPtPassEntry[v.inst][v.env][v.lens](q, v, blocks, L.total_bytes, stream, occupancy);
 }
 hipError_t launch_probe_material(const PtParams& p, uint32_t material, uint32_t n, const float* uv, uint32_t* out, hipStream_t stream) {
     size_t lds;
diff --git a/akari_render_amd/csrc/pt_kernels_relaxed.hip b/akari_render_amd/csrc/pt_kernels_relaxed.hip
--- a/akari_render_amd/csrc/pt_kernels_relaxed.hip
+++ b/akari_render_amd/csrc/pt_kernels_relaxed.hip
@@ -7,6 +7,6 @@
 #include "pt_launch.h"
 #undef akr
 
-extern "C" hipError_t akr_launch_pt_pass_relaxed(const void* params, const PtVariant* v, uint32_t blocks, size_t lds, hipStream_t stream) {
-    return akr_rx::pt_pass_entry_t<false, false>(*static_cast<const akr_rx::PtParams*>(params), *v, blocks, lds, stream);
+extern "C" hipError_t akr_launch_pt_pass_relaxed(const void* params, const PtVariant* v, uint32_t blocks, size_t lds, hipStream_t stream, int* occupancy) {
+    return akr_rx::pt_pass_entry_t<false, false>(*static_cast<const akr_rx::PtParams*>(params), *v, blocks, lds, stream, occupancy);
 }
diff --git a/akari_render_amd/csrc/pt_launch.h b/akari_render_amd/csrc/pt_launch.h
--- a/akari_render_amd/csrc/pt_launch.h
+++ b/akari_render_amd/csrc/pt_launch.h
@@ -9,26 +9,26 @@
     pt_pass_body<BVH, FD, TEX, PMJ, STAGE, DEFER, SIMPLE ? AB_SIMPLE : 0u, false, ENV, LENS, FEAT>(p);
 }
 
-using PtPassEntry = hipError_t (*)(const PtParams& q, const PtVariant& v, uint32_t blocks, size_t lds, hipStream_t stream);
-hipError_t pt_pass_entry_env(const PtParams& q, const PtVariant& v, uint32_t blocks, size_t lds, hipStream_t stream);
-hipError_t pt_pass_entry_lens(const PtParams& q, const PtVariant& v, uint32_t blocks, size_t lds, hipStream_t stream);
-hipError_t pt_pass_entry_lens_env(const PtParams& q, const PtVariant& v, uint32_t blocks, size_t lds, hipStream_t stream);
-hipError_t pt_pass_entry_feat(const PtParams& q, const PtVariant& v, uint32_t blocks, size_t lds, hipStream_t stream);
-hipError_t pt_pass_entry_feat_env(const PtParams& q, const PtVariant& v, uint32_t blocks, size_t lds, hipStream_t stream);
-hipError_t pt_pass_entry_feat_lens(const PtParams& q, const PtVariant& v, uint32_t blocks, size_t lds, hipStream_t stream);
-hipError_t pt_pass_entry_feat_lens_env(const PtParams& q, const PtVariant& v, uint32_t blocks, size_t lds, hipStream_t stream);
-hipError_t pt_pass_entry_inst(const PtParams& q, const PtVariant& v, uint32_t blocks, size_t lds, hipStream_t stream);
-hipError_t pt_pass_entry_inst_env(const PtParams& q, const PtVariant& v, uint32_t blocks, size_t lds, hipStream_t stream);
-hipError_t pt_pass_entry_inst_lens(const PtParams& q, const PtVariant& v, uint32_t blocks, size_t lds, hipStream_t stream);
-hipError_t pt_pass_entry_inst_lens_env(const PtParams& q, const PtVariant& v, uint32_t blocks, size_t lds, hipStream_t stream);
+using PtPassEntry = hipError_t (*)(const PtParams& q, const PtVariant& v, uint32_t blocks, size_t lds, hipStream_t stream, int* occupancy);
+hipError_t pt_pass_entry_env(const PtParams& q, const PtVariant& v, uint32_t blocks, size_t lds, hipStream_t stream, int* occupancy);
+hipError_t pt_pass_entry_lens(const PtParams& q, const PtVariant& v, uint32_t blocks, size_t lds, hipStream_t stream, int* occupancy);
+hipError_t pt_pass_entry_lens_env(const PtParams& q, const PtVariant& v, uint32_t blocks, size_t lds, hipStream_t stream, int* occupancy);
+hipError_t pt_pass_entry_feat(const PtParams& q, const PtVariant& v, uint32_t blocks, size_t lds, hipStream_t stream, int* occupancy);
+hipError_t pt_pass_entry_feat_env(const PtParams& q, const PtVariant& v, uint32_t blocks, size_t lds, hipStream_t stream, int* occupancy);
+hipError_t pt_pass_entry_feat_lens(const PtParams& q, const PtVariant& v, uint32_t blocks, size_t lds, hipStream_t stream, int* occupancy);
+hipError_t pt_pass_entry_feat_lens_env(const PtParams& q, const PtVariant& v, uint32_t blocks, size_t lds, hipStream_t stream, int* occupancy);
+hipError_t pt_pass_entry_inst(const PtParams& q, const PtVariant& v, uint32_t blocks, size_t lds, hipStream_t stream, int* occupancy);
+hipError_t pt_pass_entry_inst_env(const PtParams& q, const PtVariant& v, uint32_t blocks, size_t lds, hipStream_t stream, int* occupancy);
+hipError_t pt_pass_entry_inst_lens(const PtParams& q, const PtVariant& v, uint32_t blocks, size_t lds, hipStream_t stream, int* occupancy);
+hipError_t pt_pass_entry_inst_lens_env(const PtParams& q, const PtVariant& v, uint32_t blocks, size_t lds, hipStream_t stream, int* occupancy);
 
 template <bool ENV, bool LENS, bool FEAT = false>
-hipError_t pt_pass_entry_t(const PtParams& q, const PtVariant& v, uint32_t blocks, size_t lds, hipStream_t stream) {
+hipError_t pt_pass_entry_t(const PtParams& q, const PtVariant& v, uint32_t blocks, size_t lds, hipStream_t stream, int* occupancy) {
     if (v.inst || v.env != ENV || v.lens != LENS || v.feat != FEAT || !pt_variant_compiled(v)) return hipErrorInvalidValue;
     if (FEAT && (q.feat_albedo == nullptr || q.feat_normal == nullptr)) return hipErrorInvalidValue;
     dispatch_bools([&](auto B, auto F, auto T, auto P, auto S, auto D, auto X) {
         if constexpr (pt_variant_compiled(PtVariant{B(), F(), T(), P(), S(), D(), X(), false, ENV, LENS, FEAT}))
-            launch_kernel<true>(k_pt_pass<B(), F(), T(), P(), S(), D(), X(), ENV, LENS, FEAT>, blocks, lds, stream, q);
+            launch_kernel_or_occupancy<true>(occupancy, k_pt_pass<B(), F(), T(), P(), S(), D(), X(), ENV, LENS, FEAT>, blocks, lds, stream, q);
     }, v.bvh, v.fd, v.tex, v.pmj, v.stage, v.defer, v.simple);
     return hipGetLastError();
 }
diff --git a/akari_render_amd/csrc/pt_lens_env_kernels.hip b/akari_render_amd/csrc/pt_lens_env_kernels.hip
--- a/akari_render_amd/csrc/pt_lens_env_kernels.hip
+++ b/akari_render_amd/csrc/pt_lens_env_kernels.hip
@@ -2,6 +2,6 @@
 
 namespace akr {
 
-hipError_t pt_pass_entry_lens_env(const PtParams& q, const PtVariant& v, uint32_t blocks, size_t lds, hipStream_t stream) { return pt_pass_entry_t<true, true>(q, v, blocks, lds, stream); }
+hipError_t pt_pass_entry_lens_env(const PtParams& q, const PtVariant& v, uint32_t blocks, size_t lds, hipStream_t stream, int* occupancy) { return pt_pass_entry_t<true, true>(q, v, blocks, lds, stream, occupancy); }
 
 }
diff --git a/akari_render_amd/csrc/pt_lens_kernels.hip b/akari_render_amd/csrc/pt_lens_kernels.hip
--- a/akari_render_amd/csrc/pt_lens_kernels.hip
+++ b/akari_render_amd/csrc/pt_lens_kernels.hip
@@ -2,7 +2,7 @@
 
 namespace akr {
 
-hipError_t pt_pass_entry_lens(const PtParams& q, const PtVariant& v, uint32_t blocks, size_t lds, hipStream_t stream) { return pt_pass_entry_t<false, true>(q, v, blocks, lds, stream); }
+hipError_t pt_pass_entry_lens(const PtParams& q, const PtVariant& v, uint32_t blocks, size_t lds, hipStream_t stream, int* occupancy) { return pt_pass_entry_t<false, true>(q, v, blocks, lds, stream, occupancy); }
 
 __global__ void k_probe_camera_rays(const PtParams p, uint32_t n, const uint32_t* __restrict__ pixels, const float* __restrict__ u, float* __restrict__ out) {
     const uint32_t i = blockIdx.x * blockDim.x + threadIdx.x;
diff --git a/include/akari_hip.h b/include/akari_hip.h
--- a/include/akari_hip.h
+++ b/include/akari_hip.h
@@ -158,6 +158,8 @@
     double kernel_ms;
     uint32_t n_launches;
     uint32_t _pad;
+    uint32_t n_chain_deferred;
+    uint32_t _pad2;
 } akr_pt_stats;
 
 
```

Measured after the change: 3396. -2.1%, worse.
